# Galtvam/OthelloZero

Measured on AMD Instinct MI355X. Metric: mcts_node_expansions_per_sec, higher is better.
Workload: dtype f32 (3xbf16 split)

## Files before the change

include/othellozero_amd.h:

```cpp
#ifndef OTHELLOZERO_AMD_H
#define OTHELLOZERO_AMD_H
#include <stdint.h>
#ifdef __cplusplus
extern "C" {
#endif

#define OZ_OK 0
#define OZ_ERR_HIP 1
#define OZ_ERR_ARG 2
#define OZ_ERR_CAPACITY 3
#define OZ_ERR_KEY 4
#define OZ_ERR_STATE 5

#define OZ_QMODE_NEP50 0
#define OZ_QMODE_F64 1

#define OZ_LEAF_IDLE 0
#define OZ_LEAF_TERMINAL 1
#define OZ_LEAF_EVAL 2
#define OZ_LEAF_WAIT 3

const char* oz_last_error(void);
int oz_version(void);
int oz_device_count(void);
// ... 13 lines not shown
#define OZ_MINIMAX_NONE INT32_MIN
int oz_rules_minimax(const uint64_t* black, const uint64_t* white, const int8_t* player, int n, int count, int depth, int eval,
                     int32_t* values, uint64_t* bests);

#define OZ_SOLVE_MAX_EMPTIES 12
int oz_rules_solve(const uint64_t* black, const uint64_t* white, const int8_t* player, int n, int count, int max_empties,
                   int32_t* values , uint64_t* bests , int32_t* value , uint8_t* solved );
int oz_rules_solve_sign(const uint64_t* black, const uint64_t* white, const int8_t* player, int n, int count, int max_empties,
                        int8_t* sign , uint8_t* solved );
#define OZ_OPENING_MAX_PLIES 16
int oz_rules_random_openings(int n, int64_t count, int plies, uint64_t opening_seed, uint64_t first_opening_id,
                             uint64_t* black, uint64_t* white, int8_t* player, uint8_t* finished,
                             uint8_t* actions , int32_t* n_plies);
int oz_rules_profile(int enable);
int oz_rules_profile_read(double* ms_total, int64_t* launches, int reset);

typedef struct oz_net oz_net;
int oz_net_create(oz_net** out, int n, int channels, int max_batch);
int oz_net_create_bnn(oz_net** out, int n, int channels, int max_batch);
int oz_net_create_stub(oz_net** out, int n, uint64_t salt, uint64_t keep_mask, int max_batch);
int oz_net_destroy(oz_net* net);
int oz_net_num_weights(const oz_net* net);
int oz_net_weight_size(const oz_net* net, int index, int64_t* nelem);
int oz_net_set_weight(oz_net* net, int index, const float* data, int64_t nelem);
int oz_net_get_weight(const oz_net* net, int index, float* data, int64_t nelem);
int oz_net_init_random(oz_net* net, uint64_t seed);
int oz_net_set_precision(oz_net* net, int mode);
int oz_net_get_precision(const oz_net* net);
int oz_net_check(oz_net* net);
int oz_net_commit(oz_net* net);
int oz_net_predict(oz_net* net, const uint64_t* own, const uint64_t* opp, int count, float* pi, float* v);
int oz_net_predict_boards(oz_net* net, const uint8_t* boards_nhwc, int count, float* pi, float* v);
int oz_net_time_forward(oz_net* net, int count, int iters, float* ms_avg);
int oz_net_profile(oz_net* net, int enable );
int oz_net_profile_read(oz_net* net, double* conv2_ms_total, int64_t* conv2_launches);
#define OZ_NET_KERNELS 7
int oz_net_profile_kernels(oz_net* net, double* ms_total , int64_t* launches , int reset);
int oz_net_profiled_layer(oz_net* net, int* layer);
int oz_net_set_tables(oz_net* net, int mode);
int oz_net_set_eval_cache(oz_net* net, int64_t entries);
int oz_net_eval_cache_stats(oz_net* net, int64_t* entries, int64_t* lookups, int64_t* hits, int64_t* inserts);
#define OZ_NET_OPT_SIMPLE_LOOP 1
#define OZ_NET_OPT_ACT_TARGET_LOG2 2
#define OZ_NET_OPT_LOW_GUARD_LOG2 3
#define OZ_NET_OPT_SELF_CHECK 4
#define OZ_NET_OPT_W_TARGET_LOG2 5
#define OZ_NET_OPT_F32_STD_TILE 6
#define OZ_NET_OPT_LATENCY_SPLITS 7
#define OZ_NET_OPT_CONV3_TILE 8
#define OZ_NET_OPT_LOW_LOOP_PHASES 9
#define OZ_NET_OPT_B3_TILE 10
int oz_net_set_option(oz_net* net, int option, int value);
int oz_net_self_check(oz_net* net, double* max_dpi, double* max_dv, int* positions);
int oz_net_get_scaling(oz_net* net, int which, int32_t* out, int64_t nelem);
#define OZ_NET_INFO_CONV3_TILE_ROWS 1
#define OZ_NET_INFO_SELF_CHECK_GUARD 2
#define OZ_NET_INFO_ARITHMETIC 3
#define OZ_NET_INFO_LAYER_TILE_ROWS(l) (16 + (l))
#define OZ_NET_INFO_LAYER_KSLICES(l) (32 + (l))
#define OZ_NET_INFO_LAYER_KERNEL(l) (48 + (l))
enum {
    OZ_NET_KERNEL_NONE = 0,
    OZ_NET_KERNEL_F32_SKINNY = 1,
    OZ_NET_KERNEL_F32_STD = 2,
    OZ_NET_KERNEL_F32_STD_PIXMAJOR = 3,
    OZ_NET_KERNEL_F32_BIG = 4,
    OZ_NET_KERNEL_LUT = 5,
    OZ_NET_KERNEL_LUT_XCD = 6,
    OZ_NET_KERNEL_LUT_XCD_INLINE = 7,
    OZ_NET_KERNEL_H2_SMALL2 = 10, OZ_NET_KERNEL_H2_SMALL = 11, OZ_NET_KERNEL_H2_BIGPP = 12, OZ_NET_KERNEL_H2_BIGPP_LUT = 13,
    OZ_NET_KERNEL_H2_MIDPP = 14, OZ_NET_KERNEL_H2_LOWPP1 = 15, OZ_NET_KERNEL_H2_LOWPP = 16, OZ_NET_KERNEL_H2_BIG = 17, OZ_NET_KERNEL_H2_MID = 18,
    OZ_NET_KERNEL_H2_THIN2 = 19, OZ_NET_KERNEL_H2_THIN = 20, OZ_NET_KERNEL_H2_THIN4W = 21,
    OZ_NET_KERNEL_B3 = 30,
    OZ_NET_KERNEL_B3_BIG = 31
};
int oz_net_get_info(oz_net* net, int what, int* value);
int oz_net_get_activation(oz_net* net, int layer, int64_t first_row, int64_t rows, double* out );

typedef struct oz_mcts oz_mcts;
int oz_mcts_create(oz_mcts** out, int n, int num_games, int node_cap, double c, int q_mode);
int oz_mcts_destroy(oz_mcts* m);
int oz_mcts_reset(oz_mcts* m, int game );
int oz_mcts_set_dedup(oz_mcts* m, int enable);
int oz_mcts_set_roots(oz_mcts* m, const uint64_t* own, const uint64_t* opp, const uint8_t* active);
int oz_mcts_simulate(oz_mcts* m, oz_net* net, int nsims);
int oz_mcts_select(oz_mcts* m);
int oz_mcts_leaves(oz_mcts* m, int32_t* status, uint64_t* own, uint64_t* opp);
int oz_mcts_backup(oz_mcts* m, const float* pi , const float* v );
int oz_mcts_last_value(oz_mcts* m, double* value, int32_t* vtype, int32_t* depth);
int oz_mcts_root_counts(oz_mcts* m, int32_t* counts, uint64_t* legal, int32_t* rc);
int oz_mcts_policy(oz_mcts* m, double temperature, const uint64_t* tie_draws, double* policy, int32_t* rc);
int oz_mcts_num_nodes(oz_mcts* m, int32_t* num_nodes );
int oz_mcts_dump_node(oz_mcts* m, int game, int index, uint64_t* own, uint64_t* opp, int32_t* Ns, uint64_t* legal,
                      int32_t* N , double* Q , uint8_t* qtag , double* P );
int oz_mcts_stats(oz_mcts* m, int64_t* out5);

#define OZ_MCTS_MAX_LEAVES_PER_STEP 16
int oz_mcts_set_leaves_per_step(oz_mcts* m, int k);
int oz_mcts_get_leaves_per_step(oz_mcts* m, int* k);
int oz_mcts_use_wide_kernels(oz_mcts* m, int enable);
int oz_mcts_wide_stats(oz_mcts* m, int64_t* out3);

#define OZ_SOLVE_LEAVES_MAX_EMPTIES 10
int oz_mcts_set_solve_leaves(oz_mcts* m, int max_empties);
int oz_mcts_get_solve_leaves(oz_mcts* m, int* max_empties, int64_t* rows_solved );
int oz_mcts_solve_leaves_profile(oz_mcts* m, int enable);
int oz_mcts_solve_leaves_profile_read(oz_mcts* m, double* ms_total, int64_t* launches, int reset);

int oz_mcts_set_root_noise(oz_mcts* m, double eps, const double* eta, const uint8_t* armed);
int oz_mcts_sample_root_noise(oz_mcts* m, double alpha, double eps, uint64_t seed, const uint64_t* game_ids, const int32_t* plies);
int oz_mcts_get_root_noise(oz_mcts* m, double* eta , uint8_t* armed , double* eps);

int oz_mcts_sample_moves(oz_mcts* m, double temperature, uint64_t seed, const uint64_t* game_ids, const int32_t* plies,
                         int32_t* action , int32_t* rc );

typedef struct oz_selfplay oz_selfplay;
typedef struct {
    int32_t n;
    int32_t num_games;
    int32_t sims;
    int32_t q_mode;
    double c;
    double temperature;
    double e_greedy;
    uint64_t seed;
    uint64_t first_game_id;
    uint64_t game_id_stride;
    int32_t refill;
    int32_t node_cap;
    int32_t reserved0;
    int32_t record_cap;
    int32_t dedup;
    int32_t batch_cap;
    int32_t eval_cache;
    int32_t record_visits;
} oz_selfplay_config;
#define OZ_DEDUP_DEFAULT 0
#define OZ_DEDUP_ON 1
#define OZ_DEDUP_OFF 2

typedef struct {
    uint64_t black, white;
    uint64_t final_black, final_white;
    uint64_t game_id;
    uint8_t ply;
    uint8_t action;
    int8_t player;
    int8_t z;
    uint8_t greedy;
    uint8_t pad[3];
} oz_record;

typedef struct {
    int64_t simulations, node_visits, expansions, terminal_hits, fallbacks;
    int64_t moves, games_completed, records;
    int32_t live_games, overflow;
    int64_t leaves_evaluated;
} oz_selfplay_stats;

int oz_selfplay_create(oz_selfplay** out, const oz_selfplay_config* cfg, oz_net* net);
int oz_selfplay_destroy(oz_selfplay* sp);
int oz_selfplay_run(oz_selfplay* sp, int rounds);
int oz_selfplay_run_steps(oz_selfplay* sp, int steps);
int oz_selfplay_set_batch_cap(oz_selfplay* sp, int cap);
int oz_selfplay_set_dedup(oz_selfplay* sp, int enable);
int oz_selfplay_set_leaves_per_step(oz_selfplay* sp, int k);
int oz_selfplay_set_solve_leaves(oz_selfplay* sp, int max_empties);
int oz_selfplay_get_solve_leaves(oz_selfplay* sp, int* max_empties, int64_t* rows_solved);
int oz_selfplay_solve_leaves_profile(oz_selfplay* sp, int enable);
int oz_selfplay_solve_leaves_profile_read(oz_selfplay* sp, double* ms_total, int64_t* launches, int reset);
int oz_selfplay_set_root_noise(oz_selfplay* sp, double alpha, double eps);
int oz_selfplay_root_noise(oz_selfplay* sp, double* eta, uint8_t* armed);
int oz_selfplay_set_move_sampling(oz_selfplay* sp, double temperature, int plies);
int oz_selfplay_sync(oz_selfplay* sp);
int oz_selfplay_stagger(oz_selfplay* sp, int sims_pre);
#define OZ_TREE_KERNELS 5
int oz_selfplay_profile(oz_selfplay* sp, int enable);
int oz_selfplay_profile_read(oz_selfplay* sp, double* ms_total , int64_t* launches , int reset);
int oz_selfplay_get_stats(oz_selfplay* sp, oz_selfplay_stats* out);
int oz_selfplay_state(oz_selfplay* sp, uint64_t* black, uint64_t* white, int8_t* player, uint8_t* finished,
                      int32_t* ply, uint64_t* game_id);
int oz_selfplay_records(oz_selfplay* sp, oz_record* out, int64_t max_records, int64_t* written);
int oz_selfplay_records_device(oz_selfplay* sp, void* dst_device, int64_t max_records, int64_t* written);
int oz_selfplay_visits(oz_selfplay* sp, int32_t* out , int64_t max_records, int64_t* written);
int oz_selfplay_visits_device(oz_selfplay* sp, void* dst_device, int64_t max_records, int64_t* written);
typedef struct {
    int64_t records;
    int64_t solved;
    int64_t z_changed;
    int64_t optimal_moves;
    int64_t disc_loss_sum;
    int32_t disc_loss_max, pad;
} oz_endgame_stats;
int oz_selfplay_solve_records(oz_selfplay* sp, int64_t first_record, int max_empties, oz_endgame_stats* stats );
int oz_selfplay_last_counts(oz_selfplay* sp, int32_t* counts);
int oz_selfplay_eval_time(oz_selfplay* sp, double* ms_total, int64_t* launches, int64_t* leaves);

typedef struct oz_comm oz_comm;
#define OZ_COMM_ID_BYTES 128
int oz_comm_unique_id(uint8_t* id );
int oz_comm_create(oz_comm** out, const uint8_t* id, int rank, int world);
int oz_comm_destroy(oz_comm* comm);
int oz_selfplay_gather_records(oz_selfplay* sp, oz_comm* comm, int64_t first_record, oz_record* out, int64_t max_records, int64_t* written,
                               int64_t* per_rank);
int oz_selfplay_gather_visits(oz_selfplay* sp, oz_comm* comm, int64_t first_record, int32_t* out , int64_t max_records,
                              int64_t* written, int64_t* per_rank);

typedef struct oz_arena oz_arena;
int oz_arena_create(oz_arena** out, int n, int num_games, int sims, double c, int q_mode, uint64_t seed,
                    uint64_t first_game_id, oz_net* net_a, oz_net* net_b, int node_cap);
int oz_arena_destroy(oz_arena* a);
int oz_arena_run(oz_arena* a);
int oz_arena_run_rounds(oz_arena* a, int max_rounds);
int oz_arena_stats(oz_arena* a, int64_t* black5, int64_t* white5);
int oz_arena_set_dedup(oz_arena* a, int enable);
int oz_arena_leaves_evaluated(oz_arena* a, int64_t* black, int64_t* white);
int oz_arena_set_eval_cache(oz_arena* a, int enable);
int oz_arena_set_leaves_per_step(oz_arena* a, int k_black, int k_white);
int oz_arena_set_solve_leaves(oz_arena* a, int black, int white);
int oz_arena_get_solve_leaves(oz_arena* a, int64_t* rows_black, int64_t* rows_white);
int oz_arena_profile(oz_arena* a, int enable);
int oz_arena_profile_read(oz_arena* a, double* ms_total , int64_t* launches , int reset);
#define OZ_AGENT_RANDOM 0
#define OZ_AGENT_MINIMAX 1
int oz_arena_set_opponent(oz_arena* a, int side , int kind, int depth, int eval);
int oz_arena_opponent_time(oz_arena* a, double* ms_total, int64_t* launches);
int oz_arena_set_openings(oz_arena* a, int plies, uint64_t opening_seed, uint64_t first_opening_id);
int oz_arena_set_opening_moves(oz_arena* a, const uint8_t* moves , const int32_t* n_plies );
int oz_arena_opening_plies(oz_arena* a, int32_t* out );
int oz_arena_results(oz_arena* a, int8_t* winner , int32_t* points, int32_t* n_moves,
                     uint8_t* actions , int8_t* players ,
                     uint64_t* final_black, uint64_t* final_white);

int oz_examples_expand(const oz_record* records, int64_t count, int n, int alias_final, uint8_t* boards,
                       int32_t* policy_index, int8_t* z);
int oz_symmetry_table(int n, int32_t* perm );
int oz_examples_expand_visits(const oz_record* records, const int32_t* counts, int64_t count, int n, int alias_final, double temperature,
                              uint8_t* boards, double* pi, int8_t* z);

typedef struct oz_trainer oz_trainer;
int oz_trainer_arena_size(int n, int channels, int in_channels, int64_t* nelem);
int oz_trainer_create(oz_trainer** out, int n, int channels, int in_channels, int max_batch, float lr, float clipvalue ,
                      float dropout, float bn_momentum, uint64_t seed, float* external_grads);
int oz_trainer_destroy(oz_trainer* t);
int oz_trainer_set_precision(oz_trainer* t, int mode);
#define OZ_POLICY_LOSS_ROWS 0
#define OZ_POLICY_LOSS_FLAT 1
int oz_trainer_set_policy_loss(oz_trainer* t, int mode);
int oz_trainer_set_weight(oz_trainer* t, int index, const float* data, int64_t nelem);
int oz_trainer_get_weight(oz_trainer* t, int index, float* data, int64_t nelem);
int oz_trainer_get_grad(oz_trainer* t, int index, float* data, int64_t nelem);
int oz_trainer_grad_arena(oz_trainer* t, void** device_ptr, int64_t* nelem);
int oz_trainer_forward_backward(oz_trainer* t, const uint64_t* own, const uint64_t* opp, const float* pi_target,
                                const float* z_target, int B, float* losses3);
int oz_trainer_apply(oz_trainer* t);
int oz_trainer_set_dataset(oz_trainer* t, const uint64_t* own, const uint64_t* opp, const float* pi_target, const float* z_target, int64_t N);
int oz_trainer_fit_epoch(oz_trainer* t, const int32_t* order, int64_t count, int batch, float* losses3);
int oz_trainer_outputs(oz_trainer* t, int B, float* p , float* v );
int oz_trainer_get_activation(oz_trainer* t, int layer, int B, float* data, int64_t nelem);
#define OZ_TRAINER_PLAN_FIELDS 8
#define OZ_TRAINER_PLAN_FWD_KSLICES 0
#define OZ_TRAINER_PLAN_FWD_KERNEL 1
#define OZ_TRAINER_PLAN_DGRAD_KSLICES 2
#define OZ_TRAINER_PLAN_DGRAD_KERNEL 3
#define OZ_TRAINER_PLAN_DGRAD_TAP_SKIP 4
#define OZ_TRAINER_PLAN_WGRAD_KERNEL 5
#define OZ_TRAINER_PLAN_WGRAD_MSPLIT 6
enum {
    OZ_TRAINER_WGRAD_TAPS_F32 = 1,
    OZ_TRAINER_WGRAD_BOARDS_F32 = 2,
    OZ_TRAINER_WGRAD_OCT_H2 = 3,
    OZ_TRAINER_WGRAD_OCT_B3 = 4
};
int oz_trainer_get_preact(oz_trainer* t, int layer, int B, float* data, int64_t nelem);
int oz_trainer_get_dz(oz_trainer* t, int layer, int B, float* data, int64_t nelem);
int oz_trainer_set_capture(oz_trainer* t, int on);
int oz_trainer_get_dgrad(oz_trainer* t, int layer, int B, float* data, int64_t nelem);
int oz_trainer_get_head_grads(oz_trainer* t, int B, float* dlogit , float* dvpre );
int oz_trainer_get_plan(oz_trainer* t, int* plan, int n);
int oz_trainer_sync(oz_trainer* t);
int oz_trainer_step_count(oz_trainer* t, int64_t* step);

typedef struct oz_replay oz_replay;
#define OZ_REPLAY_TARGET_ONEHOT 0
#define OZ_REPLAY_TARGET_VISITS 1
int oz_replay_create(oz_replay** out, int n, int64_t capacity );
int oz_replay_destroy(oz_replay* r);
int oz_replay_clear(oz_replay* r);
int oz_replay_info(oz_replay* r, int64_t* held, int64_t* capacity, int64_t* total);
int oz_replay_append_selfplay(oz_replay* r, oz_selfplay* sp, int64_t first_record, int alias_final, int target, double temperature,
                              int64_t* appended_records);
int oz_replay_append_records(oz_replay* r, const oz_record* records, const int32_t* counts, int64_t count, int alias_final,
                             int target, double temperature);
int oz_replay_append_examples(oz_replay* r, const uint64_t* own, const uint64_t* opp, const float* pi ,
                              const float* z, int64_t count);
int oz_replay_restore(oz_replay* r, const uint64_t* own, const uint64_t* opp, const float* pi, const float* z, int64_t count, int64_t total);
int oz_replay_read(oz_replay* r, int64_t first_slot, int64_t count, uint64_t* own, uint64_t* opp, float* pi, float* z);
int oz_trainer_fit_epoch_replay(oz_trainer* t, oz_replay* r, const int32_t* order, int64_t count, int batch, float* losses3);

int oz_selftest_arith(const double* a, const double* b, int count, double* sqrt_a, double* div_ab, float* fdiv_ab,
                      float* fchain);
int oz_selftest_mfma_rate(int kind, double target_ms, double* tflops, double* clock_ghz, double* ms_measured);
int oz_selftest_b3_split(const float* x, int64_t count, float* planes, float* sum);

#ifdef __cplusplus
}
#endif
#endif
```

othellozero_amd/_lib.py:

```python
import ctypes as C
import os

import numpy as np

_HERE = os.path.dirname(os.path.abspath(__file__))
LIB_PATH = os.environ.get("OZ_LIB_PATH") or os.path.join(_HERE, "lib", "libothellozero_amd.so")

OZ_OK, OZ_ERR_HIP, OZ_ERR_ARG, OZ_ERR_CAPACITY, OZ_ERR_KEY, OZ_ERR_STATE = range(6)
QMODE_NEP50, QMODE_F64 = 0, 1
DEDUP_DEFAULT, DEDUP_ON, DEDUP_OFF = 0, 1, 2
NET_OPT_SIMPLE_LOOP, NET_OPT_ACT_TARGET_LOG2, NET_OPT_LOW_GUARD_LOG2, NET_OPT_SELF_CHECK, NET_OPT_W_TARGET_LOG2, NET_OPT_F32_STD_TILE, NET_OPT_LATENCY_SPLITS = 1, 2, 3, 4, 5, 6, 7
NET_OPT_CONV3_TILE = 8
NET_OPT_LOW_LOOP_PHASES = 9
NET_OPT_B3_TILE = 10
NET_INFO_CONV3_TILE_ROWS, NET_INFO_SELF_CHECK_GUARD, NET_INFO_ARITHMETIC = 1, 2, 3
NET_INFO_LAYER_TILE_ROWS, NET_INFO_LAYER_KSLICES, NET_INFO_LAYER_KERNEL = 16, 32, 48
NET_KERNEL_NAMES = {0: "none", 1: "f32_skinny", 2: "f32_std", 3: "f32_std_pixmajor", 4: "f32_big", 5: "lut", 6: "lut_xcd", 7: "lut_xcd_inline",
                    10: "h2_small2", 11: "h2_small", 12: "h2_bigpp", 13: "h2_bigpp_lut", 14: "h2_midpp", 15: "h2_lowpp1", 16: "h2_lowpp", 17: "h2_big",
                    18: "h2_mid", 19: "h2_thin2", 20: "h2_thin", 21: "h2_thin4w", 30: "b3", 31: "b3_big"}
LEAF_IDLE, LEAF_TERMINAL, LEAF_EVAL = 0, 1, 2
VT_INT, VT_F32, VT_F64 = 0, 1, 2
MAX_LEAVES_PER_STEP = 16
POLICY_LOSS_ROWS, POLICY_LOSS_FLAT = 0, 1
TRAINER_PLAN_FIELDS = 8
TRAINER_WGRAD_NAMES = {0: "none", 1: "taps_f32", 2: "boards_f32", 3: "oct_h2", 4: "oct_b3"}
MINIMAX_EVAL_DISCS, MINIMAX_EVAL_WEIGHTED, MINIMAX_MAX_DEPTH, MINIMAX_NONE = 0, 1, 6, -2 ** 31
MINIMAX_EVALS = {"discs": MINIMAX_EVAL_DISCS, "weighted": MINIMAX_EVAL_WEIGHTED}
SOLVE_MAX_EMPTIES = 12
SOLVE_LEAVES_MAX_EMPTIES = 10
AGENT_RANDOM, AGENT_MINIMAX = 0, 1
OPENING_MAX_PLIES = 16
REPLAY_TARGET_ONEHOT, REPLAY_TARGET_VISITS = 0, 1
NET_KERNELS = ("input", "conv2", "conv3", "conv4", "fc1", "fc2", "heads")
TREE_KERNELS = ("select", "compact", "network", "expand_backup", "roots_move")


class OzLibraryError(RuntimeError):
    pass


class OzError(RuntimeError):
    def __init__(self, code, msg):
        super().__init__(f"[oz error {code}] {msg}")
        self.code = code


class SelfplayConfig(C.Structure):
    _fields_ = [
        ("n", C.c_int32), ("num_games", C.c_int32), ("sims", C.c_int32), ("q_mode", C.c_int32),
        ("c", C.c_double), ("temperature", C.c_double), ("e_greedy", C.c_double),
        ("seed", C.c_uint64), ("first_game_id", C.c_uint64), ("game_id_stride", C.c_uint64),
        ("refill", C.c_int32), ("node_cap", C.c_int32), ("reserved0", C.c_int32), ("record_cap", C.c_int32),
        ("dedup", C.c_int32), ("batch_cap", C.c_int32), ("eval_cache", C.c_int32), ("record_visits", C.c_int32),
    ]


class SelfplayStats(C.Structure):
    _fields_ = [
        ("simulations", C.c_int64), ("node_visits", C.c_int64), ("expansions", C.c_int64),
        ("terminal_hits", C.c_int64), ("fallbacks", C.c_int64),
        ("moves", C.c_int64), ("games_completed", C.c_int64), ("records", C.c_int64),
        ("live_games", C.c_int32), ("overflow", C.c_int32),
        ("leaves_evaluated", C.c_int64),
    ]


class EndgameStats(C.Structure):
    _fields_ = [
        ("records", C.c_int64), ("solved", C.c_int64), ("z_changed", C.c_int64), ("optimal_moves", C.c_int64), ("disc_loss_sum", C.c_int64),
        ("disc_loss_max", C.c_int32), ("pad", C.c_int32),
    ]


RECORD_DTYPE = np.dtype([
    ("black", "<u8"), ("white", "<u8"), ("final_black", "<u8"), ("final_white", "<u8"), ("game_id", "<u8"),
    ("ply", "u1"), ("action", "u1"), ("player", "i1"), ("z", "i1"), ("greedy", "u1"), ("pad", "u1", (3,)),
])
assert RECORD_DTYPE.itemsize == 48

_u64p, _i32p, _f32p, _f64p = (C.POINTER(t) for t in (C.c_uint64, C.c_int32, C.c_float, C.c_double))
_u8p, _i8p, _i64p, _vp = C.POINTER(C.c_uint8), C.POINTER(C.c_int8), C.POINTER(C.c_int64), C.c_void_p

SIGNATURES = {
    "oz_version": [], "oz_device_count": [], "oz_set_device": [C.c_int],
    "oz_rules_legal_moves": [_u64p, _u64p, C.c_int, C.c_int, _u64p],
    "oz_rules_apply_moves": [_u64p, _u64p, _u8p, C.c_int, C.c_int, _u64p, _u64p],
    "oz_rules_status": [_u64p, _u64p, C.c_int, C.c_int, _u8p, _i32p, _i32p, _i8p],
    "oz_rules_play": [_u64p, _u64p, _i8p, _u8p, C.c_int, C.c_int, _u64p, _u64p, _i8p, _u8p],
    "oz_rules_minimax": [_u64p, _u64p, _i8p, C.c_int, C.c_int, C.c_int, C.c_int, _i32p, _u64p],
    "oz_rules_solve": [_u64p, _u64p, _i8p, C.c_int, C.c_int, C.c_int, _i32p, _u64p, _i32p, _u8p],
    "oz_rules_solve_sign": [_u64p, _u64p, _i8p, C.c_int, C.c_int, C.c_int, _i8p, _u8p],
    "oz_rules_random_openings": [C.c_int, C.c_int64, C.c_int, C.c_uint64, C.c_uint64, _u64p, _u64p, _i8p, _u8p, _u8p, _i32p],
    "oz_rules_profile": [C.c_int], "oz_rules_profile_read": [_f64p, _i64p, C.c_int],
    "oz_selfplay_solve_records": [_vp, C.c_int64, C.c_int, C.POINTER(EndgameStats)],
    "oz_net_create": [C.POINTER(_vp), C.c_int, C.c_int, C.c_int],
    "oz_net_create_bnn": [C.POINTER(_vp), C.c_int, C.c_int, C.c_int],
    "oz_net_create_stub": [C.POINTER(_vp), C.c_int, C.c_uint64, C.c_uint64, C.c_int],
    "oz_net_destroy": [_vp], "oz_net_num_weights": [_vp],
    "oz_net_weight_size": [_vp, C.c_int, _i64p],
    "oz_net_set_weight": [_vp, C.c_int, _f32p, C.c_int64],
    "oz_net_get_weight": [_vp, C.c_int, _f32p, C.c_int64],
    "oz_net_commit": [_vp],
    "oz_net_set_precision": [_vp, C.c_int], "oz_net_get_precision": [_vp], "oz_net_check": [_vp],
    "oz_net_init_random": [_vp, C.c_uint64],
    "oz_net_predict": [_vp, _u64p, _u64p, C.c_int, _f32p, _f32p],
    "oz_net_predict_boards": [_vp, _u8p, C.c_int, _f32p, _f32p],
    "oz_net_time_forward": [_vp, C.c_int, C.c_int, _f32p],
    "oz_net_profile": [_vp, C.c_int], "oz_net_profile_read": [_vp, _f64p, _i64p],
    "oz_net_profiled_layer": [_vp, C.POINTER(C.c_int)], "oz_net_set_tables": [_vp, C.c_int],
    "oz_net_profile_kernels": [_vp, _f64p, _i64p, C.c_int],
    "oz_net_set_eval_cache": [_vp, C.c_int64], "oz_net_eval_cache_stats": [_vp, _i64p, _i64p, _i64p, _i64p],
    "oz_net_set_option": [_vp, C.c_int, C.c_int], "oz_net_get_info": [_vp, C.c_int, C.POINTER(C.c_int)],
    "oz_net_get_scaling": [_vp, C.c_int, _i32p, C.c_int64],
    "oz_net_get_activation": [_vp, C.c_int, C.c_int64, C.c_int64, _f64p],
    "oz_net_self_check": [_vp, _f64p, _f64p, C.POINTER(C.c_int)],
    "oz_mcts_create": [C.POINTER(_vp), C.c_int, C.c_int, C.c_int, C.c_double, C.c_int],
    "oz_mcts_destroy": [_vp], "oz_mcts_reset": [_vp, C.c_int], "oz_mcts_set_dedup": [_vp, C.c_int],
    "oz_mcts_set_roots": [_vp, _u64p, _u64p, _u8p],
    "oz_mcts_simulate": [_vp, _vp, C.c_int], "oz_mcts_select": [_vp],
    "oz_mcts_leaves": [_vp, _i32p, _u64p, _u64p],
    "oz_mcts_backup": [_vp, _f32p, _f32p],
    "oz_mcts_last_value": [_vp, _f64p, _i32p, _i32p],
    "oz_mcts_root_counts": [_vp, _i32p, _u64p, _i32p],
    "oz_mcts_policy": [_vp, C.c_double, _u64p, C.POINTER(C.c_double), _i32p],
    "oz_mcts_num_nodes": [_vp, _i32p],
    "oz_mcts_dump_node": [_vp, C.c_int, C.c_int, _u64p, _u64p, _i32p, _u64p, _i32p, _f64p, _u8p, _f64p],
    "oz_mcts_stats": [_vp, _i64p],
    "oz_mcts_set_leaves_per_step": [_vp, C.c_int], "oz_mcts_get_leaves_per_step": [_vp, C.POINTER(C.c_int)],
    "oz_mcts_use_wide_kernels": [_vp, C.c_int], "oz_mcts_wide_stats": [_vp, _i64p],
    "oz_selfplay_set_leaves_per_step": [_vp, C.c_int], "oz_arena_set_leaves_per_step": [_vp, C.c_int, C.c_int],
    "oz_mcts_set_solve_leaves": [_vp, C.c_int], "oz_mcts_get_solve_leaves": [_vp, C.POINTER(C.c_int), _i64p],
    "oz_mcts_solve_leaves_profile": [_vp, C.c_int], "oz_mcts_solve_leaves_profile_read": [_vp, _f64p, _i64p, C.c_int],
    "oz_selfplay_set_solve_leaves": [_vp, C.c_int], "oz_selfplay_get_solve_leaves": [_vp, C.POINTER(C.c_int), _i64p],
    "oz_selfplay_solve_leaves_profile": [_vp, C.c_int], "oz_selfplay_solve_leaves_profile_read": [_vp, _f64p, _i64p, C.c_int],
    "oz_arena_set_solve_leaves": [_vp, C.c_int, C.c_int], "oz_arena_get_solve_leaves": [_vp, _i64p, _i64p],
    "oz_mcts_set_root_noise": [_vp, C.c_double, _f64p, _u8p],
    "oz_mcts_sample_root_noise": [_vp, C.c_double, C.c_double, C.c_uint64, _u64p, _i32p],
    "oz_mcts_get_root_noise": [_vp, _f64p, _u8p, _f64p],
    "oz_selfplay_set_root_noise": [_vp, C.c_double, C.c_double], "oz_selfplay_root_noise": [_vp, _f64p, _u8p],
    "oz_mcts_sample_moves": [_vp, C.c_double, C.c_uint64, _u64p, _i32p, _i32p, _i32p],
    "oz_selfplay_set_move_sampling": [_vp, C.c_double, C.c_int],
    "oz_selfplay_create": [C.POINTER(_vp), C.POINTER(SelfplayConfig), _vp],
    "oz_selfplay_destroy": [_vp], "oz_selfplay_run": [_vp, C.c_int], "oz_selfplay_run_steps": [_vp, C.c_int], "oz_selfplay_sync": [_vp],
    "oz_selfplay_stagger": [_vp, C.c_int], "oz_selfplay_profile": [_vp, C.c_int], "oz_selfplay_set_batch_cap": [_vp, C.c_int], "oz_selfplay_set_dedup": [_vp, C.c_int],
    "oz_selfplay_profile_read": [_vp, _f64p, _i64p, C.c_int],
    "oz_selfplay_get_stats": [_vp, C.POINTER(SelfplayStats)],
    "oz_selfplay_state": [_vp, _u64p, _u64p, _i8p, _u8p, _i32p, _u64p],
    "oz_selfplay_records": [_vp, _vp, C.c_int64, _i64p],
    "oz_selfplay_records_device": [_vp, _vp, C.c_int64, _i64p],
    "oz_selfplay_visits": [_vp, _i32p, C.c_int64, _i64p],
    "oz_selfplay_visits_device": [_vp, _vp, C.c_int64, _i64p],
    "oz_selfplay_last_counts": [_vp, _i32p],
    "oz_selfplay_eval_time": [_vp, _f64p, _i64p, _i64p],
    "oz_comm_unique_id": [_u8p], "oz_comm_create": [C.POINTER(_vp), _u8p, C.c_int, C.c_int], "oz_comm_destroy": [_vp],
    "oz_selfplay_gather_records": [_vp, _vp, C.c_int64, _vp, C.c_int64, _i64p, _i64p],
    "oz_selfplay_gather_visits": [_vp, _vp, C.c_int64, _i32p, C.c_int64, _i64p, _i64p],
    "oz_arena_create": [C.POINTER(_vp), C.c_int, C.c_int, C.c_int, C.c_double, C.c_int, C.c_uint64, C.c_uint64, _vp, _vp, C.c_int],
    "oz_arena_destroy": [_vp], "oz_arena_run": [_vp], "oz_arena_run_rounds": [_vp, C.c_int], "oz_arena_stats": [_vp, _i64p, _i64p],
    "oz_arena_set_dedup": [_vp, C.c_int], "oz_arena_set_eval_cache": [_vp, C.c_int], "oz_arena_profile": [_vp, C.c_int], "oz_arena_profile_read": [_vp, _f64p, _i64p, C.c_int], "oz_arena_leaves_evaluated": [_vp, _i64p, _i64p],
    "oz_arena_set_opponent": [_vp, C.c_int, C.c_int, C.c_int, C.c_int], "oz_arena_opponent_time": [_vp, _f64p, _i64p],
    "oz_arena_set_openings": [_vp, C.c_int, C.c_uint64, C.c_uint64], "oz_arena_set_opening_moves": [_vp, _u8p, _i32p],
    "oz_arena_opening_plies": [_vp, _i32p],
    "oz_arena_results": [_vp, _i8p, _i32p, _i32p, _u8p, _i8p, _u64p, _u64p],
    "oz_examples_expand": [_vp, C.c_int64, C.c_int, C.c_int, _u8p, _i32p, _i8p],
    "oz_examples_expand_visits": [_vp, _i32p, C.c_int64, C.c_int, C.c_int, C.c_double, _u8p, _f64p, _i8p],
    "oz_symmetry_table": [C.c_int, _i32p],
    "oz_selftest_arith": [_f64p, _f64p, C.c_int, _f64p, _f64p, _f32p, _f32p],
    "oz_selftest_mfma_rate": [C.c_int, C.c_double, _f64p, _f64p, _f64p],
    "oz_selftest_b3_split": [_f32p, C.c_int64, _f32p, _f32p],
    "oz_trainer_arena_size": [C.c_int, C.c_int, C.c_int, C.POINTER(C.c_int64)],
    "oz_trainer_create": [C.POINTER(_vp), C.c_int, C.c_int, C.c_int, C.c_int, C.c_float, C.c_float, C.c_float, C.c_float,
                          C.c_uint64, _vp],
    "oz_trainer_destroy": [_vp],
    "oz_trainer_set_weight": [_vp, C.c_int, _f32p, C.c_int64],
    "oz_trainer_get_weight": [_vp, C.c_int, _f32p, C.c_int64],
    "oz_trainer_get_grad": [_vp, C.c_int, _f32p, C.c_int64],
    "oz_trainer_grad_arena": [_vp, C.POINTER(_vp), C.POINTER(C.c_int64)],
    "oz_trainer_forward_backward": [_vp, _u64p, _u64p, _f32p, _f32p, C.c_int, _f32p],
    "oz_trainer_apply": [_vp],
    "oz_trainer_set_dataset": [_vp, _u64p, _u64p, _f32p, _f32p, C.c_int64],
    "oz_trainer_fit_epoch": [_vp, _i32p, C.c_int64, C.c_int, _f32p],
    "oz_trainer_outputs": [_vp, C.c_int, _f32p, _f32p],
    "oz_trainer_get_activation": [_vp, C.c_int, C.c_int, _f32p, C.c_int64],
    "oz_trainer_get_preact": [_vp, C.c_int, C.c_int, _f32p, C.c_int64], "oz_trainer_get_dz": [_vp, C.c_int, C.c_int, _f32p, C.c_int64],
    "oz_trainer_set_capture": [_vp, C.c_int], "oz_trainer_get_dgrad": [_vp, C.c_int, C.c_int, _f32p, C.c_int64],
    "oz_trainer_get_plan": [_vp, _i32p, C.c_int],
    "oz_trainer_get_head_grads": [_vp, C.c_int, _f32p, _f32p],
    "oz_trainer_sync": [_vp],
    "oz_trainer_set_precision": [_vp, C.c_int],
    "oz_trainer_set_policy_loss": [_vp, C.c_int],
    "oz_trainer_step_count": [_vp, C.POINTER(C.c_int64)],
    "oz_replay_create": [C.POINTER(_vp), C.c_int, C.c_int64], "oz_replay_destroy": [_vp], "oz_replay_clear": [_vp],
    "oz_replay_info": [_vp, _i64p, _i64p, _i64p],
    "oz_replay_append_selfplay": [_vp, _vp, C.c_int64, C.c_int, C.c_int, C.c_double, _i64p],
    "oz_replay_append_records": [_vp, _vp, _i32p, C.c_int64, C.c_int, C.c_int, C.c_double],
    "oz_replay_append_examples": [_vp, _u64p, _u64p, _f32p, _f32p, C.c_int64],
    "oz_replay_restore": [_vp, _u64p, _u64p, _f32p, _f32p, C.c_int64, C.c_int64],
    "oz_replay_read": [_vp, C.c_int64, C.c_int64, _u64p, _u64p, _f32p, _f32p],
    "oz_trainer_fit_epoch_replay": [_vp, _vp, _i32p, C.c_int64, C.c_int, _f32p],
}

_LIB = None
PRELOAD_TORCH_HIP = True


HIP_RUNTIME_BOUND = None


def _elf_dynamic_strings(path):
    import struct
    with open(path, "rb") as f:
        data = f.read()
    if data[:4] != b"\x7fELF" or data[4] != 2 or data[5] != 1:
        raise ValueError("not a little-endian ELF64 file")
    phoff, = struct.unpack_from("<Q", data, 0x20)
    phentsize, phnum = struct.unpack_from("<HH", data, 0x36)
    loads, dyn = [], None
    for k in range(phnum):
        p_type, _flags, p_offset, p_vaddr, _paddr, p_filesz = struct.unpack_from("<IIQQQQ", data, phoff + k * phentsize)
        if p_type == 1:
            loads.append((p_vaddr, p_offset, p_filesz))
        elif p_type == 2:
            dyn = (p_offset, p_filesz)
    if dyn is None:
        return None, []
    entries = [struct.unpack_from("<qQ", data, dyn[0] + 16 * k) for k in range(dyn[1] // 16)]
    strtab = next((v for t, v in entries if t == 5), None)
    if strtab is None:
        return None, []
    off = next((strtab - va + fo for va, fo, sz in loads if va <= strtab < va + sz), strtab)

    def name(idx):
        end = data.index(b"\0", off + idx)
        return data[off + idx:end].decode()
    soname = next((name(v) for t, v in entries if t == 14), None)
    return soname, [name(v) for t, v in entries if t == 1]


def _one_hip_runtime(lib_path):
    global HIP_RUNTIME_BOUND
    import importlib.util
    import sys
    import warnings
    HIP_RUNTIME_BOUND = "system"
    if not PRELOAD_TORCH_HIP:
        return
    try:
        spec = importlib.util.find_spec("torch")
        cand = os.path.join(os.path.dirname(spec.origin), "lib", "libamdhip64.so") if spec and spec.origin else None
    except Exception:
        return
    if not cand or not os.path.exists(cand):
        return
    try:
        bundled_soname, _ = _elf_dynamic_strings(cand)
        _, needed = _elf_dynamic_strings(lib_path)
        wanted = next((x for x in needed if x.startswith("libamdhip64.so")), None)
    except Exception as e:
        warnings.warn(f"othellozero_amd: could not compare PyTorch's bundled HIP runtime with the library's ({e}); using the system runtime")
        return
    if "torch" in sys.modules:
        HIP_RUNTIME_BOUND = "torch:" + cand
        if wanted and bundled_soname != wanted:
            warnings.warn(f"othellozero_amd: PyTorch's HIP runtime ({bundled_soname}) is not the one this library was linked against ({wanted}): "
                          "two HIP runtimes in one process; do not hand torch device pointers or streams to the library")
            HIP_RUNTIME_BOUND = "system"
        return
    if wanted and bundled_soname == wanted:
        C.CDLL(cand, mode=C.RTLD_GLOBAL)
        HIP_RUNTIME_BOUND = "torch:" + cand
    else:
        warnings.warn(f"othellozero_amd: PyTorch bundles HIP runtime {bundled_soname}, the library was linked against {wanted}: not preloading it; "
                      "a later `import torch` will put two HIP runtimes in this process (keep torch device pointers away from the library)")


def load(path=None):
    global _LIB
    if _LIB is not None and path is None:
        return _LIB
    p = path or LIB_PATH
    if not os.path.exists(p):
        raise OzLibraryError(
            f"{p} not found: the HIP extension is required (no CPU fallback). Build it with "
            "`python -m othellozero_amd.build` (hipcc --offload-arch=gfx950).")
    _one_hip_runtime(p)
    try:
        lib = C.CDLL(p)
    except OSError as e:
        raise OzLibraryError(f"cannot load {p}: {e}") from e
    lib.oz_last_error.restype = C.c_char_p
    lib.oz_last_error.argtypes = []
    for name, args in SIGNATURES.items():
        try:
            fn = getattr(lib, name)
        except AttributeError as e:
            raise OzLibraryError(f"{p} does not export {name}") from e
        fn.argtypes = args
        fn.restype = C.c_int
    if path is None:
        _LIB = lib
    return lib


def check_root_noise(root_noise):
    if root_noise is None:
        return None
    try:
        alpha, eps = (float(x) for x in root_noise)
    except (TypeError, ValueError):
        raise ValueError(f"root_noise must be None or (alpha, epsilon), got {root_noise!r}") from None
    if not 0.01 <= alpha <= 100.0:
        raise ValueError(f"root_noise: alpha must be in [0.01, 100] (got {alpha})")
    if not 0.0 <= eps <= 1.0:
        raise ValueError(f"root_noise: epsilon must be in [0, 1] (got {eps})")
    return alpha, eps


def check_sample_moves(sample_moves):
    if sample_moves is None:
        return None
    try:
        temperature, plies = sample_moves
        temperature = float(temperature)
        if isinstance(plies, bool) or int(plies) != plies:
            raise ValueError
        plies = int(plies)
    except (TypeError, ValueError):
        raise ValueError(f"sample_moves must be None or (temperature, plies), got {sample_moves!r}") from None
    if not 0.01 <= temperature <= 100.0:
        raise ValueError(f"sample_moves: temperature must be in [0.01, 100] (got {temperature})")
    if not 0 <= plies <= 64:
        raise ValueError(f"sample_moves: plies must be in [0, 64] (got {plies})")
    return temperature, plies


def check_minimax(depth, evaluation):
    if isinstance(depth, bool) or not isinstance(depth, (int, np.integer)) or not 1 <= depth <= MINIMAX_MAX_DEPTH:
        raise ValueError(f"minimax: depth must be a whole number in 1..{MINIMAX_MAX_DEPTH} (got {depth!r})")
    if not isinstance(evaluation, str) or evaluation not in MINIMAX_EVALS:
        raise ValueError(f"minimax: evaluation must be 'discs' or 'weighted' (got {evaluation!r})")
    return int(depth), MINIMAX_EVALS[evaluation]


def check_solve_empties(empties, least=0, what="max_empties"):
    if isinstance(empties, bool) or not isinstance(empties, (int, np.integer)) or not least <= empties <= SOLVE_MAX_EMPTIES:
        raise ValueError(f"endgame solver: {what} must be a whole number in {least}..{SOLVE_MAX_EMPTIES} (got {empties!r})")
    return int(empties)


def check_solve_leaves(solve_leaves, what="solve_leaves"):
    if (isinstance(solve_leaves, bool) or not isinstance(solve_leaves, (int, np.integer))
            or not 0 <= solve_leaves <= SOLVE_LEAVES_MAX_EMPTIES):
        raise ValueError(f"{what} must be a whole number in 0..{SOLVE_LEAVES_MAX_EMPTIES} (got {solve_leaves!r})")
    return int(solve_leaves)


def check_solve_leaves_pair(solve_leaves):
    if isinstance(solve_leaves, (tuple, list)):
        if len(solve_leaves) != 2:
            raise ValueError(f"solve_leaves must be E or (E_black, E_white) (got {solve_leaves!r})")
        return check_solve_leaves(solve_leaves[0], "solve_leaves[black]"), check_solve_leaves(solve_leaves[1], "solve_leaves[white]")
    e = check_solve_leaves(solve_leaves)
    return e, e


def check_endgame_targets(endgame_targets, alias_final_boards):
    e = check_solve_empties(endgame_targets, 0, "endgame_targets")
    if e > 0 and alias_final_boards:
        raise ValueError("endgame_targets needs alias_final_boards=False: an exact value belongs to the position of its move, not to the "
                         "game's final position")
    return e


def check_opponent(opponent):
    if opponent is None or (isinstance(opponent, str) and opponent == "random"):
        return None
    if isinstance(opponent, (tuple, list)) and len(opponent) in (2, 3) and isinstance(opponent[0], str) and opponent[0] == "minimax":
        return check_minimax(opponent[1], opponent[2] if len(opponent) == 3 else "weighted")
    raise ValueError(f"opponent must be None, 'random', ('minimax', depth) or ('minimax', depth, 'discs' | 'weighted'), got {opponent!r}")


def check_opponents(opponent, black_free, white_free):
    if isinstance(opponent, dict):
        if set(opponent) - {"black", "white"}:
            raise ValueError(f"opponent: a dict takes the keys 'black' and 'white' (got {sorted(map(str, opponent))})")
        black, white = check_opponent(opponent.get("black")), check_opponent(opponent.get("white"))
        if (black is not None and not black_free) or (white is not None and not white_free):
            raise ValueError("opponent: a colour that has a network cannot be given a minimax opponent")
        return black, white
    spec = check_opponent(opponent)
    if spec is None:
        return None, None
    if black_free and white_free:
        raise ValueError("opponent: neither colour has a network; say who plays which as {'black': ..., 'white': ...}")
    if not black_free and not white_free:
        raise ValueError("opponent: both colours have a network, there is no colour for the minimax opponent to play")
    return (spec, None) if black_free else (None, spec)


def _whole(x, lo, hi):
    return not isinstance(x, bool) and isinstance(x, (int, np.integer)) and lo <= x <= hi


def check_opening_plies(plies, what="openings"):
    if not _whole(plies, 0, OPENING_MAX_PLIES):
        raise ValueError(f"{what}: plies must be a whole number in 0..{OPENING_MAX_PLIES} (got {plies!r})")
    return int(plies)


def check_openings(openings=None, first_opening_id=0, opening_moves=None, num_games=None):
    if not _whole(first_opening_id, 0, 2 ** 64 - 1):
        raise ValueError(f"first_opening_id must be a whole number in 0..2^64 - 1 (got {first_opening_id!r})")
    if openings is not None and opening_moves is not None:
        raise ValueError("openings and opening_moves are two ways to say how the games start: give one of them")
    if openings is not None:
        if not isinstance(openings, (tuple, list)) or len(openings) != 2:
            raise ValueError(f"openings must be None or (plies, opening_seed), got {openings!r}")
        plies = check_opening_plies(openings[0])
        if not _whole(openings[1], 0, 2 ** 64 - 1):
            raise ValueError(f"openings: opening_seed must be a whole number in 0..2^64 - 1 (got {openings[1]!r})")
        return "random", plies, int(openings[1]), int(first_opening_id)
    if opening_moves is not None:
        if not isinstance(opening_moves, (tuple, list)) or len(opening_moves) != 2:
            raise ValueError(f"opening_moves must be None or (moves, n_plies), got {opening_moves!r}")
        moves, n_plies = opening_moves
        if not isinstance(moves, np.ndarray) or moves.dtype != np.uint8 or moves.ndim != 2 or moves.shape[1] != OPENING_MAX_PLIES:
            raise ValueError(f"opening_moves: moves must be a uint8 array of shape (num_games, {OPENING_MAX_PLIES})")
        if not isinstance(n_plies, np.ndarray) or n_plies.dtype != np.int32 or n_plies.shape != (moves.shape[0],):
            raise ValueError("opening_moves: n_plies must be an int32 array of shape (num_games,)")
        if num_games is not None and moves.shape[0] != num_games:
            raise ValueError(f"opening_moves: {moves.shape[0]} move lists for {num_games} games")
        if n_plies.size and (n_plies.min() < 0 or n_plies.max() > OPENING_MAX_PLIES):
            raise ValueError(f"opening_moves: every n_plies must be in 0..{OPENING_MAX_PLIES}")
        return "moves", np.ascontiguousarray(moves), np.ascontiguousarray(n_plies)
    return None


def check(rc):
    if rc != OZ_OK:
        msg = load().oz_last_error().decode("utf-8", "replace")
        if rc == OZ_ERR_KEY:
            raise KeyError(msg)
        raise OzError(rc, msg)


def require_gpu():
    lib = load()
    if lib.oz_device_count() <= 0:
        raise OzLibraryError("no HIP device visible: othellozero_amd computes on an MI355X only (no CPU fallback)")
    return lib


def mfma_rate(kind, target_ms=50.0):
    t, g, m = C.c_double(), C.c_double(), C.c_double()
    check(require_gpu().oz_selftest_mfma_rate({"f32": 0, "f16": 1, "bf16": 2}[kind], float(target_ms), C.byref(t), C.byref(g), C.byref(m)))
    return {"tflops": t.value, "clock_ghz": g.value, "ms": m.value}


def p_u64(a): return a.ctypes.data_as(_u64p)
def p_i32(a): return a.ctypes.data_as(_i32p)
def p_f32(a): return a.ctypes.data_as(_f32p)
def p_f64(a): return a.ctypes.data_as(_f64p)
def p_u8(a): return a.ctypes.data_as(_u8p)
def p_i8(a): return a.ctypes.data_as(_i8p)
def p_i64(a): return a.ctypes.data_as(_i64p)


def pack_board(board):
    b = np.asarray(board).astype(bool)
    n = b.shape[0]
    w = (np.uint64(1) << (np.arange(n, dtype=np.uint64)[:, None] * np.uint64(8) + np.arange(n, dtype=np.uint64)[None, :]))
    return int(w[b[:, :, 0]].sum(dtype=np.uint64)), int(w[b[:, :, 1]].sum(dtype=np.uint64))
# ... 9 lines not shown
```

othellozero_amd/csrc/oz_common.h:

```cpp
#pragma once
#include <hip/hip_runtime.h>
#include <math.h>
#include <stdint.h>

#define OZ_HD __host__ __device__ __forceinline__

OZ_HD uint64_t oz_sm64(uint64_t z) {
    z += 0x9E3779B97F4A7C15ULL;
    z = (z ^ (z >> 30)) * 0xBF58476D1CE4E5B9ULL;
    z = (z ^ (z >> 27)) * 0x94D049BB133111EBULL;
    return z ^ (z >> 31);
}
OZ_HD uint64_t oz_rotl64(uint64_t x, int r) { return (x << r) | (x >> (64 - r)); }

enum { OZ_RNG_COIN = 0, OZ_RNG_EXPLORE = 1, OZ_RNG_TIE = 2, OZ_RNG_NOISE = 3, OZ_RNG_SAMPLE = 4, OZ_RNG_OPENING = 5 };
OZ_HD uint64_t oz_rng(uint64_t seed, uint64_t game, uint64_t move, uint64_t stream) {
    uint64_t a = oz_sm64(seed + 0x632BE59BD9B4E019ULL * game);
    return oz_sm64(a ^ (move * 0x9E3779B97F4A7C15ULL) ^ (stream * 0xD1B54A32D192ED03ULL));
}
OZ_HD double oz_rng_unit(uint64_t u) { return (double)(u >> 11) * (1.0 / 9007199254740992.0); }

OZ_HD uint64_t oz_stub_h(uint64_t own, uint64_t opp, uint64_t salt, uint64_t i) {
    return oz_sm64(oz_sm64(own ^ salt) ^ oz_rotl64(opp, 29) ^ ((i + 1) * 0xD6E8FEB86659FD93ULL));
}

OZ_HD uint64_t oz_valid_mask(int n) {
    uint64_t row = (1ULL << n) - 1ULL, m = 0;
    for (int r = 0; r < n; ++r) m |= row << (8 * r);
    return m;
}

#define OZ_NOT_COL0 0xFEFEFEFEFEFEFEFEULL
#define OZ_NOT_COL7 0x7F7F7F7F7F7F7F7FULL

template <int D> OZ_HD uint64_t oz_shift(uint64_t x) {
    if (D == 0) return x << 8;
    if (D == 1) return x >> 8;
    if (D == 2) return (x << 1) & OZ_NOT_COL0;
    if (D == 3) return (x >> 1) & OZ_NOT_COL7;
    if (D == 4) return (x << 9) & OZ_NOT_COL0;
    if (D == 5) return (x >> 9) & OZ_NOT_COL7;
    if (D == 6) return (x << 7) & OZ_NOT_COL7;
    return (x >> 7) & OZ_NOT_COL0;
}

template <int D> OZ_HD uint64_t oz_legal_dir(uint64_t own, uint64_t opp) {
    uint64_t t = oz_shift<D>(own) & opp;
    t |= oz_shift<D>(t) & opp; t |= oz_shift<D>(t) & opp; t |= oz_shift<D>(t) & opp;
    t |= oz_shift<D>(t) & opp; t |= oz_shift<D>(t) & opp;
    return oz_shift<D>(t);
}

OZ_HD uint64_t oz_legal(uint64_t own, uint64_t opp, uint64_t valid) {
    uint64_t m = oz_legal_dir<0>(own, opp) | oz_legal_dir<1>(own, opp) | oz_legal_dir<2>(own, opp) |
                 oz_legal_dir<3>(own, opp) | oz_legal_dir<4>(own, opp) | oz_legal_dir<5>(own, opp) |
                 oz_legal_dir<6>(own, opp) | oz_legal_dir<7>(own, opp);
    return m & ~(own | opp) & valid;
}

template <int D, int B> OZ_HD uint64_t oz_flips_dir(uint64_t bit, uint64_t own, uint64_t opp) {
    uint64_t x = oz_shift<D>(bit) & opp;
    if (!x) return 0;
    const uint64_t occ = own | opp;
    uint64_t seg = x;
    seg |= oz_shift<D>(seg) & occ; seg |= oz_shift<D>(seg) & occ; seg |= oz_shift<D>(seg) & occ;
    seg |= oz_shift<D>(seg) & occ; seg |= oz_shift<D>(seg) & occ; seg |= oz_shift<D>(seg) & occ;
    uint64_t back = seg & own;
    back |= oz_shift<B>(back) & seg; back |= oz_shift<B>(back) & seg; back |= oz_shift<B>(back) & seg;
    back |= oz_shift<B>(back) & seg; back |= oz_shift<B>(back) & seg; back |= oz_shift<B>(back) & seg;
    return back & opp;
}

OZ_HD uint64_t oz_flips(uint64_t own, uint64_t opp, int sq) {
    const uint64_t bit = 1ULL << sq;
    return oz_flips_dir<0, 1>(bit, own, opp) | oz_flips_dir<1, 0>(bit, own, opp) |
           oz_flips_dir<2, 3>(bit, own, opp) | oz_flips_dir<3, 2>(bit, own, opp) |
           oz_flips_dir<4, 5>(bit, own, opp) | oz_flips_dir<5, 4>(bit, own, opp) |
           oz_flips_dir<6, 7>(bit, own, opp) | oz_flips_dir<7, 6>(bit, own, opp);
}

OZ_HD void oz_apply(uint64_t& own, uint64_t& opp, int sq) {
    const uint64_t f = oz_flips(own, opp, sq);
    own |= f | (1ULL << sq);
    opp &= ~(f | (1ULL << sq));
}

OZ_HD void oz_game_play(uint64_t& black, uint64_t& white, int& player, int& finished, int sq, uint64_t valid) {
    if (player == 1) oz_apply(black, white, sq); else oz_apply(white, black, sq);
    player = -player;
    uint64_t mine = player == 1 ? black : white, theirs = player == 1 ? white : black;
    if (oz_legal(mine, theirs, valid) == 0) {
        if (oz_legal(theirs, mine, valid) == 0) finished = 1;
        else player = -player;
    }
}

OZ_HD int oz_popc(uint64_t x) {
#if defined(__HIP_DEVICE_COMPILE__)
    return __popcll(x);
#else
    return __builtin_popcountll(x);
#endif
}
OZ_HD int oz_ctz(uint64_t x) {
#if defined(__HIP_DEVICE_COMPILE__)
    return __ffsll((unsigned long long)x) - 1;
#else
    return __builtin_ctzll(x);
#endif
}
OZ_HD int oz_kth_bit(uint64_t m, int k) {
    for (int i = 0; i < k; ++i) m &= m - 1;
    return oz_ctz(m);
}

__host__ __device__ inline double pairwise_sum(const double* a, int len) {
    double r0 = a[0], r1 = a[1], r2 = a[2], r3 = a[3], r4 = a[4], r5 = a[5], r6 = a[6], r7 = a[7];
    int i;
    for (i = 8; i < len - (len % 8); i += 8) {
        r0 += a[i]; r1 += a[i + 1]; r2 += a[i + 2]; r3 += a[i + 3];
        r4 += a[i + 4]; r5 += a[i + 5]; r6 += a[i + 6]; r7 += a[i + 7];
    }
    double res = ((r0 + r1) + (r2 + r3)) + ((r4 + r5) + (r6 + r7));
    for (; i < len; ++i) res += a[i];
    return res;
}

OZ_HD int oz_sym_src(int t, int n, int r, int c) {
    const int k = (t >> 1) + 1, flip = !(t & 1);
    int rr = r, cc = flip ? (n - 1 - c) : c;
    for (int q = 0; q < (k & 3); ++q) { int ti = cc, tj = n - 1 - rr; rr = ti; cc = tj; }
    return rr * n + cc;
}

__device__ __forceinline__ double oz_count_pow(int cnt, double inv, int k) {
    const double x = (double)cnt;
    if (k > 0) {
        double r = x;
        for (int i = 1; i < k; ++i) r *= x;
        if (r <= 9007199254740992.0) return r;
    }
    return pow(x, inv);
}
inline int oz_count_pow_k(double inv) { return (inv == floor(inv) && inv <= 64.0) ? (int)inv : 0; }

#include <stdio.h>
void oz_set_error(const char* fmt, ...);
#define OZ_HIP(call)                                                                     \
    do {                                                                                  \
        hipError_t e__ = (call);                                                          \
        if (e__ != hipSuccess) {                                                          \
            oz_set_error("%s failed: %s (%s:%d)", #call, hipGetErrorString(e__), __FILE__, __LINE__); \
            return OZ_ERR_HIP;                                                            \
        }                                                                                 \
    } while (0)
#define OZ_REQUIRE(cond, ...)                                                             \
    do {                                                                                  \
        if (!(cond)) { oz_set_error(__VA_ARGS__); return OZ_ERR_ARG; }                    \
    } while (0)

typedef float f32x4 __attribute__((ext_vector_type(4)));
typedef float f32x16 __attribute__((ext_vector_type(16)));
typedef _Float16 f16x8 __attribute__((ext_vector_type(8)));
typedef __bf16 bf16x8 __attribute__((ext_vector_type(8)));
typedef unsigned u32x4 __attribute__((ext_vector_type(4)));
typedef const __attribute__((address_space(1))) void* oz_gptr;
typedef __attribute__((address_space(3))) void* oz_lptr;

__device__ __forceinline__ void h2_split(float x, _Float16& h1, _Float16& h2) {
    h1 = (_Float16)x;
    h2 = (_Float16)(x - (float)h1);
}
__device__ __forceinline__ void b3_split(float x, __bf16& b1, __bf16& b2, __bf16& b3) {
    b1 = (__bf16)x;
    if (__builtin_isinf((float)b1) && !__builtin_isinf(x)) b1 = __builtin_bit_cast(__bf16, (unsigned short)(x < 0.f ? 0xFF7Fu : 0x7F7Fu));
    const float r1 = x - (float)b1;
    b2 = (__bf16)r1;
    b3 = (__bf16)(r1 - (float)b2);
}
template <bool NT> __device__ __forceinline__ void oz_store16(uint4* dst, u32x4 v) {
    if constexpr (NT) __builtin_nontemporal_store(v, reinterpret_cast<u32x4*>(dst));
    else *reinterpret_cast<u32x4*>(dst) = v;
}
template <int PLANES, bool NT = false>
__device__ __forceinline__ void oz_split8_store(uint4* dst, size_t pstride, const float (&v)[8]) {
    static_assert(PLANES == 2 || PLANES == 3, "f16x2 or bf16x3");
    if constexpr (PLANES == 2) {
        f16x8 h1, h2;
#pragma unroll
        for (int j = 0; j < 8; ++j) {
            _Float16 a, b;
            h2_split(v[j], a, b);
            h1[j] = a; h2[j] = b;
        }
        oz_store16<NT>(dst, __builtin_bit_cast(u32x4, h1));
        oz_store16<NT>(dst + pstride, __builtin_bit_cast(u32x4, h2));
    } else {
        bf16x8 p0, p1, p2;
#pragma unroll
        for (int j = 0; j < 8; ++j) {
            __bf16 a, b, c;
            b3_split(v[j], a, b, c);
            p0[j] = a; p1[j] = b; p2[j] = c;
        }
        oz_store16<NT>(dst, __builtin_bit_cast(u32x4, p0));
        oz_store16<NT>(dst + pstride, __builtin_bit_cast(u32x4, p1));
        oz_store16<NT>(dst + 2 * pstride, __builtin_bit_cast(u32x4, p2));
    }
}
OZ_HD size_t h2_group_chunk(size_t row, int K, int k) { return (row * (size_t)(K >> 3) + (k >> 3)) * 2; }
template <bool NT = false>
__device__ __forceinline__ void h2_store8(uint4* out, size_t row, int K, int k, const float (&v)[8]) {
    oz_split8_store<2, NT>(out + h2_group_chunk(row, K, k), 1, v);
}
OZ_HD size_t b3_group_chunk(size_t row, int K, int k) { return row * (size_t)(K / 32 * 12) + (k >> 5) * 12 + ((k >> 3) & 3); }
template <bool NT = false>
__device__ __forceinline__ void b3_store8(uint4* out, size_t row, int K, int k, const float (&v)[8]) {
    oz_split8_store<3, NT>(out + b3_group_chunk(row, K, k), 4, v);
}
template <int PLANES>
__device__ __forceinline__ void oz_split8_load(const uint4* src, size_t pstride, double (&v)[8]) {
    static_assert(PLANES == 2 || PLANES == 3, "f16x2 or bf16x3");
#pragma unroll
    for (int j = 0; j < 8; ++j) v[j] = 0.0;
#pragma unroll
    for (int p = 0; p < PLANES; ++p) {
        const u32x4 raw = *reinterpret_cast<const u32x4*>(src + p * pstride);
        if constexpr (PLANES == 2) {
            const f16x8 h = __builtin_bit_cast(f16x8, raw);
#pragma unroll
            for (int j = 0; j < 8; ++j) v[j] += (double)(float)h[j];
        } else {
            const bf16x8 b = __builtin_bit_cast(bf16x8, raw);
#pragma unroll
            for (int j = 0; j < 8; ++j) v[j] += (double)(float)b[j];
        }
    }
}
```

othellozero_amd/csrc/oz_net.hip:

```cpp
#include <math.h>
#include <stdlib.h>
#include <string.h>

#include <algorithm>
#include <type_traits>
#include <vector>

#include "oz_internal.h"

__global__ __launch_bounds__(256) void k_conv1(const uint64_t* __restrict__ own, const uint64_t* __restrict__ opp,
                                               const int* __restrict__ d_count, int n, int C,
                                               const float* __restrict__ W , const float* __restrict__ scale,
                                               const float* __restrict__ shift, float* __restrict__ out ) {
    const int P = n * n, cq = C >> 2;
    const long long M = (long long)(*d_count) * P;
    const long long idx = (long long)blockIdx.x * blockDim.x + threadIdx.x;
    const long long m = idx / cq;
    if (m >= M) return;
    const int c4 = (int)(idx % cq) * 4;
    const int b = (int)(m / P), pix = (int)(m % P), y = pix / n, x = pix % n;
    const uint64_t o = own[b], p = opp[b];
    float acc0 = 0.f, acc1 = 0.f, acc2 = 0.f, acc3 = 0.f;
#pragma unroll
    for (int ky = 0; ky < 3; ++ky)
// ... 101 lines not shown
    };
    const int swz = chunk ^ ((srow >> 1) & 7);
    static_assert((RPP / 2) % 8 == 0, "rows of one thread must share the swizzle key");
    const int wave_u = __builtin_amdgcn_readfirstlane(wave);
    const float* brow[IB];
#pragma unroll
    for (int i = 0; i < IB; ++i) brow[i] = Wt + (size_t)(nt * BN + srow + RPP * i) * g.K + swz * 4;
    const float* zsrc = g_gm_zero_line + swz * 4;

    auto stage = [&](int kt, int buf) {
        const int tap = tap_of(kt), ci0 = (kt % kpt) * GM_BK, k0 = tap * g.Cin + ci0;
        const long long toff = ((long long)(tap / 3) * g.Hin + (tap % 3)) * g.Cin + ci0 + swz * 4;
        float* la = tileA(buf);
        float* lb = tileB(buf);
#pragma unroll
        for (int i = 0; i < IA; ++i) {
            const float* ga = ((amask[i] >> tap) & 1) ? in + abase[i] + toff : zsrc;
            __builtin_amdgcn_global_load_lds((oz_gptr)ga, (oz_lptr)(la + (wave_u * 8 + RPP * i) * GM_LDS_STRIDE), 16, 0, 0);
        }
#pragma unroll
        for (int i = 0; i < IB; ++i)
            __builtin_amdgcn_global_load_lds((oz_gptr)(brow[i] + k0), (oz_lptr)(lb + (wave_u * 8 + RPP * i) * GM_LDS_STRIDE), 16, 0, 0);
    };

    f32x16 acc[TI][TJ];
#pragma unroll
    for (int i = 0; i < TI; ++i)
#pragma unroll
        for (int jj = 0; jj < TJ; ++jj)
#pragma unroll
            for (int r = 0; r < 16; ++r) acc[i][jj][r] = 0.f;

    const int nk_all = g.pixmajor ? __builtin_popcount(tmask) * kpt : g.K / GM_BK, nk_s = (nk_all + g.ksplit - 1) / g.ksplit;
    const int kt0 = blockIdx.y * nk_s, nk = min(nk_all, kt0 + nk_s);
    const int r32 = lane & 31, half = lane >> 5;
    const int key = (r32 >> 1) & 7;
    if (kt0 < nk) stage(kt0, kt0 & 1);
    asm volatile("s_waitcnt vmcnt(0)" ::: "memory");
    __syncthreads();
    for (int kt = kt0; kt < nk; ++kt) {
        const int buf = kt & 1;
        if (kt + 1 < nk) stage(kt + 1, buf ^ 1);
        const float* At = tileA(buf) + (wm * TI * 32 + r32) * GM_LDS_STRIDE;
        const float* Bt = tileB(buf) + (wn * TJ * 32 + r32) * GM_LDS_STRIDE;
        f32x4 fa[2][TI], fb[2][TJ];
        auto ldfrag = [&](int s, int w) {
            const int off = ((2 * s + half) ^ key) * 4;
#pragma unroll
            for (int i = 0; i < TI; ++i) fa[w][i] = *reinterpret_cast<const f32x4*>(At + i * 32 * GM_LDS_STRIDE + off);
#pragma unroll
            for (int jj = 0; jj < TJ; ++jj) fb[w][jj] = *reinterpret_cast<const f32x4*>(Bt + jj * 32 * GM_LDS_STRIDE + off);
        };
        ldfrag(0, 0);
#pragma unroll
        for (int s = 0; s < 4; ++s) {
            const int w = s & 1;
            if (s < 3) ldfrag(s + 1, w ^ 1);
            __builtin_amdgcn_sched_barrier(0);
#pragma unroll
            for (int q = 0; q < 4; ++q)
#pragma unroll
                for (int i = 0; i < TI; ++i)
#pragma unroll
                    for (int jj = 0; jj < TJ; ++jj)
                        acc[i][jj] = __builtin_amdgcn_mfma_f32_32x32x2f32(fa[w][i][q], fb[w][jj][q], acc[i][jj], 0, 0, 0);
            __builtin_amdgcn_sched_barrier(0);
        }
        asm volatile("s_waitcnt vmcnt(0)" ::: "memory");
        __syncthreads();
    }

    int colj[TJ];
    float scj[TJ], shj[TJ];
#pragma unroll
    for (int jj = 0; jj < TJ; ++jj) {
        colj[jj] = nt * BN + wn * TJ * 32 + jj * 32 + r32;
        scj[jj] = scale[colj[jj]]; shj[jj] = shift[colj[jj]];
    }
#pragma unroll
    for (int i = 0; i < TI; ++i)
#pragma unroll
        for (int r = 0; r < 16; ++r) {
            const int tr = wm * TI * 32 + i * 32 + (r & 3) + 8 * (r >> 2) + 4 * half;
            const long long m = g.pixmajor ? (long long)(tile_b0 + tr) * P + tile_pix : (long long)mt * BM + tr;
            const bool ok = g.pixmajor ? tile_b0 + tr < count : m < M;
            if (!ok) continue;
            if (g.ksplit > 1) {
                float* prow = partial + (size_t)blockIdx.y * g.slab + (size_t)m * g.N;
#pragma unroll
                for (int jj = 0; jj < TJ; ++jj) prow[colj[jj]] = acc[i][jj][r];
            } else {
                float* orow = out + (size_t)m * g.N;
#pragma unroll
                for (int jj = 0; jj < TJ; ++jj) {
                    float v = fmaf(acc[i][jj][r], scj[jj], shj[jj]);
                    if (g.relu) v = v > 0.f ? v : 0.f;
                    orow[colj[jj]] = v;
                }
            }
        }
}

#define SK_COLS 128
#define SK_KB_MAX 256
__global__ __launch_bounds__(256) void k_gemm_f32_skinny(const float* __restrict__ A, const float* __restrict__ Wt, const int* __restrict__ d_count,
                                                         int K, int N, int kb, float* __restrict__ partial, long long slab, GemmGeom g) {
    __shared__ __attribute__((aligned(16))) float As[64 * (SK_KB_MAX + 4)];
    const int P = g.Hout * g.Hout;
    const int M = *d_count * P;
    const int tid = threadIdx.x, lane = tid & 63, wave = tid >> 6, r32 = lane & 31, half = lane >> 5;
    const int n0 = blockIdx.x * SK_COLS + wave * 32, k0 = blockIdx.y * kb, stride = kb + 4;
    const float* wrow = Wt + (size_t)(n0 + r32) * K + k0 + 4 * half;
    f32x4 b[SK_KB_MAX / 8];
#pragma unroll
    for (int q = 0; q < SK_KB_MAX / 8; ++q)
        if (q * 8 < kb) b[q] = *reinterpret_cast<const f32x4*>(wrow + 8 * q);
    const int tiles = M > 32 ? 2 : 1, q4 = kb / 4;
    const int tap = k0 / g.Cin, ci0 = k0 - tap * g.Cin, dy = g.taps == 9 ? tap / 3 : 0, dx = g.taps == 9 ? tap % 3 : 0;
    for (int u = tid; u < tiles * 32 * q4; u += 256) {
        const int m = u / q4, c = (u % q4) * 4;
        f32x4 v = {0.f, 0.f, 0.f, 0.f};
        if (m < M) {
            const int b = m / P, pix = m - b * P, iy = pix / g.Hout - g.pad + dy, ix = pix % g.Hout - g.pad + dx;
            if (iy >= 0 && iy < g.Hin && ix >= 0 && ix < g.Hin)
                v = *reinterpret_cast<const f32x4*>(A + (((size_t)b * g.Hin + iy) * g.Hin + ix) * g.Cin + ci0 + c);
        }
        *reinterpret_cast<f32x4*>(&As[m * stride + c]) = v;
    }
    __syncthreads();
    f32x16 acc0, acc1;
#pragma unroll
    for (int r = 0; r < 16; ++r) { acc0[r] = 0.f; acc1[r] = 0.f; }
    const float* a0p = &As[r32 * stride + 4 * half];
    const float* a1p = a0p + 32 * stride;
#pragma unroll
    for (int q = 0; q < SK_KB_MAX / 8; ++q) {
        if (q * 8 < kb) {
            const f32x4 a0 = *reinterpret_cast<const f32x4*>(a0p + 8 * q);
#pragma unroll
            for (int j = 0; j < 4; ++j) acc0 = __builtin_amdgcn_mfma_f32_32x32x2f32(a0[j], b[q][j], acc0, 0, 0, 0);
            if (tiles == 2) {
                const f32x4 a1 = *reinterpret_cast<const f32x4*>(a1p + 8 * q);
#pragma unroll
                for (int j = 0; j < 4; ++j) acc1 = __builtin_amdgcn_mfma_f32_32x32x2f32(a1[j], b[q][j], acc1, 0, 0, 0);
            }
        }
    }
    float* outp = partial + (size_t)blockIdx.y * slab;
#pragma unroll
    for (int r = 0; r < 16; ++r) {
        const int m = (r & 3) + 8 * (r >> 2) + 4 * half;
        if (m < M) outp[(size_t)m * N + n0 + r32] = acc0[r];
        if (tiles == 2 && m + 32 < M) outp[(size_t)(m + 32) * N + n0 + r32] = acc1[r];
    }
}

__global__ __launch_bounds__(256) void k_splitk_reduce_f32(const float* __restrict__ partial, long long slab, int ksplit, int N, int P,
                                                           const int* __restrict__ d_count, const float* __restrict__ scale,
                                                           const float* __restrict__ shift, int relu, float* __restrict__ out) {
    const long long total = (long long)(*d_count) * P * N;
    const long long i = ((long long)blockIdx.x * blockDim.x + threadIdx.x) * 4;
    if (i >= total) return;
    f32x4 a = *reinterpret_cast<const f32x4*>(partial + i);
    constexpr int RB = 24;
    for (int s0 = 1; s0 < ksplit; s0 += RB) {
        f32x4 b[RB];
#pragma unroll
        for (int q = 0; q < RB; ++q) if (s0 + q < ksplit) b[q] = *reinterpret_cast<const f32x4*>(partial + (size_t)(s0 + q) * slab + i);
#pragma unroll
        for (int q = 0; q < RB; ++q) if (s0 + q < ksplit) { a[0] += b[q][0]; a[1] += b[q][1]; a[2] += b[q][2]; a[3] += b[q][3]; }
    }
    const int col = (int)(i % N);
    f32x4 r;
#pragma unroll
    for (int q = 0; q < 4; ++q) {
        float v = fmaf(a[q], scale[col + q], shift[col + q]);
        r[q] = relu && v < 0.f ? 0.f : v;
    }
    *reinterpret_cast<f32x4*>(out + i) = r;
}

static inline int gemm_grid(int num_mt, int per_mt) { return num_mt < 8 ? ((per_mt + 7) / 8) * 8 * num_mt : ((num_mt + 7) / 8) * 8 * per_mt; }

static void launch_splitk_reduce_f32(const float* partial, long long slab, int ksplit, int N, int P, int max_count, const int* d_count,
                                     const float* scale, const float* shift, int relu, float* out, hipStream_t s) {
    const long long quads = ((long long)max_count * P * N + 3) / 4;
    hipLaunchKernelGGL(k_splitk_reduce_f32, dim3((unsigned)((quads + 255) / 256)), dim3(256), 0, s, partial, slab, ksplit, N, P, d_count, scale, shift, relu, out);
}

int oz_gemm_f32_launch(const float* in, const float* Wt, const float* scale, const float* shift, float* out,
                       const int* d_count, int max_count, int Hin, int Hout, int pad, int Cin, int taps, int N, int relu,
                       hipStream_t s, float* partial, long long partial_floats, int sizing_count, int core_lo, int core_hi,
                       int* tile_rows_out, int force_std_tile, OzDeferredReduce* defer, int* plan_out) {
    if (defer) *defer = OzDeferredReduce();
    int tile_rows_dummy = 0, plan_dummy[2] = {1, 0};
    int& tile_rows = tile_rows_out ? *tile_rows_out : tile_rows_dummy;
    int* const plan = plan_out ? plan_out : plan_dummy;
    OZ_REQUIRE(N % GM_BN == 0 && Cin % GM_BK == 0, "gemm_f32: N %% 128 and Cin %% 32 must be 0 (N=%d Cin=%d)", N, Cin);
    GemmGeom g;
    oz_geom_set_shape(g, OzLayerShape{Hin, Hout, pad, Cin, taps, N});
    g.relu = relu; g.core_lo = core_lo; g.core_hi = core_hi;
    const long long Mmax = (long long)max_count * Hout * Hout;
    const int cap = sizing_count > 0 ? sizing_count : max_count;
    const bool has_zero_taps = pad > 0 || core_lo > 0 || (core_hi >= 0 && core_hi < Hin);
    g.pixmajor = taps == 9 && has_zero_taps && cap >= 2 * GM_BM && ((cap + GM_BM - 1) / GM_BM) * GM_BM <= cap + cap / 8;
    const int num_mt = g.pixmajor ? ((max_count + GM_BM - 1) / GM_BM) * Hout * Hout : (int)((Mmax + GM_BM - 1) / GM_BM);
    const int grid = ((num_mt + 7) / 8) * 8 * (N / GM_BN);
    const int Pout = Hout * Hout;
    if (partial && (long long)cap * Pout <= 64 && (long long)max_count * Pout <= 64 && Cin % 64 == 0 && N % SK_COLS == 0) {
        int kb = SK_KB_MAX;
        while (kb > 64 && (Cin % kb != 0 || (long long)(N / SK_COLS) * (g.K / kb) < 192)) kb /= 2;
        const int ks = g.K / kb;
        if ((long long)ks * max_count * Pout * N <= partial_floats) {
            const long long slab = (long long)max_count * Pout * N;
            g.ksplit = ks; g.slab = slab; g.pixmajor = 0;
            tile_rows = 64; plan[0] = ks; plan[1] = OZ_NET_KERNEL_F32_SKINNY;
            hipLaunchKernelGGL(k_gemm_f32_skinny, dim3(N / SK_COLS, ks), dim3(256), 0, s, in, Wt, d_count, g.K, N, kb, partial, slab, g);
            if (defer && relu) { defer->partial = partial; defer->slab = slab; defer->ksplit = ks; defer->scale = scale; defer->shift = shift; OZ_HIP(hipGetLastError()); return OZ_OK; }
            launch_splitk_reduce_f32(partial, slab, ks, N, Pout, max_count, d_count, scale, shift, relu, out, s);
            OZ_HIP(hipGetLastError());
            return OZ_OK;
        }
    }
    int ksplit = 1;
    const int nk = g.K / GM_BK;
    if (partial && !g.pixmajor) {
        const long long Ms = (long long)(sizing_count > 0 ? sizing_count : max_count) * Hout * Hout;
        const int grid_s = (int)((Ms + GM_BM - 1) / GM_BM) * (N / GM_BN);
        const int split_blocks = 256;
        while (ksplit < 16 && grid_s * ksplit < split_blocks && nk / (ksplit * 2) >= 8 && (long long)(ksplit * 2) * (Ms > Mmax ? Ms : Mmax) * N <= partial_floats) ksplit *= 2;
    }
    g.ksplit = ksplit; g.slab = Mmax * N;
    const long long big_blocks = ((Mmax + GmBig::BM - 1) / GmBig::BM) * (N / GmBig::BN);
    if (taps == 9 && !g.pixmajor && ksplit == 1 && N % GmBig::BN == 0 && big_blocks >= 192 && !force_std_tile) {
        tile_rows = GmBig::BM; plan[0] = 1; plan[1] = OZ_NET_KERNEL_F32_BIG;
        const int num_mt_big = (int)((Mmax + GmBig::BM - 1) / GmBig::BM);
        const int grid_big = ((num_mt_big + 7) / 8) * 8 * (N / GmBig::BN);
        if (int rc = set_max_lds_once<k_gemm_f32<GmBig>>(GmBig::LDS_BYTES)) return rc;
        hipLaunchKernelGGL(k_gemm_f32<GmBig>, dim3(grid_big, 1), dim3(GmBig::NT), GmBig::LDS_BYTES, s, in, Wt, scale, shift, out, d_count, g, num_mt_big, partial);
        OZ_HIP(hipGetLastError());
        return OZ_OK;
    }
    tile_rows = GmStd::BM; plan[0] = ksplit; plan[1] = g.pixmajor ? OZ_NET_KERNEL_F32_STD_PIXMAJOR : OZ_NET_KERNEL_F32_STD;
    if (int rc = set_max_lds_once<k_gemm_f32<GmStd>>(GmStd::LDS_BYTES)) return rc;
    hipLaunchKernelGGL(k_gemm_f32<GmStd>, dim3(grid, ksplit), dim3(GmStd::NT), GmStd::LDS_BYTES, s, in, Wt, scale, shift, out, d_count, g, num_mt, partial);
    OZ_HIP(hipGetLastError());
    if (ksplit > 1 && defer && relu) { defer->partial = partial; defer->slab = g.slab; defer->ksplit = ksplit; defer->scale = scale; defer->shift = shift; }
    else if (ksplit > 1) {
        launch_splitk_reduce_f32(partial, g.slab, ksplit, N, Pout, max_count, d_count, scale, shift, relu, out, s);
        OZ_HIP(hipGetLastError());
    }
    return OZ_OK;
}

#include "oz_net_h2.h"
#include "oz_net_b3.h"
#define B3_MIN_BATCH 128
#define CONV3_LOW_COST 1.30


static int trainer_ksplit(long long blocks, int nk, long long slab_floats, long long partial_floats) {
    int ksplit = 1;
    while (ksplit < 16 && blocks * (ksplit + 1) <= 256 && nk / (ksplit + 1) >= 8 && (long long)(ksplit + 1) * slab_floats <= partial_floats) ++ksplit;
    return ksplit;
}

static long long tile_cost(long long rows, int N, int bm) { return ((((rows + bm - 1) / bm) * (N / 256) + 255) / 256) * bm; }

template <typename CF, int TAG = 0>
static int launch_h2(const OzLayerShape& L, const void* in, const uint4* W, const float* scale, const float* shift, void* out, int packed, OzDeferredReduce* defer,
                     const int* d_count, int max_count, int ksplit, float* slabs, long long slab, const uint4* zero_line, int* flag, hipStream_t s,
                     int relu = 1, H2Low low = H2Low(), const unsigned* lut_ids = nullptr) {
    if (defer) *defer = OzDeferredReduce();
    H2Geom g;
    oz_geom_set_shape(g, L);
    g.out_h2 = packed; g.relu = relu; g.ksplit = ksplit; g.slab = slab;
    if (packed && ksplit == 1) g.low = low;
    const int P = L.pixels(), N = L.N;
    const int num_mt = (int)(((long long)max_count * P + CF::BM - 1) / CF::BM);
    constexpr int LDS = CF::LDS + (CF::LUT ? 9 * CF::BM * 2 : 0);
    if (int rc = set_max_lds_once<k_gemm_h2<CF, TAG>>(LDS)) return rc;
    hipLaunchKernelGGL((k_gemm_h2<CF, TAG>), dim3(gemm_grid(num_mt, (N / CF::BN) * ksplit)), dim3(CF::NT), LDS, s, (const uint4*)in, W, scale, shift,
                       ksplit > 1 ? (void*)slabs : out, d_count, g, num_mt, zero_line, flag, lut_ids);
    if (ksplit > 1 && packed) {
        const long long threads = (long long)max_count * P * (N / 8);
        hipLaunchKernelGGL(k_splitk_reduce_h2, dim3((unsigned)((threads + 255) / 256)), dim3(256), 0, s, (const float*)slabs, slab, ksplit, N, P, d_count,
                           scale, shift, relu, (uint4*)out, flag, low);
    } else if (ksplit > 1 && defer && relu) *defer = OzDeferredReduce{slabs, slab, ksplit, scale, shift};
    else if (ksplit > 1) launch_splitk_reduce_f32(slabs, slab, ksplit, N, P, max_count, d_count, scale, shift, relu, (float*)out, s);
    OZ_HIP(hipGetLastError());
    return OZ_OK;
}

template <int TAG>
static int launch_b3(const OzLayerShape& L, const uint4* in, const uint4* W, const float* scale, const float* shift, void* out, int packed, OzDeferredReduce* defer,
                     const int* d_count, int max_count, bool big, int ksplit, float* slabs, long long slab, const uint4* zero_line, hipStream_t s, int relu = 1) {
    OZ_REQUIRE(L.N % B3_BN == 0 && L.Cin % B3_BK == 0, "gemm_b3: N %% 256 and Cin %% 32 must be 0 (N=%d Cin=%d)", L.N, L.Cin);
    if (defer) *defer = OzDeferredReduce();
    B3Geom g;
    oz_geom_set_shape(g, L);
    g.out_b3 = packed; g.relu = relu; g.ksplit = ksplit; g.slab = slab;
    const int P = L.pixels(), N = L.N, BM = big ? B3B_BM : B3_BM;
    const int num_mt = (int)(((long long)max_count * P + BM - 1) / BM);
    const dim3 grid(gemm_grid(num_mt, (N / B3_BN) * ksplit));
    void* dst = ksplit > 1 ? (void*)slabs : out;
    if (big) {
        if (int rc = set_max_lds_once<k_gemm_b3_big<TAG>>(B3B_LDS)) return rc;
        hipLaunchKernelGGL((k_gemm_b3_big<TAG>), grid, dim3(B3_NT), B3B_LDS, s, in, W, scale, shift, dst, d_count, g, num_mt, zero_line);
    } else {
        if (int rc = set_max_lds_once<k_gemm_b3<TAG>>(B3_LDS)) return rc;
        hipLaunchKernelGGL((k_gemm_b3<TAG>), grid, dim3(B3_NT), B3_LDS, s, in, W, scale, shift, dst, d_count, g, num_mt, zero_line);
    }
    if (ksplit > 1 && packed) {
        const long long threads = (long long)max_count * P * (N / 8);
        hipLaunchKernelGGL(k_splitk_reduce_b3, dim3((unsigned)((threads + 255) / 256)), dim3(256), 0, s, (const float*)slabs, slab, ksplit, N, P, d_count,
                           scale, shift, (uint4*)out);
    } else if (ksplit > 1 && defer && relu) *defer = OzDeferredReduce{slabs, slab, ksplit, scale, shift};
    else if (ksplit > 1) launch_splitk_reduce_f32(slabs, slab, ksplit, N, P, max_count, d_count, scale, shift, relu, (float*)out, s);
    OZ_HIP(hipGetLastError());
    return OZ_OK;
}

static bool b3_big_tile_pays(long long rows, int N) {
    auto paid = [&](int bm) { return (double)tile_cost(rows, N, bm); };
    const long long big_blocks = ((rows + B3B_BM - 1) / B3B_BM) * (N / B3B_BN);
    return big_blocks >= 192 && 0.96 * paid(B3B_BM) <= paid(B3_BM);
}

int oz_gemm_h2_launch(const void* in_h2, const void* Wh, const float* scale, const float* shift, float* out, const int* d_count, int max_count,
                      int Hin, int Hout, int pad, int Cin, int taps, int N, hipStream_t s, float* partial, long long partial_floats,
                      const void* zero_line, int* flag, int* plan_out) {
    OZ_REQUIRE(N % 256 == 0 && Cin % 32 == 0, "gemm_h2: N %% 256 and Cin %% 32 must be 0 (N=%d Cin=%d)", N, Cin);
    const OzLayerShape L = {Hin, Hout, pad, Cin, taps, N};
    const long long Mmax = (long long)max_count * L.pixels();
    const bool big = ((Mmax + 255) / 256) * (N / 256) >= 192;
    const bool mid = big && tile_cost(Mmax, N, 192) < tile_cost(Mmax, N, 256);
    const bool low = !big && partial != nullptr;
    const int ksplit = low ? trainer_ksplit(((Mmax + 127) / 128) * (N / 256), L.K() / H2_BK, Mmax * N, partial_floats) : 1;
    auto go = [&](auto cf) {
        return launch_h2<decltype(cf)>(L, in_h2, (const uint4*)Wh, scale, shift, out, 0, nullptr, d_count, max_count, ksplit, partial, Mmax * N,
                                       (const uint4*)zero_line, flag, s, 0);
    };
    if (plan_out) { plan_out[0] = ksplit; plan_out[1] = mid ? OZ_NET_KERNEL_H2_MIDPP : big ? OZ_NET_KERNEL_H2_BIGPP : low ? OZ_NET_KERNEL_H2_LOWPP : OZ_NET_KERNEL_H2_SMALL; }
    return mid ? go(H2MidPP()) : big ? go(H2BigPP()) : low ? go(H2LowPP()) : go(H2Small());
}

int oz_gemm_b3_launch(const void* in_b3, const void* Wb, const float* scale, const float* shift, float* out, const int* d_count, int max_count,
                      int Hin, int Hout, int pad, int Cin, int taps, int N, int relu, hipStream_t s, float* partial, long long partial_floats,
                      const void* zero_line, int tag, int* plan_out) {
    const OzLayerShape L = {Hin, Hout, pad, Cin, taps, N};
    const long long Mmax = (long long)max_count * L.pixels();
    const bool big = pad == 0 && b3_big_tile_pays(Mmax, N);
    const int ksplit = !big && partial ? trainer_ksplit(((Mmax + B3_BM - 1) / B3_BM) * (N / B3_BN), L.K() / B3_BK, Mmax * N, partial_floats) : 1;
    auto go = [&](auto t) {
        return launch_b3<decltype(t)::value>(L, (const uint4*)in_b3, (const uint4*)Wb, scale, shift, out, 0, nullptr, d_count, max_count, big, ksplit, partial,
                                             Mmax * N, (const uint4*)zero_line, s, relu);
    };
    if (plan_out) { plan_out[0] = ksplit; plan_out[1] = big ? OZ_NET_KERNEL_B3_BIG : OZ_NET_KERNEL_B3; }
    return tag ? go(std::integral_constant<int, 8>()) : go(std::integral_constant<int, 7>());
}
int oz_f32_to_b3_launch(const float* x, const int* d_count, int max_count, int P, int C, void* out, hipStream_t s) {
    OZ_REQUIRE(C % 32 == 0, "f32_to_b3: C %% 32 must be 0 (C=%d)", C);
    const long long threads = (long long)max_count * P * (C / 8);
    hipLaunchKernelGGL(k_f32_to_b3, dim3((unsigned)((threads + 255) / 256)), dim3(256), 0, s, x, d_count, P, C, (uint4*)out);
    OZ_HIP(hipGetLastError());
    return OZ_OK;
}
int oz_w_to_b3_launch(const float* W, int K, int N, int taps, void* out, hipStream_t s) {
    OZ_REQUIRE(K % (32 * taps) == 0, "w_to_b3: K / taps %% 32 must be 0 (K=%d, taps=%d)", K, taps);
    const long long threads = (long long)N * (K / 8);
    hipLaunchKernelGGL(k_w_to_b3, dim3((unsigned)((threads + 255) / 256)), dim3(256), 0, s, W, K, N, taps, (uint4*)out);
    OZ_HIP(hipGetLastError());
    return OZ_OK;
}

__device__ __forceinline__ float oz_deferred_finish(float a, float sc, float sh) { const float y = fmaf(a, sc, sh); return y < 0.f ? 0.f : y; }
template <int LP>
__global__ __launch_bounds__(256) void k_heads_t(const float* __restrict__ f2 , const int* __restrict__ d_count,
                                                 int A, const float* __restrict__ Wpi , const float* __restrict__ bpi,
                                                 const float* __restrict__ Wv , const float* __restrict__ bv,
                                                 float* __restrict__ pi, float* __restrict__ v, OzDeferredReduce dr) {
    __shared__ __attribute__((aligned(16))) float xs[LP][512];
    __shared__ float part[4][LP][64];
    __shared__ float vpart_s[4][LP];
    const int b0 = blockIdx.x * LP, lane = threadIdx.x & 63, w = __builtin_amdgcn_readfirstlane(threadIdx.x >> 6), count = *d_count;
    if (b0 >= count) return;
    const bool act = lane < A;
    const auto wrs = __builtin_amdgcn_make_buffer_rsrc(const_cast<float*>(Wpi + (size_t)w * 128 * A), 0, 128 * A * 4, 0x00020000);
    const int lo = (act ? lane : 0) * 4;
    const float wv0 = Wv[w * 128 + lane * 2], wv1 = Wv[w * 128 + lane * 2 + 1];
    const float bl = act ? bpi[lane] : 0.f, bvv = bv[0];
    constexpr int WB = LP <= 8 ? 64 : 32;
    float wgt[WB];
#pragma unroll
    for (int j = 0; j < WB; ++j) wgt[j] = __builtin_bit_cast(float, __builtin_amdgcn_raw_buffer_load_b32(wrs, lo, j * A * 4, 0));
    if (dr.ksplit > 1) {
#pragma unroll 1
        for (int q = threadIdx.x; q < LP * 128; q += 256) {
            const int p = q >> 7, c4 = (q & 127) * 4;
            if (b0 + p >= count) break;
            const float* src = dr.partial + (size_t)(b0 + p) * 512 + c4;
            f32x4 a = *reinterpret_cast<const f32x4*>(src);
            constexpr int RB = 15;
            for (int s0 = 1; s0 < dr.ksplit; s0 += RB) {
                f32x4 b[RB];
#pragma unroll
                for (int t = 0; t < RB; ++t) if (s0 + t < dr.ksplit) b[t] = *reinterpret_cast<const f32x4*>(src + (size_t)(s0 + t) * dr.slab);
#pragma unroll
                for (int t = 0; t < RB; ++t) if (s0 + t < dr.ksplit) { a[0] += b[t][0]; a[1] += b[t][1]; a[2] += b[t][2]; a[3] += b[t][3]; }
            }
            const f32x4 sc = *reinterpret_cast<const f32x4*>(dr.scale + c4), sh = *reinterpret_cast<const f32x4*>(dr.shift + c4);
            f32x4 r;
#pragma unroll
            for (int t = 0; t < 4; ++t) r[t] = oz_deferred_finish(a[t], sc[t], sh[t]);
            *reinterpret_cast<f32x4*>(&xs[p][c4]) = r;
        }
    } else
    for (int q = threadIdx.x; q < LP * 128; q += 256) {
        const int p = q >> 7, c4 = (q & 127) * 4;
        *reinterpret_cast<f32x4*>(&xs[p][c4]) = *reinterpret_cast<const f32x4*>(f2 + (size_t)(b0 + p < count ? b0 + p : count - 1) * 512 + c4);
    }
    __syncthreads();
    float logit[LP], vp[LP];
#pragma unroll
    for (int p = 0; p < LP; ++p) { logit[p] = 0.f; vp[p] = 0.f; }
#pragma unroll 1
    for (int i0 = 0; i0 < 128; i0 += WB) {
        float nxt[WB];
        const bool more = i0 + WB < 128;
#pragma unroll
        for (int j = 0; j < WB; ++j) nxt[j] = __builtin_bit_cast(float, __builtin_amdgcn_raw_buffer_load_b32(wrs, lo, ((more ? i0 + WB : 0) + j) * A * 4, 0));
        __builtin_amdgcn_sched_barrier(0);
#pragma unroll
        for (int p = 0; p < LP; ++p) {
#pragma unroll
            for (int j4 = 0; j4 < WB; j4 += 4) {
                const f32x4 x = *reinterpret_cast<const f32x4*>(&xs[p][w * 128 + i0 + j4]);
#pragma unroll
                for (int j = 0; j < 4; ++j) logit[p] = fmaf(x[j], wgt[j4 + j], logit[p]);
            }
            if ((p & 1) == 1) __builtin_amdgcn_sched_barrier(0);
        }
#pragma unroll
        for (int j = 0; j < WB; ++j) wgt[j] = nxt[j];
    }
#pragma unroll
    for (int i = 0; i < 2; ++i) {
        const float wv = i == 0 ? wv0 : wv1;
#pragma unroll
        for (int p = 0; p < LP; ++p) vp[p] = fmaf(xs[p][w * 128 + lane * 2 + i], wv, vp[p]);
    }
#pragma unroll
    for (int p = 0; p < LP; ++p) {
#pragma unroll
        for (int off = 32; off > 0; off >>= 1) vp[p] += __shfl_xor(vp[p], off, 64);
        part[w][p][lane] = logit[p];
        if (lane == 0) vpart_s[w][p] = vp[p];
    }
    __syncthreads();
#pragma unroll
    for (int q = 0; q < LP / 4; ++q) {
        const int p = w * (LP / 4) + q;
        const float sum = ((part[0][p][lane] + part[1][p][lane]) + part[2][p][lane]) + part[3][p][lane];
        const float lg = act ? sum + bl : -INFINITY;
        float mx = lg;
#pragma unroll
        for (int off = 32; off > 0; off >>= 1) mx = fmaxf(mx, __shfl_xor(mx, off, 64));
        const float e = act ? expf(lg - mx) : 0.f;
        float s = e;
#pragma unroll
        for (int off = 32; off > 0; off >>= 1) s += __shfl_xor(s, off, 64);
        if (b0 + p < count) {
            if (act) pi[(size_t)(b0 + p) * A + lane] = e / s;
            if (lane == 0) v[b0 + p] = tanhf(((vpart_s[0][p] + vpart_s[1][p]) + vpart_s[2][p]) + vpart_s[3][p] + bvv);
        }
    }
}
#define HEADS_P 8
#define HEADS_LP 16

template <int FMT>
__global__ __launch_bounds__(256) void k_act_rows_f64(const void* __restrict__ src, const int* __restrict__ aexp, long long first_row, long long rows, int N,
                                                      double* __restrict__ out) {
    const int ng = N >> 3;
    const long long idx = (long long)blockIdx.x * blockDim.x + threadIdx.x;
    const long long r = idx / ng;
    if (r >= rows) return;
    const int c8 = (int)(idx % ng) * 8;
    const size_t row = (size_t)(first_row + r);
    double v[8];
    if constexpr (FMT == 0) {
#pragma unroll
        for (int j = 0; j < 8; ++j) v[j] = (double)static_cast<const float*>(src)[row * N + c8 + j];
    } else if constexpr (FMT == 1) {
        oz_split8_load<2>(static_cast<const uint4*>(src) + h2_group_chunk(row, N, c8), 1, v);
#pragma unroll
        for (int j = 0; j < 8; ++j) v[j] = ldexp(v[j], -aexp[c8 + j]);
    } else oz_split8_load<3>(static_cast<const uint4*>(src) + b3_group_chunk(row, N, c8), 4, v);
#pragma unroll
    for (int j = 0; j < 8; ++j) out[(size_t)r * N + c8 + j] = v[j];
}
__global__ __launch_bounds__(256) void k_deferred_rows_f64(OzDeferredReduce dr, long long first_row, long long rows, int N, double* __restrict__ out) {
    const long long idx = (long long)blockIdx.x * blockDim.x + threadIdx.x;
    if (idx >= rows * N) return;
    const int c = (int)(idx % N);
    const float* src = dr.partial + (size_t)(first_row + idx / N) * N + c;
    float a = src[0];
    for (int s = 1; s < dr.ksplit; ++s) a += src[(size_t)s * dr.slab];
    out[idx] = (double)oz_deferred_finish(a, dr.scale[c], dr.shift[c]);
}

__global__ __launch_bounds__(64) void k_stub(const uint64_t* __restrict__ own, const uint64_t* __restrict__ opp,
                                             const int* __restrict__ d_count, int n, uint64_t salt, uint64_t keep,
                                             float* __restrict__ pi, float* __restrict__ v) {
    const int b = blockIdx.x, lane = threadIdx.x;
    if (b >= *d_count) return;
    const uint64_t o = own[b], p = opp[b];
    const int r = lane >> 3, c = lane & 7;
    const bool inb = r < n && c < n;
    uint32_t w = 0;
    if (inb) {
        const uint64_t u = oz_stub_h(o, p, salt, (uint64_t)lane);
        w = (uint32_t)((u >> 40) & 0xFFFF);
        if (((u >> 8) & keep) != 0) w = 0;
    }
    uint32_t sum = w;
#pragma unroll
    for (int off = 32; off > 0; off >>= 1) sum += __shfl_xor(sum, off, 64);
    if (sum == 0) { if (lane == 0) w = 1; sum = 1; }
    if (inb) pi[(size_t)b * n * n + r * n + c] = (float)w / (float)sum;
    if (lane == 0) {
        const int32_t m = (int32_t)(oz_stub_h(o, p, salt, 64) >> 40);
        v[b] = (float)(m - 8388608) / 8388608.0f;
    }
}

struct StubNet : oz_net {
    uint64_t salt = 0, keep = 0;
    int forward_device(const uint64_t* d_own, const uint64_t* d_opp, const int* d_count, int max_count, float* d_pi,
                       float* d_v, hipStream_t s) override {
        hipLaunchKernelGGL(k_stub, dim3(max_count), dim3(64), 0, s, d_own, d_opp, d_count, n, salt, keep, d_pi, d_v);
        OZ_HIP(hipGetLastError());
        return OZ_OK;
    }
};

static void calib_positions(int n, int total, std::vector<uint64_t>& own, std::vector<uint64_t>& opp) {
    const uint64_t valid = oz_valid_mask(n);
    const int h = n / 2;
    uint64_t r = 0x0CA11B8A7E5EEDull + (uint64_t)n;
    own.clear(); opp.clear();
    while ((int)own.size() < total) {
        uint64_t white = (1ULL << ((h - 1) * 8 + h - 1)) | (1ULL << (h * 8 + h)), black = (1ULL << ((h - 1) * 8 + h)) | (1ULL << (h * 8 + h - 1));
        int player = 1, finished = 0;
        while (!finished && (int)own.size() < total) {
            const uint64_t mine = player == 1 ? black : white, theirs = player == 1 ? white : black;
            own.push_back(mine); opp.push_back(theirs);
            const uint64_t legal = oz_legal(mine, theirs, valid);
            if (!legal) break;
            r = oz_sm64(r);
            oz_game_play(black, white, player, finished, oz_kth_bit(legal, (int)(r % (uint64_t)oz_popc(legal))), valid);
        }
    }
}
static void pick_exponents(const std::vector<float>& mx, int top, std::vector<int>& e) {
    e.assign(mx.size(), 0);
    std::vector<int> live;
    for (size_t c = 0; c < mx.size(); ++c)
        if (mx[c] > 0.f) {
            int ex = 0;
            frexpf(mx[c], &ex);
            e[c] = std::min(60, std::max(-60, top - ex));
            live.push_back(e[c]);
        }
    int med = 0;
    if (!live.empty()) { std::nth_element(live.begin(), live.begin() + live.size() / 2, live.end()); med = live[live.size() / 2]; }
    for (size_t c = 0; c < mx.size(); ++c) if (!(mx[c] > 0.f)) e[c] = med;
}

struct OnnNet : oz_net {
    int F = 0, A = 0;
    int cin = 2;
    std::vector<std::vector<float>> w;
    bool committed = false;
    float *d_w1 = nullptr, *d_wt[5] = {nullptr, nullptr, nullptr, nullptr, nullptr};
    float *d_scale[6] = {}, *d_shift[6] = {};
    float *d_wpi = nullptr, *d_bpi = nullptr, *d_wv = nullptr, *d_bv = nullptr;
    float *act1 = nullptr, *act2 = nullptr, *act3 = nullptr, *act4 = nullptr, *f1 = nullptr, *f2 = nullptr;
    int precision = 0;
    uint4* d_wh[5] = {nullptr, nullptr, nullptr, nullptr, nullptr};
    float* d_scale_h2[5] = {nullptr, nullptr, nullptr, nullptr, nullptr};
    int* d_flag = nullptr;
    float* d_partial = nullptr;
    float* d_part32 = nullptr;
    uint4* d_zero = nullptr;
    uint4* d_lut = nullptr;
    unsigned* d_lut_ids = nullptr;
    bool lut_ok = false;
    float* d_t2 = nullptr;
    uint4* d_wtap = nullptr;
    float* d_raw = nullptr;
    float* d_lut32 = nullptr;
    float* d_wtap32 = nullptr;
    bool t2f_ok = false;
    float *d_one = nullptr, *d_nul = nullptr;
    int* d_rows = nullptr;
    bool t2_ok = false;
    std::vector<void*> allocs;
    int profile = 0;
    OzTimer timer{OZ_NET_KERNELS};
    int tables_mode = -1;
    OzLayers layers() const { return oz_onn_layers(n, C); }
    int sizing() const { return max_batch; }
    size_t partial_cap = 0;
// ... 755 lines not shown
    *nelem = (int64_t)o->w[index].size();
    return OZ_OK;
}
OZ_API int oz_net_set_weight(oz_net* net, int index, const float* data, int64_t nelem) {
    OnnNet* o = as_onn(net);
    OZ_REQUIRE(o && data, "not an OthelloNN network");
    OZ_REQUIRE(index >= 0 && index < 40, "weight index out of range");
    OZ_REQUIRE(nelem == (int64_t)o->w[index].size(), "weight %d: expected %lld elements, got %lld", index, (long long)o->w[index].size(), (long long)nelem);
    std::lock_guard<std::mutex> lk(o->mu);
    memcpy(o->w[index].data(), data, sizeof(float) * (size_t)nelem);
    o->committed = false;
    return OZ_OK;
}
OZ_API int oz_net_init_random(oz_net* net, uint64_t seed) {
    OnnNet* o = as_onn(net);
    OZ_REQUIRE(o, "not an OthelloNN network");
    std::lock_guard<std::mutex> lk(o->mu);
    const int C_ = o->C, n2 = o->A;
    for (int i = 0; i < 40; ++i) {
        std::vector<float>& a = o->w[i];
        const int layer = i < 36 ? i / 6 : 6 + (i - 36) / 2, part = i < 36 ? i % 6 : (i - 36) % 2;
        if (part == 0) {
            double fan_in, fan_out;
            if (layer < 4) { fan_in = 9.0 * (layer == 0 ? o->cin : C_); fan_out = 9.0 * C_; }
            else if (layer == 4) { fan_in = o->F; fan_out = 1024; }
            else if (layer == 5) { fan_in = 1024; fan_out = 512; }
            else { fan_in = 512; fan_out = layer == 6 ? n2 : 1; }
            const double lim = sqrt(6.0 / (fan_in + fan_out));
            for (size_t k = 0; k < a.size(); ++k) {
                const uint64_t r = oz_sm64(oz_sm64(seed * 0x9E3779B97F4A7C15ull + (uint64_t)i) + k);
                a[k] = (float)((2.0 * ((double)(r >> 11) * (1.0 / 9007199254740992.0)) - 1.0) * lim);
            }
        } else {
            const float fill = (part == 2 || part == 5) ? 1.0f : 0.0f;
            for (auto& x : a) x = fill;
        }
    }
    o->committed = false;
    return OZ_OK;
}
OZ_API int oz_net_get_weight(const oz_net* net, int index, float* data, int64_t nelem) {
    const OnnNet* o = as_onn(const_cast<oz_net*>(net));
    OZ_REQUIRE(o && data, "not an OthelloNN network");
    OZ_REQUIRE(index >= 0 && index < 40, "weight index out of range");
    OZ_REQUIRE(nelem == (int64_t)o->w[index].size(), "weight %d: size mismatch", index);
    memcpy(data, o->w[index].data(), sizeof(float) * (size_t)nelem);
    return OZ_OK;
}

static int upload(OnnNet* o, float** dst, const std::vector<float>& h) {
    if (!*dst) { if (int rc = o->alloc(dst, h.size())) return rc; }
    OZ_HIP(hipMemcpy(*dst, h.data(), sizeof(float) * h.size(), hipMemcpyHostToDevice));
    return OZ_OK;
}

OZ_API int oz_net_commit(oz_net* net) {
    OnnNet* o = as_onn(net);
    OZ_REQUIRE(o, "not an OthelloNN network");
    std::lock_guard<std::mutex> lk(o->mu);
    hipSetDevice(o->device);
    const int C = o->C, n = o->n;
    const int widths[6] = {C, C, C, C, 1024, 512};
    for (int l = 0; l < 6; ++l) {
        std::vector<float> sc(widths[l]), sh(widths[l]);
        const auto &bias = o->w[6 * l + 1], &g = o->w[6 * l + 2], &be = o->w[6 * l + 3], &mu = o->w[6 * l + 4], &var = o->w[6 * l + 5];
        for (int c = 0; c < widths[l]; ++c) {
            const double s = (double)g[c] / sqrt((double)var[c] + 1e-3);
            sc[c] = (float)s;
            sh[c] = (float)(((double)bias[c] - (double)mu[c]) * s + (double)be[c]);
        }
        if (int rc = upload(o, &o->d_scale[l], sc)) return rc;
        if (int rc = upload(o, &o->d_shift[l], sh)) return rc;
        o->bn_sc[l] = sc; o->bn_sh[l] = sh;
    }
    if (o->cin == 2) {
        if (int rc = upload(o, &o->d_w1, o->w[0])) return rc;
    } else {
        std::vector<float> w2((size_t)9 * 2 * C);
        for (int t = 0; t < 9; ++t)
            for (int c = 0; c < C; ++c) { w2[(size_t)(t * 2) * C + c] = o->w[0][(size_t)t * C + c]; w2[(size_t)(t * 2 + 1) * C + c] = -o->w[0][(size_t)t * C + c]; }
        if (int rc = upload(o, &o->d_w1, w2)) return rc;
    }
    const int gl[5] = {6, 12, 18, 24, 30};
    const OzLayers L = o->layers();
    {
        size_t raw_max = 0;
        for (const OzLayerShape& l : L) raw_max = std::max(raw_max, (size_t)l.K() * l.N);
        if (!o->d_raw) { if (int rc = o->alloc(&o->d_raw, raw_max)) return rc; }
    }
    if (o->precision != 1 && !o->d_part32 && o->part32_mult() > 0) {
        if (int rc = o->alloc(&o->d_part32, o->part32_floats())) return rc;
    }
    if (!o->act1) {
        const size_t B = (size_t)o->max_batch;
        if (int rc = o->alloc(&o->act1, B * n * n * C)) return rc;
        float** const outs[5] = {&o->act2, &o->act3, &o->act4, &o->f1, &o->f2};
        for (int i = 0; i < 5; ++i)
            if (int rc = o->alloc(outs[i], B * L[i].pixels() * L[i].N)) return rc;
    }
    if (int rc = upload(o, &o->d_wpi, o->w[36])) return rc;
    if (int rc = upload(o, &o->d_bpi, o->w[37])) return rc;
    if (int rc = upload(o, &o->d_wv, o->w[38])) return rc;
    if (int rc = upload(o, &o->d_bv, o->w[39])) return rc;
    o->t2f_ok = false;
    o->t2_ok = false;
    if (o->precision != 1) {
        for (int i = 0; i < 5; ++i) {
            const auto& src = o->w[gl[i]];
            const int K = L[i].K(), N = L[i].N;
            OZ_REQUIRE(src.size() == (size_t)K * N, "weight %d has %zu values, expected %zu", gl[i], src.size(), (size_t)K * N);
            OZ_HIP(hipMemcpy(o->d_raw, src.data(), sizeof(float) * src.size(), hipMemcpyHostToDevice));
            if (!o->d_wt[i]) { if (int rc = o->alloc(&o->d_wt[i], (size_t)K * N)) return rc; }
            hipLaunchKernelGGL(k_w_transpose, dim3((K + 31) / 32, (N + 31) / 32), dim3(256), 0, 0, o->d_raw, K, N, o->d_wt[i]);
            if (i == 0) {
                if (!o->d_wtap32) { if (int rc = o->alloc(&o->d_wtap32, (size_t)9 * C * C)) return rc; }
                for (int t = 0; t < 9; ++t)
                    hipLaunchKernelGGL(k_w_transpose, dim3((C + 31) / 32, (C + 31) / 32), dim3(256), 0, 0, o->d_raw + (size_t)t * C * C, C, C,
                                       o->d_wtap32 + (size_t)t * C * C);
            }
            if (o->use_b3()) {
                if (!o->d_wb[i]) { if (int rc = o->alloc(&o->d_wb[i], (size_t)N * (K / 32) * 12)) return rc; }
                if (int rc = oz_w_to_b3_launch(o->d_raw, K, N, L[i].taps, o->d_wb[i], 0)) return rc;
            }
            OZ_HIP(hipGetLastError());
            OZ_HIP(hipDeviceSynchronize());
        }
        if (o->use_b3() && !o->b3a2) {
            const size_t B = (size_t)o->max_batch;
            uint4** const outs[4] = {&o->b3a2, &o->b3a3, &o->b3a4, &o->b3f1};
            for (int q = 0; q < 4; ++q)
                if (int rc = o->alloc(outs[q], B * L[q].pixels() * (L[q].N / 32 * 12))) return rc;
            size_t part = (size_t)std::max(o->fc1_b3_ksplit() * L[3].N, o->fc2_b3_ksplit() * L[4].N) * B;
            for (int q = 0; q < 3; ++q)
                if (const int k = o->conv_b3_ksplit(L[q].pixels()); k > 1) part = std::max(part, (size_t)k * B * L[q].pixels() * C);
            if (int rc = o->alloc(&o->d_part_b3, part)) return rc;
            if (!o->d_zero) { if (int rc = o->alloc(&o->d_zero, 16)) return rc; }
            OZ_HIP(hipMemset(o->d_zero, 0, 256));
        }
        if (int rc = o->ensure_b3a1()) return rc;
        if (int rc = o->build_t2_f32()) return rc;
    } else {
        if (int rc = o->commit_h2()) return rc;
    }
    OZ_HIP(hipDeviceSynchronize());
    if (int rc = eval_cache_clear(o)) return rc;
    o->last_count = 0;
    o->committed = true;
    return OZ_OK;
}

OZ_API int oz_net_predict(oz_net* net, const uint64_t* own, const uint64_t* opp, int count, float* pi, float* v) {
    OZ_REQUIRE(net && own && opp && pi && v, "null argument");
    OZ_REQUIRE(count >= 0 && count <= net->max_batch, "count %d outside [0, max_batch=%d]", count, net->max_batch);
    if (count == 0) return OZ_OK;
    std::lock_guard<std::mutex> lk(net->mu);
    hipSetDevice(net->device);
    const int n2 = net->n * net->n;
    const size_t B = (size_t)net->max_batch;
    if (count <= OZ_PREDICT_DIRECT) {
        if (!net->hp_in) {
            hipError_t e;
            int consts[OZ_PREDICT_DIRECT + 1];
            for (int i = 0; i <= OZ_PREDICT_DIRECT; ++i) consts[i] = i;
            if ((e = hipHostMalloc((void**)&net->hp_in, 8 * 2 * OZ_PREDICT_DIRECT, hipHostMallocDefault)) != hipSuccess ||
                (e = hipHostMalloc((void**)&net->hp_out, 4 * OZ_PREDICT_DIRECT * 65, hipHostMallocDefault)) != hipSuccess ||
                (e = hipMalloc((void**)&net->d_counts, sizeof consts)) != hipSuccess ||
                (e = hipMemcpy(net->d_counts, consts, sizeof consts, hipMemcpyHostToDevice)) != hipSuccess) {
                if (net->hp_in) hipHostFree(net->hp_in);
                if (net->hp_out) hipHostFree(net->hp_out);
                if (net->d_counts) hipFree(net->d_counts);
                net->hp_in = nullptr; net->hp_out = nullptr; net->d_counts = nullptr;
                oz_set_error("pinned staging allocation failed: %s", hipGetErrorString(e));
                return OZ_ERR_HIP;
            }
        }
        memcpy(net->hp_in, own, 8ull * count);
        memcpy(net->hp_in + OZ_PREDICT_DIRECT, opp, 8ull * count);
        float* h_pi = net->hp_out;
        float* h_v = net->hp_out + (size_t)OZ_PREDICT_DIRECT * 64;
        if (int rc = net->forward_device(net->hp_in, net->hp_in + OZ_PREDICT_DIRECT, net->d_counts + count, count, h_pi, h_v, 0)) return rc;
        int flag = 0;
        const int* fd = net->flag_device();
        if (fd) OZ_HIP(hipMemcpyAsync(&flag, fd, sizeof(int), hipMemcpyDeviceToHost, 0));
        hipError_t e = hipStreamSynchronize(0);
        if (e != hipSuccess) { oz_set_error("forward failed: %s", hipGetErrorString(e)); return OZ_ERR_HIP; }
        memcpy(pi, h_pi, 4ull * count * n2);
        memcpy(v, h_v, 4ull * count);
        return flag ? net->check() : OZ_OK;
    }
    if (!net->p_in) {
        hipError_t e;
        if ((e = hipMalloc((void**)&net->p_in, 8 * (2 * B + 1))) != hipSuccess || (e = hipMalloc((void**)&net->p_out, 4 * B * (n2 + 1))) != hipSuccess) {
            hipFree(net->p_in); hipFree(net->p_out);
            net->p_in = nullptr; net->p_out = nullptr;
            oz_set_error("hipMalloc failed: %s", hipGetErrorString(e));
            return OZ_ERR_HIP;
        }
        net->h_in.resize(2 * B + 1);
        net->h_out.resize(B * (n2 + 1) + 1);
    }
    memcpy(net->h_in.data(), own, 8ull * count);
    memcpy(net->h_in.data() + count, opp, 8ull * count);
    net->h_in[2 * count] = (uint64_t)(uint32_t)count;
    OZ_HIP(hipMemcpyAsync(net->p_in, net->h_in.data(), 8ull * (2 * count + 1), hipMemcpyHostToDevice, 0));
    float* d_pi = net->p_out;
    float* d_v = net->p_out + (size_t)count * n2;
    if (int rc = net->forward_device(net->p_in, net->p_in + count, reinterpret_cast<const int*>(net->p_in + 2 * count), count, d_pi, d_v, 0)) return rc;
    OZ_HIP(hipMemcpyAsync(net->h_out.data(), net->p_out, 4ull * count * (n2 + 1), hipMemcpyDeviceToHost, 0));
    int flag = 0;
    const int* fd = net->flag_device();
    if (fd) OZ_HIP(hipMemcpyAsync(&flag, fd, sizeof(int), hipMemcpyDeviceToHost, 0));
    hipError_t e = hipStreamSynchronize(0);
    if (e != hipSuccess) { oz_set_error("forward failed: %s", hipGetErrorString(e)); return OZ_ERR_HIP; }
    memcpy(pi, net->h_out.data(), 4ull * count * n2);
    memcpy(v, net->h_out.data() + (size_t)count * n2, 4ull * count);
    return flag ? net->check() : OZ_OK;
}

OZ_API int oz_net_predict_boards(oz_net* net, const uint8_t* boards, int count, float* pi, float* v) {
    OZ_REQUIRE(net && boards && pi && v, "null argument");
    OZ_REQUIRE(count >= 0 && count <= net->max_batch, "count %d outside [0, max_batch=%d]", count, net->max_batch);
    const int n = net->n;
    std::vector<uint64_t> own((size_t)count), opp((size_t)count);
    for (int b = 0; b < count; ++b) {
        const uint8_t* p = boards + (size_t)b * n * n * 2;
        uint64_t o = 0, q = 0;
        for (int r = 0; r < n; ++r)
            for (int c = 0; c < n; ++c) {
                const uint8_t* cell = p + (size_t)(r * n + c) * 2;
                OZ_REQUIRE(!(cell[0] && cell[1]), "board %d: square (%d, %d) holds a disc in both channels", b, r, c);
                if (cell[0]) o |= 1ull << (r * 8 + c);
                if (cell[1]) q |= 1ull << (r * 8 + c);
            }
        own[b] = o; opp[b] = q;
    }
    return oz_net_predict(net, own.data(), opp.data(), count, pi, v);
}

__global__ void k_fill_boards(uint64_t* own, uint64_t* opp, int count, uint64_t valid) {
    const int i = blockIdx.x * blockDim.x + threadIdx.x;
    if (i >= count) return;
    const uint64_t a = oz_sm64(0x1234 + i), b = oz_sm64(0x9876 + 7ull * i), e = oz_sm64(0x5555 + 3ull * i);
    own[i] = a & ~b & e & valid;
    opp[i] = b & ~a & e & valid;
}

OZ_API int oz_net_time_forward(oz_net* net, int count, int iters, float* ms_avg) {
    OZ_REQUIRE(net && ms_avg, "null argument");
    OZ_REQUIRE(count > 0 && count <= net->max_batch && iters > 0, "bad count / iters");
    std::lock_guard<std::mutex> lk(net->mu);
    hipSetDevice(net->device);
    const int n2 = net->n * net->n;
    uint64_t *d_own, *d_opp; int* d_count; float *d_pi, *d_v;
    OZ_HIP(hipMalloc((void**)&d_own, 8ull * count)); OZ_HIP(hipMalloc((void**)&d_opp, 8ull * count));
    OZ_HIP(hipMalloc((void**)&d_count, 4)); OZ_HIP(hipMalloc((void**)&d_pi, 4ull * count * n2)); OZ_HIP(hipMalloc((void**)&d_v, 4ull * count));
    hipLaunchKernelGGL(k_fill_boards, dim3((count + 255) / 256), dim3(256), 0, 0, d_own, d_opp, count, oz_valid_mask(net->n));
    hipMemcpy(d_count, &count, 4, hipMemcpyHostToDevice);
    hipEvent_t e0, e1;
    hipEventCreate(&e0); hipEventCreate(&e1);
    int rc = net->forward_device(d_own, d_opp, d_count, count, d_pi, d_v, 0);
    hipEventRecord(e0, 0);
    for (int i = 0; i < iters && !rc; ++i) rc = net->forward_device(d_own, d_opp, d_count, count, d_pi, d_v, 0);
    hipEventRecord(e1, 0);
    hipError_t e = hipEventSynchronize(e1);
    float ms = 0;
    hipEventElapsedTime(&ms, e0, e1);
    *ms_avg = ms / iters;
    hipEventDestroy(e0); hipEventDestroy(e1);
    hipFree(d_own); hipFree(d_opp); hipFree(d_count); hipFree(d_pi); hipFree(d_v);
    if (rc) return rc;
    OZ_HIP(e);
    return OZ_OK;
}

__global__ __launch_bounds__(256) void k_selftest_b3_split(const float* __restrict__ x, long long count, float* __restrict__ planes, float* __restrict__ sum) {
    const long long i = (long long)blockIdx.x * blockDim.x + threadIdx.x;
    if (i >= count) return;
    __bf16 b1, b2, b3;
    b3_split(x[i], b1, b2, b3);
    const float f1 = (float)b1, f2 = (float)b2, f3 = (float)b3;
    if (planes) { planes[3 * i] = f1; planes[3 * i + 1] = f2; planes[3 * i + 2] = f3; }
    sum[i] = (f1 + f2) + f3;
}
OZ_API int oz_selftest_b3_split(const float* x, int64_t count, float* planes, float* sum) {
    OZ_REQUIRE(x && sum && count > 0 && count <= (1ll << 28), "oz_selftest_b3_split: null argument or count outside (0, 2^28]");
    float *d_x = nullptr, *d_p = nullptr, *d_s = nullptr;
    hipError_t e = hipMalloc((void**)&d_x, sizeof(float) * (size_t)count);
    if (e == hipSuccess) e = hipMalloc((void**)&d_s, sizeof(float) * (size_t)count);
    if (e == hipSuccess && planes) e = hipMalloc((void**)&d_p, sizeof(float) * 3 * (size_t)count);
    if (e == hipSuccess) e = hipMemcpy(d_x, x, sizeof(float) * (size_t)count, hipMemcpyHostToDevice);
    if (e == hipSuccess) {
        hipLaunchKernelGGL(k_selftest_b3_split, dim3((unsigned)((count + 255) / 256)), dim3(256), 0, 0, d_x, (long long)count, d_p, d_s);
        e = hipGetLastError();
    }
    if (e == hipSuccess) e = hipMemcpy(sum, d_s, sizeof(float) * (size_t)count, hipMemcpyDeviceToHost);
    if (e == hipSuccess && planes) e = hipMemcpy(planes, d_p, sizeof(float) * 3 * (size_t)count, hipMemcpyDeviceToHost);
    if (d_x) hipFree(d_x);
    if (d_s) hipFree(d_s);
    if (d_p) hipFree(d_p);
    OZ_HIP(e);
    return OZ_OK;
}

OZ_API int oz_net_set_precision(oz_net* net, int mode) {
    OnnNet* o = as_onn(net);
    OZ_REQUIRE(o, "not an OthelloNN network");
    OZ_REQUIRE(mode == 0 || mode == 1 || mode == 2, "precision must be 0 (f32), 1 (f16x2) or 2 (bf16x3)");
    OZ_REQUIRE(mode == 0 || o->C % 256 == 0, "precision f16x2 / bf16x3 needs channels %% 256 == 0 (got %d)", o->C);
    OZ_REQUIRE(mode != 1 || o->C <= 2048, "precision f16x2 supports at most 2048 channels (got %d): use precision f32", o->C);
    std::lock_guard<std::mutex> lk(o->mu);
    if (o->precision != mode) { o->precision = mode; o->committed = false; }
    return OZ_OK;
}
OZ_API int oz_net_get_precision(const oz_net* net) {
    const OnnNet* o = as_onn(const_cast<oz_net*>(net));
    return o ? o->precision : 0;
}
OZ_API int oz_net_check(oz_net* net) {
    OZ_REQUIRE(net, "null net");
    std::lock_guard<std::mutex> lk(net->mu);
    hipSetDevice(net->device);
    return net->check();
}

OZ_API int oz_net_profile(oz_net* net, int enable) {
    OnnNet* o = as_onn(net);
    OZ_REQUIRE(o, "not an OthelloNN network");
    OZ_REQUIRE(enable >= 0 && enable <= 2, "profile mode must be 0 (off), 1 (dominant launch) or 2 (every kernel)");
    std::lock_guard<std::mutex> lk(o->mu);
    o->profile = enable;
    return OZ_OK;
}

OZ_API int oz_net_set_tables(oz_net* net, int mode) {
    OnnNet* o = as_onn(net);
    OZ_REQUIRE(o, "not an OthelloNN network");
    OZ_REQUIRE(mode >= -1 && mode <= 2, "tables mode must be -1 (default), 0 (none), 1 (conv1) or 2 (conv1 + conv2)");
    std::lock_guard<std::mutex> lk(o->mu);
    if (o->tables_mode != mode) {
        hipSetDevice(o->device);
        OZ_HIP(hipDeviceSynchronize());
        if (int rc = eval_cache_clear(o)) return rc;
    }
    o->tables_mode = mode;
    if (o->committed) { hipSetDevice(o->device); return o->ensure_b3a1(); }
    return OZ_OK;
}

OZ_API int oz_net_set_option(oz_net* net, int option, int value) {
    OnnNet* o = as_onn(net);
    OZ_REQUIRE(o, "not an OthelloNN network");
    OZ_REQUIRE(option == OZ_NET_OPT_SIMPLE_LOOP || option == OZ_NET_OPT_ACT_TARGET_LOG2 || option == OZ_NET_OPT_LOW_GUARD_LOG2 ||
               option == OZ_NET_OPT_SELF_CHECK || option == OZ_NET_OPT_W_TARGET_LOG2 || option == OZ_NET_OPT_F32_STD_TILE ||
               option == OZ_NET_OPT_LATENCY_SPLITS || option == OZ_NET_OPT_CONV3_TILE || option == OZ_NET_OPT_LOW_LOOP_PHASES || option == OZ_NET_OPT_B3_TILE, "unknown network option %d", option);
    std::lock_guard<std::mutex> lk(o->mu);
    if (option == OZ_NET_OPT_SIMPLE_LOOP) o->simple_loop = value != 0;
    else if (option == OZ_NET_OPT_B3_TILE) {
        OZ_REQUIRE(value == 0 || value == 128 || value == 256, "OZ_NET_OPT_B3_TILE must be 0, 128 or 256 (got %d)", value);
        o->b3_tile = value;
    }
    else if (option == OZ_NET_OPT_LOW_LOOP_PHASES) {
        OZ_REQUIRE(value == 1 || value == 2, "OZ_NET_OPT_LOW_LOOP_PHASES must be 1 or 2 (got %d)", value);
        o->low_loop_phases = value;
    }
    else if (option == OZ_NET_OPT_F32_STD_TILE) o->f32_std_tile = value != 0;
    else if (option == OZ_NET_OPT_CONV3_TILE) {
        OZ_REQUIRE(value == 0 || value == 128 || value == 192 || value == 256, "OZ_NET_OPT_CONV3_TILE must be 0, 128, 192 or 256 (got %d)", value);
        o->conv3_tile = value;
    }
    else if (option == OZ_NET_OPT_LATENCY_SPLITS) { if (o->latency_splits != (value != 0)) { o->latency_splits = value != 0; o->committed = false; } }
    else if (option == OZ_NET_OPT_W_TARGET_LOG2) {
        OZ_REQUIRE(value >= -12 && value <= 15, "OZ_NET_OPT_W_TARGET_LOG2 must be in [-12, 15] (got %d)", value);
        if (o->w_target_log2 != value) { o->w_target_log2 = value; o->committed = false; }
    } else if (option == OZ_NET_OPT_SELF_CHECK) {
        OZ_REQUIRE(value >= 0 && value <= 2, "OZ_NET_OPT_SELF_CHECK must be 0 (off), 1 (enforce) or 2 (measure only); got %d", value);
        if (o->self_check != value) { o->self_check = value; o->committed = false; }
    } else if (option == OZ_NET_OPT_ACT_TARGET_LOG2) {
        OZ_REQUIRE(value >= -12 && value <= 20, "OZ_NET_OPT_ACT_TARGET_LOG2 must be in [-12, 20] (got %d)", value);
        if (o->act_target_log2 != value) { o->act_target_log2 = value; o->committed = false; }
    } else {
        OZ_REQUIRE(value <= 15, "OZ_NET_OPT_LOW_GUARD_LOG2 must be <= 15 (got %d)", value);
        if (o->low_guard_log2 != value) { o->low_guard_log2 = value; o->committed = false; }
    }
    return OZ_OK;
}

OZ_API int oz_net_self_check(oz_net* net, double* max_dpi, double* max_dv, int* positions) {
    OnnNet* o = as_onn(net);
    OZ_REQUIRE(o, "not an OthelloNN network");
    std::lock_guard<std::mutex> lk(o->mu);
    if (max_dpi) *max_dpi = o->sc_dpi;
    if (max_dv) *max_dv = o->sc_dv;
    if (positions) *positions = o->sc_positions;
    return OZ_OK;
}

OZ_API int oz_net_get_scaling(oz_net* net, int which, int32_t* out, int64_t nelem) {
    OnnNet* o = as_onn(net);
    OZ_REQUIRE(o && out, "not an OthelloNN network / null argument");
    OZ_REQUIRE(which >= 0 && which <= 9, "oz_net_get_scaling: which must be 0 .. 9 (got %d)", which);
    std::lock_guard<std::mutex> lk(o->mu);
    OZ_REQUIRE(o->precision == 1 && o->committed, "oz_net_get_scaling: the network is not committed in precision f16x2");
    const std::vector<int>& e = which < 5 ? o->aexp[which] : o->wexp[which - 5];
    OZ_REQUIRE(nelem == (int64_t)e.size(), "oz_net_get_scaling(%d): %lld elements expected, got %lld", which, (long long)e.size(), (long long)nelem);
    for (size_t i = 0; i < e.size(); ++i) out[i] = e[i];
    return OZ_OK;
}

OZ_API int oz_net_get_info(oz_net* net, int what, int* value) {
    OnnNet* o = as_onn(net);
    OZ_REQUIRE(o && value, "not an OthelloNN network / null argument");
    std::lock_guard<std::mutex> lk(o->mu);
    for (int l = 1; l <= 5; ++l) {
        const OnnNet::LayerPlan& p = o->plan[l];
        if (what == OZ_NET_INFO_LAYER_TILE_ROWS(l)) { *value = p.tile_rows; return OZ_OK; }
        if (what == OZ_NET_INFO_LAYER_KSLICES(l)) { *value = p.ksplit; return OZ_OK; }
        if (what == OZ_NET_INFO_LAYER_KERNEL(l)) { *value = p.kernel; return OZ_OK; }
    }
    OZ_REQUIRE(what == OZ_NET_INFO_CONV3_TILE_ROWS || what == OZ_NET_INFO_SELF_CHECK_GUARD || what == OZ_NET_INFO_ARITHMETIC, "unknown network info %d", what);
    *value = what == OZ_NET_INFO_CONV3_TILE_ROWS ? o->last_conv3_rows : what == OZ_NET_INFO_ARITHMETIC ? (o->precision == 2 && !o->use_b3() ? 0 : o->precision) : o->sc_guard;
    return OZ_OK;
}

OZ_API int oz_net_get_activation(oz_net* net, int layer, int64_t first_row, int64_t rows, double* out) {
    OnnNet* o = as_onn(net);
    OZ_REQUIRE(o && out, "oz_net_get_activation: not an OthelloNN network / null argument");
    OZ_REQUIRE(layer >= 0 && layer <= 5, "oz_net_get_activation: layer must be 0 .. 5 (got %d)", layer);
    std::lock_guard<std::mutex> lk(o->mu);
    hipSetDevice(o->device);
    if (!o->committed || o->last_count == 0) { oz_set_error("oz_net_get_activation: no forward since the last oz_net_commit"); return OZ_ERR_STATE; }
    const int P = layer == 0 ? o->n * o->n : o->layers()[layer - 1].pixels(), N = layer == 0 ? o->C : o->layers()[layer - 1].N;
    const long long total = (long long)o->last_count * P;
    OZ_REQUIRE(first_row >= 0 && rows > 0 && first_row <= total && rows <= total - first_row,
               "oz_net_get_activation: rows [%lld, %lld) outside the %lld rows of the last forward", (long long)first_row, (long long)(first_row + rows), total);
    const OnnNet::ActView v = o->view[layer];
    if (v.fmt < 0 || (v.fmt != 3 && !v.p)) {
        oz_set_error("oz_net_get_activation: the last forward did not materialise the output of layer %d (conv1 folded into a pattern table: "
                     "oz_net_set_tables(0) runs it as a kernel)", layer);
        return OZ_ERR_STATE;
    }
    double* d_out = nullptr;
    OZ_HIP(hipMalloc((void**)&d_out, sizeof(double) * (size_t)rows * N));
    const dim3 grid8((unsigned)((rows * (N / 8) + 255) / 256)), grid1((unsigned)((rows * N + 255) / 256));
    if (v.fmt == 0) hipLaunchKernelGGL(k_act_rows_f64<0>, grid8, dim3(256), 0, 0, v.p, (const int*)nullptr, (long long)first_row, (long long)rows, N, d_out);
    else if (v.fmt == 1) hipLaunchKernelGGL(k_act_rows_f64<1>, grid8, dim3(256), 0, 0, v.p, v.aexp, (long long)first_row, (long long)rows, N, d_out);
    else if (v.fmt == 2) hipLaunchKernelGGL(k_act_rows_f64<2>, grid8, dim3(256), 0, 0, v.p, (const int*)nullptr, (long long)first_row, (long long)rows, N, d_out);
    else hipLaunchKernelGGL(k_deferred_rows_f64, grid1, dim3(256), 0, 0, o->last_defer, (long long)first_row, (long long)rows, N, d_out);
    hipError_t e = hipGetLastError();
    if (e == hipSuccess) e = hipMemcpy(out, d_out, sizeof(double) * (size_t)rows * N, hipMemcpyDeviceToHost);
    hipFree(d_out);
    OZ_HIP(e);
    return OZ_OK;
}

OZ_API int oz_net_profiled_layer(oz_net* net, int* layer) {
    OnnNet* o = as_onn(net);
    OZ_REQUIRE(o && layer, "not an OthelloNN network / null argument");
    std::lock_guard<std::mutex> lk(o->mu);
    *layer = o->profiled_layer;
    return OZ_OK;
}

OZ_API int oz_net_profile_read(oz_net* net, double* conv2_ms_total, int64_t* conv2_launches) {
    OnnNet* o = as_onn(net);
    OZ_REQUIRE(o, "not an OthelloNN network");
    std::lock_guard<std::mutex> lk(o->mu);
    hipSetDevice(o->device);
    if (int rc = o->collect_profile()) return rc;
    const int slot = o->profiled_layer - 1;
    if (conv2_ms_total) *conv2_ms_total = o->timer.ms[slot];
    if (conv2_launches) *conv2_launches = o->timer.count[slot];
    return OZ_OK;
}

OZ_API int oz_net_profile_kernels(oz_net* net, double* ms_total, int64_t* launches, int reset) {
    OnnNet* o = as_onn(net);
    OZ_REQUIRE(o, "not an OthelloNN network");
    std::lock_guard<std::mutex> lk(o->mu);
    hipSetDevice(o->device);
    if (int rc = o->collect_profile()) return rc;
    for (int i = 0; i < OZ_NET_KERNELS; ++i) {
        if (ms_total) ms_total[i] = o->timer.ms[i];
        if (launches) launches[i] = o->timer.count[i];
    }
    if (reset) o->timer.reset();
    return OZ_OK;
}
```

othellozero_amd/csrc/oz_net_b3.h:

```cpp
#pragma once

#define B3_BK 32
#define B3_BM 128
#define B3_BN 256
#define B3_NT 512
#define B3_ROWB 192
#define B3_BLK (16 * B3_ROWB)
#define B3_TILEA (B3_BM * B3_ROWB)
#define B3_TILEB (B3_BN * B3_ROWB)
#define B3_BUF (B3_TILEA + B3_TILEB)
#define B3_LDS (2 * B3_BUF)
#define B3_SLICE (32 * 384)

struct B3Geom {
    int Hin, Hout, pad, Cin, taps;
    int N, K;
    int out_b3;
    int relu;
    int ksplit;
    long long slab;
};


__global__ __launch_bounds__(256) void k_f32_to_b3(const float* __restrict__ x, const int* __restrict__ d_count, int P, int C, uint4* __restrict__ out) {
    const int cg = C >> 3;
    const long long idx = (long long)blockIdx.x * blockDim.x + threadIdx.x;
    const long long row = idx / cg;
    if (row >= (long long)(*d_count) * P) return;
    const int c8 = (int)(idx % cg) * 8;
    const f32x4 lo = *reinterpret_cast<const f32x4*>(x + (size_t)row * C + c8), hi = *reinterpret_cast<const f32x4*>(x + (size_t)row * C + c8 + 4);
    const float v[8] = {lo[0], lo[1], lo[2], lo[3], hi[0], hi[1], hi[2], hi[3]};
    b3_store8(out, row, C, c8, v);
}

__global__ __launch_bounds__(256) void k_splitk_reduce_b3(const float* __restrict__ part, long long slab, int ksplit, int N, int P,
                                                          const int* __restrict__ d_count, const float* __restrict__ scale,
                                                          const float* __restrict__ shift, uint4* __restrict__ out) {
    const int ng = N >> 3;
    const long long idx = (long long)blockIdx.x * blockDim.x + threadIdx.x;
    const long long m = idx / ng;
    if (m >= (long long)(*d_count) * P) return;
    const int c8 = (int)(idx % ng) * 8;
    const float* p = part + (size_t)m * N + c8;
    f32x4 lo = *reinterpret_cast<const f32x4*>(p), hi = *reinterpret_cast<const f32x4*>(p + 4);
    for (int s = 1; s < ksplit; ++s) {
        lo += *reinterpret_cast<const f32x4*>(p + (size_t)s * slab);
        hi += *reinterpret_cast<const f32x4*>(p + (size_t)s * slab + 4);
    }
    float v[8];
#pragma unroll
    for (int j = 0; j < 8; ++j) v[j] = fmaxf(fmaf(j < 4 ? lo[j] : hi[j - 4], scale[c8 + j], shift[c8 + j]), 0.f);
    b3_store8(out, m, N, c8, v);
}

__global__ __launch_bounds__(256) void k_w_to_b3(const float* __restrict__ src, int K, int N, int taps, uint4* __restrict__ out) {
    const long long idx = (long long)blockIdx.x * blockDim.x + threadIdx.x;
    const int c = (int)(idx % N);
    const int grp = (int)(idx / N);
    if (grp >= (K >> 3)) return;
    const int Cin = K / taps;
    float v[8];
#pragma unroll
    for (int j = 0; j < 8; ++j) {
        const int kp = grp * 8 + j, tile = kp >> 5, c32 = kp & 31, slice = tile / taps, tap = tile - slice * taps;
        const int k = tap * Cin + slice * 32 + c32;
        v[j] = src[(size_t)k * N + c];
    }
    b3_store8(out, c, K, grp * 8, v);
}

template <int TAG = 0>
__global__ __launch_bounds__(B3_NT, 2) void k_gemm_b3(const uint4* __restrict__ in, const uint4* __restrict__ Wb,
                                                      const float* __restrict__ scale, const float* __restrict__ shift,
                                                      void* __restrict__ out, const int* __restrict__ d_count, B3Geom g,
                                                      int num_mt, const uint4* __restrict__ zero_line) {
    extern __shared__ __attribute__((aligned(16))) unsigned char smem[];
    constexpr int BM = B3_BM, BN = B3_BN, RI = 4, RJ = 4;
    const int nnt = g.N / BN, per_mt = nnt * g.ksplit;
    const int id = blockIdx.x, xcd = id & 7, jb = id >> 3;
    int mt, nt, ks;
    if (num_mt < 8) {
        mt = jb % num_mt;
        const int q = (jb / num_mt) * 8 + xcd;
        if (q >= per_mt) return;
        nt = q / g.ksplit; ks = q - nt * g.ksplit;
    } else {
        const int rem = jb % per_mt;
        mt = (jb / per_mt) * 8 + xcd; nt = rem / g.ksplit; ks = rem - nt * g.ksplit;
    }
    const int P = g.Hout * g.Hout;
    const long long M = (long long)(*d_count) * P;
    if (mt >= num_mt || (long long)mt * BM >= M) return;

    const int tid = threadIdx.x, lane = tid & 63;
    const int wave = __builtin_amdgcn_readfirstlane(tid >> 6);
    const int wm = wave >> 2, wn = wave & 3;
    const int rowq = g.Cin / 32 * 12;
    const int wrowq = g.K / 32 * 12;

    long long aidx[3];
    unsigned amask[3];
    unsigned bidx_e[3], bidx_l[3];
    const int eb = (wave >> 1) * 4 + (wave & 1), lb = eb + 2;
#pragma unroll
    for (int i = 0; i < 3; ++i) {
        const int cidx = 64 * i + lane, r = cidx / 12, pos = cidx - 12 * r, pl = pos >> 2, kgs = (pos & 3) ^ ((4 - (r >> 2)) & 3);
        const int src_chunk = pl * 4 + kgs;
        const long long m = (long long)mt * BM + wave * 16 + r;
        aidx[i] = 0; amask[i] = 0;
        if (m < M) {
            const int b = (int)(m / P), pix = (int)(m % P), oy = pix / g.Hout, ox = pix % g.Hout;
            aidx[i] = (((long long)b * g.Hin + (oy - g.pad)) * g.Hin + (ox - g.pad)) * rowq + src_chunk;
            unsigned mk = 0;
            for (int t = 0; t < g.taps; ++t) {
                const int iy = oy - g.pad + t / 3, ix = ox - g.pad + t % 3;
                if (iy >= 0 && iy < g.Hin && ix >= 0 && ix < g.Hin) mk |= 1u << t;
            }
            amask[i] = mk;
        }
        bidx_e[i] = (unsigned)(nt * BN + eb * 16 + r) * (unsigned)wrowq + (unsigned)src_chunk;
        bidx_l[i] = (unsigned)(nt * BN + lb * 16 + r) * (unsigned)wrowq + (unsigned)src_chunk;
    }
    const uint4* zsrc = zero_line + (lane & 7);
    const int nk_all = g.K / B3_BK, kbeg = (int)((long long)nk_all * ks / g.ksplit), nk = (int)((long long)nk_all * (ks + 1) / g.ksplit);

    auto put_a = [&](int slice, int tap, unsigned char* la) {
        const int dy = (tap * 11) >> 5, dx = tap - 3 * dy;
        const long long toff = ((long long)dy * g.Hin + dx) * rowq + slice * 12;
#pragma unroll
        for (int i = 0; i < 3; ++i) {
            const uint4* ga = ((amask[i] >> tap) & 1) ? in + (aidx[i] + toff) : zsrc;
            __builtin_amdgcn_global_load_lds((oz_gptr)ga, (oz_lptr)(la + wave * B3_BLK + i * 1024), 16, 0, 0);
        }
    };
    auto put_be = [&](int ktc, unsigned char* lbp) {
#pragma unroll
        for (int i = 0; i < 3; ++i)
            __builtin_amdgcn_global_load_lds((oz_gptr)(Wb + bidx_e[i] + ktc * 12), (oz_lptr)(lbp + eb * B3_BLK + i * 1024), 16, 0, 0);
    };
    auto put_bl = [&](int ktc, unsigned char* lbp) {
#pragma unroll
        for (int i = 0; i < 3; ++i)
            __builtin_amdgcn_global_load_lds((oz_gptr)(Wb + bidx_l[i] + ktc * 12), (oz_lptr)(lbp + lb * B3_BLK + i * 1024), 16, 0, 0);
    };

    f32x4 acc[RI][RJ];
#pragma unroll
    for (int i = 0; i < RI; ++i)
#pragma unroll
        for (int j = 0; j < RJ; ++j)
#pragma unroll
            for (int r = 0; r < 4; ++r) acc[i][j][r] = 0.f;

    const int r16 = lane & 15, kg = lane >> 4;
    const int lofs = r16 * B3_ROWB + ((kg ^ ((4 - (r16 >> 2)) & 3)) * 16);

    constexpr int KEEP = 9;
    int k1 = kbeg + 1 < nk ? kbeg + 1 : nk - 1, slice1 = k1 / g.taps, tap1 = k1 - slice1 * g.taps;
    int k2 = kbeg + 2 < nk ? kbeg + 2 : nk - 1, slice2 = k2 / g.taps, tap2 = k2 - slice2 * g.taps;
    {
        const int slice0 = kbeg / g.taps, tap0 = kbeg - slice0 * g.taps;
        put_a(slice0, tap0, smem);
        put_be(kbeg, smem + B3_TILEA); put_bl(kbeg, smem + B3_TILEA);
        put_be(k1, smem + B3_BUF + B3_TILEA);
        put_a(slice1, tap1, smem + B3_BUF);
    }
    asm volatile("s_waitcnt vmcnt(6)" ::: "memory");
    __builtin_amdgcn_s_barrier();
    asm volatile("" ::: "memory");
    bf16x8 fa[3][RI], fb[3][RJ];
    {
        const unsigned char* Bt0 = smem + B3_TILEA + wn * 4 * B3_BLK + lofs;
#pragma unroll
        for (int j = 0; j < 2; ++j)
#pragma unroll
            for (int p = 0; p < 3; ++p) fb[p][j] = *reinterpret_cast<const bf16x8*>(Bt0 + j * B3_BLK + p * 64);
        asm volatile("s_waitcnt lgkmcnt(0)" ::: "memory");
    }
    __builtin_amdgcn_s_barrier();
    asm volatile("" ::: "memory");
    if (wm == 1) __builtin_amdgcn_s_barrier();
    for (int kt = kbeg; kt < nk; ++kt) {
        const int buf = (kt - kbeg) & 1;
        unsigned char* la_cur = smem + (size_t)buf * B3_BUF;
        unsigned char* la_oth = smem + (size_t)(buf ^ 1) * B3_BUF;
        const unsigned char* At = la_cur + wm * 4 * B3_BLK + lofs;
        const unsigned char* Bt = la_cur + B3_TILEA + wn * 4 * B3_BLK + lofs;
        const unsigned char* Btn = la_oth + B3_TILEA + wn * 4 * B3_BLK + lofs;
        auto ldb = [&](int half, const unsigned char* base) {
#pragma unroll
            for (int j = 0; j < 2; ++j)
#pragma unroll
                for (int p = 0; p < 3; ++p) fb[p][half * 2 + j] = *reinterpret_cast<const bf16x8*>(base + (half * 2 + j) * B3_BLK + p * 64);
        };
        auto l_end = [&]() {
            asm volatile("s_waitcnt vmcnt(%0)" :: "n"(KEEP) : "memory");
            asm volatile("s_waitcnt lgkmcnt(0)" ::: "memory");
            __builtin_amdgcn_s_barrier();
            asm volatile("" ::: "memory");
            __builtin_amdgcn_sched_barrier(0);
        };
        auto mma = [&](int nh) {
#pragma unroll
            for (int q = 0; q < 6; ++q) {
                constexpr int PA[6] = {2, 0, 1, 1, 0, 0}, PB[6] = {0, 2, 1, 0, 1, 0};
#pragma unroll
                for (int i = 0; i < RI; ++i)
#pragma unroll
                    for (int j = 0; j < 2; ++j) {
                        f32x4& c = acc[i][nh * 2 + j];
                        c = __builtin_amdgcn_mfma_f32_16x16x32_bf16(fa[PA[q]][i], fb[PB[q]][nh * 2 + j], c, 0, 0, 0);
                    }
            }
            __builtin_amdgcn_sched_barrier(0);
        };
        auto m_end = [&]() {
            asm volatile("" ::: "memory");
            __builtin_amdgcn_s_barrier();
            asm volatile("" ::: "memory");
            __builtin_amdgcn_sched_barrier(0);
        };
#pragma unroll
        for (int i = 0; i < RI; ++i)
#pragma unroll
            for (int p = 0; p < 3; ++p) fa[p][i] = *reinterpret_cast<const bf16x8*>(At + i * B3_BLK + p * 64);
        put_bl(k1, la_oth + B3_TILEA); put_be(k2, la_cur + B3_TILEA);
        l_end(); mma(0); m_end();
        ldb(1, Bt); ldb(0, Btn);
        put_a(slice2, tap2, la_cur);
        l_end(); mma(1); m_end();
        k1 = k2; slice1 = slice2; tap1 = tap2;
        if (k2 + 1 < nk) { ++k2; if (++tap2 == g.taps) { tap2 = 0; ++slice2; } }
    }
    if (wm == 0) __builtin_amdgcn_s_barrier();
    asm volatile("s_waitcnt vmcnt(0)" ::: "memory");
    __builtin_amdgcn_s_barrier();
    asm volatile("" ::: "memory");

    if (g.ksplit > 1) {
        float* o = reinterpret_cast<float*>(out) + (size_t)ks * g.slab;
#pragma unroll
        for (int j = 0; j < RJ; ++j) {
            const int col = nt * BN + wn * 64 + j * 16 + r16;
#pragma unroll
            for (int i = 0; i < RI; ++i)
#pragma unroll
                for (int r = 0; r < 4; ++r) {
                    const long long m = (long long)mt * BM + wm * 64 + i * 16 + kg * 4 + r;
                    if (m < M) o[(size_t)m * g.N + col] = acc[i][j][r];
                }
        }
        return;
    }
    if (!g.out_b3) {
        float* o = reinterpret_cast<float*>(out);
#pragma unroll
        for (int j = 0; j < RJ; ++j) {
            const int col = nt * BN + wn * 64 + j * 16 + r16;
            const float sc = scale[col], sh = shift[col];
#pragma unroll
            for (int i = 0; i < RI; ++i)
#pragma unroll
                for (int r = 0; r < 4; ++r) {
                    const long long m = (long long)mt * BM + wm * 64 + i * 16 + kg * 4 + r;
                    float v = fmaf(acc[i][j][r], sc, sh);
                    if (g.relu) v = fmaxf(v, 0.f);
                    if (m < M) o[(size_t)m * g.N + col] = v;
                }
        }
        return;
    }
    __bf16* slice = reinterpret_cast<__bf16*>(smem + wave * B3_SLICE);
    uint4* o = reinterpret_cast<uint4*>(out);
    const int nq = g.N / 32 * 12;
#pragma unroll
    for (int hh = 0; hh < 2; ++hh) {
#pragma unroll
        for (int ii = 0; ii < 2; ++ii) {
            const int i = hh * 2 + ii;
#pragma unroll
            for (int j = 0; j < RJ; ++j) {
                const int lc = j * 16 + r16;
                const int col = nt * BN + wn * 64 + lc;
                const float sc = scale[col], sh = shift[col];
#pragma unroll
                for (int r = 0; r < 4; ++r) {
                    const int lr = ii * 16 + kg * 4 + r;
                    float v = fmaf(acc[i][j][r], sc, sh);
                    if (g.relu) v = fmaxf(v, 0.f);
                    __bf16 b1, b2, b3;
                    b3_split(v, b1, b2, b3);
                    __bf16* p = slice + lr * 192 + (lc >> 5) * 96 + (lc & 31);
                    p[0] = b1; p[32] = b2; p[64] = b3;
                }
            }
        }
        __builtin_amdgcn_s_waitcnt(0xC07F);
        __builtin_amdgcn_wave_barrier();
#pragma unroll
        for (int c = 0; c < 12; ++c) {
            const int q = c * 64 + lane, lr = q / 24, cq = q - lr * 24;
            const long long m = (long long)mt * BM + wm * 64 + hh * 32 + lr;
            const uint4 val = *reinterpret_cast<const uint4*>(reinterpret_cast<const unsigned char*>(slice) + lr * 384 + cq * 16);
            if (m < M) o[(size_t)m * nq + ((nt * BN + wn * 64) >> 5) * 12 + cq] = val;
        }
        __builtin_amdgcn_s_waitcnt(0xC07F);
        __builtin_amdgcn_wave_barrier();
    }
}

#define B3B_BM 256
#define B3B_BN 256
#define B3B_REG (8 * B3_BLK)
#define B3B_LDS (5 * B3B_REG)
template <int TAG = 0>
__global__ __launch_bounds__(B3_NT, 2) void k_gemm_b3_big(const uint4* __restrict__ in, const uint4* __restrict__ Wb,
                                                          const float* __restrict__ scale, const float* __restrict__ shift,
                                                          void* __restrict__ out, const int* __restrict__ d_count, B3Geom g,
                                                          int num_mt, const uint4* __restrict__ zero_line) {
    extern __shared__ __attribute__((aligned(16))) unsigned char smem[];
    constexpr int BM = B3B_BM, BN = B3B_BN, HA = 4, RJ = 4;
    unsigned char* const rA0 = smem;
    unsigned char* const rA1 = smem + B3B_REG;
    unsigned char* const rB0 = smem + 2 * B3B_REG;
    unsigned char* const rB1 = smem + 4 * B3B_REG;
    const int nnt = g.N / BN, per_mt = nnt * g.ksplit;
    const int id = blockIdx.x, xcd = id & 7, jb = id >> 3;
    int mt, nt, ks;
    if (num_mt < 8) {
        mt = jb % num_mt;
        const int q = (jb / num_mt) * 8 + xcd;
        if (q >= per_mt) return;
        nt = q / g.ksplit; ks = q - nt * g.ksplit;
    } else {
        const int rem = jb % per_mt;
        mt = (jb / per_mt) * 8 + xcd; nt = rem / g.ksplit; ks = rem - nt * g.ksplit;
    }
    const int P = g.Hout * g.Hout;
    const long long M = (long long)(*d_count) * P;
    if (mt >= num_mt || (long long)mt * BM >= M) return;

    const int tid = threadIdx.x, lane = tid & 63;
    const int wave = __builtin_amdgcn_readfirstlane(tid >> 6);
    const int wm = wave >> 2, wn = wave & 3;
    const int rowq = g.Cin / 32 * 12, wrowq = g.K / 32 * 12;

    unsigned aoff[2][3], boff[3];
#pragma unroll
    for (int i = 0; i < 3; ++i) {
        const int cidx = 64 * i + lane, r = cidx / 12, pos = cidx - 12 * r, src_chunk = (pos >> 2) * 4 + ((pos & 3) ^ ((4 - (r >> 2)) & 3));
#pragma unroll
        for (int h = 0; h < 2; ++h) {
            const long long m = (long long)mt * BM + (wave >> 2) * 128 + h * 64 + (wave & 3) * 16 + r;
            aoff[h][i] = ~0u;
            if (m < M) {
                const int b = (int)(m / P), pix = (int)(m % P), oy = pix / g.Hout, ox = pix % g.Hout;
                aoff[h][i] = (unsigned)((((long long)b * g.Hin + oy) * g.Hin + ox) * rowq + src_chunk);
            }
        }
        boff[i] = (unsigned)(nt * BN + (wave >> 1) * 64 + (wave & 1) * 16 + r) * (unsigned)wrowq + (unsigned)src_chunk;
    }
    const unsigned bhalf = 32u * (unsigned)wrowq;
    const uint4* zsrc = zero_line + (lane & 7);
    const int nk_all = g.K / B3_BK, kbeg = (int)((long long)nk_all * ks / g.ksplit), nk = (int)((long long)nk_all * (ks + 1) / g.ksplit);

    auto put_a = [&](int h, int slice, int tap, unsigned char* reg) {
        const int dy = (tap * 11) >> 5, dx = tap - 3 * dy;
        const unsigned toff = (unsigned)((dy * g.Hin + dx) * rowq + slice * 12);
#pragma unroll
        for (int i = 0; i < 3; ++i) {
            const uint4* ga = aoff[h][i] != ~0u ? in + (aoff[h][i] + toff) : zsrc;
            __builtin_amdgcn_global_load_lds((oz_gptr)ga, (oz_lptr)(reg + wave * B3_BLK + i * 1024), 16, 0, 0);
        }
    };
    auto put_b = [&](int h, int ktc, unsigned char* reg) {
#pragma unroll
        for (int i = 0; i < 3; ++i)
            __builtin_amdgcn_global_load_lds((oz_gptr)(Wb + (boff[i] + (h ? bhalf : 0u) + (unsigned)ktc * 12u)), (oz_lptr)(reg + wave * B3_BLK + i * 1024), 16, 0, 0);
    };

    f32x4 acc[2 * HA][RJ];
#pragma unroll
    for (int i = 0; i < 2 * HA; ++i)
#pragma unroll
        for (int j = 0; j < RJ; ++j)
#pragma unroll
            for (int r = 0; r < 4; ++r) acc[i][j][r] = 0.f;

    const int r16 = lane & 15, kg = lane >> 4;
    const int lofs = r16 * B3_ROWB + ((kg ^ ((4 - (r16 >> 2)) & 3)) * 16);
    const unsigned char* const At0 = rA0 + wm * HA * B3_BLK + lofs;
    const unsigned char* const At1 = rA1 + wm * HA * B3_BLK + lofs;
    const unsigned char* const Bt1 = rB1 + wn * 2 * B3_BLK + lofs;

    constexpr int KEEP = 6;
    int ktn = kbeg + 1 < nk ? kbeg + 1 : nk - 1, slice_n = ktn / g.taps, tap_n = ktn - slice_n * g.taps;
    {
        const int slice0 = kbeg / g.taps, tap0 = kbeg - slice0 * g.taps;
        put_b(0, kbeg, rB0); put_a(0, slice0, tap0, rA0); put_b(1, kbeg, rB1); put_a(1, slice0, tap0, rA1);
    }
    asm volatile("s_waitcnt vmcnt(%0)" :: "n"(KEEP) : "memory");
    __builtin_amdgcn_s_barrier();
    asm volatile("" ::: "memory");
    if (wm == 1) __builtin_amdgcn_s_barrier();
    bf16x8 fa[3][HA], fb[3][2];
    for (int kt = kbeg; kt < nk; ++kt) {
        const int par = (kt - kbeg) & 1;
        unsigned char* const rB0cur = rB0 + par * B3B_REG;
        unsigned char* const rB0nxt = rB0 + (par ^ 1) * B3B_REG;
        const unsigned char* const Bt0 = rB0cur + wn * 2 * B3_BLK + lofs;
        auto lda = [&](const unsigned char* base) {
#pragma unroll
            for (int i = 0; i < HA; ++i)
#pragma unroll
                for (int p = 0; p < 3; ++p) fa[p][i] = *reinterpret_cast<const bf16x8*>(base + i * B3_BLK + p * 64);
        };
        auto ldb = [&](const unsigned char* base) {
#pragma unroll
            for (int j = 0; j < 2; ++j)
#pragma unroll
                for (int p = 0; p < 3; ++p) fb[p][j] = *reinterpret_cast<const bf16x8*>(base + j * B3_BLK + p * 64);
        };
        auto l_end = [&]() {
            asm volatile("s_waitcnt vmcnt(%0)" :: "n"(KEEP) : "memory");
            asm volatile("s_waitcnt lgkmcnt(0)" ::: "memory");
            __builtin_amdgcn_s_barrier();
            asm volatile("" ::: "memory");
            __builtin_amdgcn_sched_barrier(0);
        };
        auto mma = [&](int mh, int nh) {
#pragma unroll
            for (int q = 0; q < 6; ++q) {
                constexpr int PA[6] = {2, 0, 1, 1, 0, 0}, PB[6] = {0, 2, 1, 0, 1, 0};
#pragma unroll
                for (int i = 0; i < HA; ++i)
#pragma unroll
                    for (int j = 0; j < 2; ++j) {
                        f32x4& c = acc[mh * HA + i][nh * 2 + j];
                        c = __builtin_amdgcn_mfma_f32_16x16x32_bf16(fa[PA[q]][i], fb[PB[q]][j], c, 0, 0, 0);
                    }
            }
            __builtin_amdgcn_sched_barrier(0);
        };
        auto m_end = [&]() {
            asm volatile("" ::: "memory");
            __builtin_amdgcn_s_barrier();
            asm volatile("" ::: "memory");
            __builtin_amdgcn_sched_barrier(0);
        };
        lda(At0); ldb(Bt0); put_b(0, ktn, rB0nxt); l_end(); mma(0, 0); m_end();
        ldb(Bt1); put_a(0, slice_n, tap_n, rA0); l_end(); mma(0, 1); m_end();
        lda(At1); put_b(1, ktn, rB1); l_end(); mma(1, 1); m_end();
        ldb(Bt0); put_a(1, slice_n, tap_n, rA1); l_end(); mma(1, 0); m_end();
        if (ktn + 1 < nk) { ++ktn; if (++tap_n == g.taps) { tap_n = 0; ++slice_n; } }
    }
    if (wm == 0) __builtin_amdgcn_s_barrier();
    asm volatile("s_waitcnt vmcnt(0)" ::: "memory");
    __builtin_amdgcn_s_barrier();
    asm volatile("" ::: "memory");

    if (g.ksplit > 1) {
        float* o = reinterpret_cast<float*>(out) + (size_t)ks * g.slab;
#pragma unroll
        for (int j = 0; j < RJ; ++j) {
            const int col = nt * BN + wn * 64 + j * 16 + r16;
#pragma unroll
            for (int i = 0; i < 2 * HA; ++i)
#pragma unroll
                for (int r = 0; r < 4; ++r) {
                    const long long m = (long long)mt * BM + wm * 128 + i * 16 + kg * 4 + r;
                    if (m < M) o[(size_t)m * g.N + col] = acc[i][j][r];
                }
        }
        return;
    }
    if (!g.out_b3) {
        float* o = reinterpret_cast<float*>(out);
#pragma unroll
        for (int j = 0; j < RJ; ++j) {
            const int col = nt * BN + wn * 64 + j * 16 + r16;
            const float sc = scale[col], sh = shift[col];
#pragma unroll
            for (int i = 0; i < 2 * HA; ++i)
#pragma unroll
                for (int r = 0; r < 4; ++r) {
                    const long long m = (long long)mt * BM + wm * 128 + i * 16 + kg * 4 + r;
                    float v = fmaf(acc[i][j][r], sc, sh);
                    if (g.relu) v = fmaxf(v, 0.f);
                    if (m < M) o[(size_t)m * g.N + col] = v;
                }
        }
        return;
    }
    __bf16* slice = reinterpret_cast<__bf16*>(smem + wave * B3_SLICE);
    uint4* o = reinterpret_cast<uint4*>(out);
    const int nq = g.N / 32 * 12;
#pragma unroll
    for (int hh = 0; hh < HA; ++hh) {
#pragma unroll
        for (int ii = 0; ii < 2; ++ii) {
            const int i = hh * 2 + ii;
#pragma unroll
            for (int j = 0; j < RJ; ++j) {
                const int lc = j * 16 + r16;
                const int col = nt * BN + wn * 64 + lc;
                const float sc = scale[col], sh = shift[col];
#pragma unroll
                for (int r = 0; r < 4; ++r) {
                    const int lr = ii * 16 + kg * 4 + r;
                    float v = fmaf(acc[i][j][r], sc, sh);
                    if (g.relu) v = fmaxf(v, 0.f);
                    __bf16 b1, b2, b3;
                    b3_split(v, b1, b2, b3);
                    __bf16* p = slice + lr * 192 + (lc >> 5) * 96 + (lc & 31);
                    p[0] = b1; p[32] = b2; p[64] = b3;
                }
            }
        }
        __builtin_amdgcn_s_waitcnt(0xC07F);
        __builtin_amdgcn_wave_barrier();
#pragma unroll
        for (int c = 0; c < 12; ++c) {
            const int q = c * 64 + lane, lr = q / 24, cq = q - lr * 24;
            const long long m = (long long)mt * BM + wm * 128 + hh * 32 + lr;
            const uint4 val = *reinterpret_cast<const uint4*>(reinterpret_cast<const unsigned char*>(slice) + lr * 384 + cq * 16);
            if (m < M) o[(size_t)m * nq + ((nt * BN + wn * 64) >> 5) * 12 + cq] = val;
        }
        __builtin_amdgcn_s_waitcnt(0xC07F);
        __builtin_amdgcn_wave_barrier();
    }
}
```

Baseline: 947,400.

## Specialize b3 GEMM for unpadded layers and replace integer divisions with magic multiplies

New measurement: 959,300 (median of 6 runs). No clear change (+1.3%).

```diff
diff --git a/include/othellozero_amd.h b/include/othellozero_amd.h
--- a/include/othellozero_amd.h
+++ b/include/othellozero_amd.h
@@ -339,6 +339,7 @@
                       float* fchain);
 int oz_selftest_mfma_rate(int kind, double target_ms, double* tflops, double* clock_ghz, double* ms_measured);
 int oz_selftest_b3_split(const float* x, int64_t count, float* planes, float* sum);
+int oz_selftest_b3_row_map(uint32_t m0, int64_t count, int Hout, uint32_t* out, int* ok);
 
 #ifdef __cplusplus
 }
diff --git a/othellozero_amd/_lib.py b/othellozero_amd/_lib.py
--- a/othellozero_amd/_lib.py
+++ b/othellozero_amd/_lib.py
@@ -168,6 +168,7 @@
     "oz_selftest_arith": [_f64p, _f64p, C.c_int, _f64p, _f64p, _f32p, _f32p],
     "oz_selftest_mfma_rate": [C.c_int, C.c_double, _f64p, _f64p, _f64p],
     "oz_selftest_b3_split": [_f32p, C.c_int64, _f32p, _f32p],
+    "oz_selftest_b3_row_map": [C.c_uint32, C.c_int64, C.c_int, C.POINTER(C.c_uint32), _i32p],
     "oz_trainer_arena_size": [C.c_int, C.c_int, C.c_int, C.POINTER(C.c_int64)],
     "oz_trainer_create": [C.POINTER(_vp), C.c_int, C.c_int, C.c_int, C.c_int, C.c_float, C.c_float, C.c_float, C.c_float,
                           C.c_uint64, _vp],
diff --git a/othellozero_amd/csrc/oz_common.h b/othellozero_amd/csrc/oz_common.h
--- a/othellozero_amd/csrc/oz_common.h
+++ b/othellozero_amd/csrc/oz_common.h
@@ -171,9 +171,12 @@
     h1 = (_Float16)x;
     h2 = (_Float16)(x - (float)h1);
 }
+#define B3_SPLIT_CLAMP_FROM_BITS 0x7F7F8000u
+template <bool CLAMP = true>
 __device__ __forceinline__ void b3_split(float x, __bf16& b1, __bf16& b2, __bf16& b3) {
     b1 = (__bf16)x;
-    if (__builtin_isinf((float)b1) && !__builtin_isinf(x)) b1 = __builtin_bit_cast(__bf16, (unsigned short)(x < 0.f ? 0xFF7Fu : 0x7F7Fu));
+    if constexpr (CLAMP)
+        if (__builtin_isinf((float)b1) && !__builtin_isinf(x)) b1 = __builtin_bit_cast(__bf16, (unsigned short)(x < 0.f ? 0xFF7Fu : 0x7F7Fu));
     const float r1 = x - (float)b1;
     b2 = (__bf16)r1;
     b3 = (__bf16)(r1 - (float)b2);
@@ -218,6 +221,15 @@
 __device__ __forceinline__ void b3_store8(uint4* out, size_t row, int K, int k, const float (&v)[8]) {
     oz_split8_store<3, NT>(out + b3_group_chunk(row, K, k), 4, v);
 }
+OZ_HD unsigned oz_div_magic(unsigned d) { return d > 1 ? (unsigned)(((1ull << 32) + d - 1) / d) : 0u; }
+OZ_HD bool oz_div_magic_ok(unsigned long long max_m, unsigned d) { return max_m * d <= (1ull << 32); }
+OZ_HD unsigned oz_div_u32(unsigned m, unsigned mul) { return mul ? (unsigned)(((unsigned long long)m * mul) >> 32) : m; }
+OZ_HD void oz_row_map(unsigned m, unsigned P, unsigned Hout, unsigned mulP, unsigned mulH, unsigned& b, unsigned& oy, unsigned& ox) {
+    b = oz_div_u32(m, mulP);
+    const unsigned pix = m - b * P;
+    oy = oz_div_u32(pix, mulH);
+    ox = pix - oy * Hout;
+}
 template <int PLANES>
 __device__ __forceinline__ void oz_split8_load(const uint4* src, size_t pstride, double (&v)[8]) {
     static_assert(PLANES == 2 || PLANES == 3, "f16x2 or bf16x3");
diff --git a/othellozero_amd/csrc/oz_net.hip b/othellozero_amd/csrc/oz_net.hip
--- a/othellozero_amd/csrc/oz_net.hip
+++ b/othellozero_amd/csrc/oz_net.hip
@@ -427,14 +427,26 @@
     g.out_b3 = packed; g.relu = relu; g.ksplit = ksplit; g.slab = slab;
     const int P = L.pixels(), N = L.N, BM = big ? B3B_BM : B3_BM;
     const int num_mt = (int)(((long long)max_count * P + BM - 1) / BM);
+    g.mulP = oz_div_magic((unsigned)P); g.mulH = oz_div_magic((unsigned)L.Hout);
+    g.mulNumMt = oz_div_magic((unsigned)num_mt); g.mulPerMt = oz_div_magic((unsigned)((N / B3_BN) * ksplit));
+    g.mulKs = oz_div_magic((unsigned)ksplit); g.mulTaps = oz_div_magic((unsigned)L.taps);
+    const long long in_chunks = (long long)max_count * L.Hin * L.Hin * (L.Cin / 32 * 12);
+    OZ_REQUIRE((long long)num_mt * BM < (1ll << 31) && oz_div_magic_ok((unsigned long long)num_mt * BM, (unsigned)P) && in_chunks < 0xFFFFFFFFll &&
+               num_mt > 0 && ksplit > 0 && (long long)gemm_grid(num_mt, (N / B3_BN) * ksplit) * std::max(num_mt, (N / B3_BN) * ksplit) < (1ll << 31) &&
+               (long long)(L.K() / B3_BK) * (ksplit + 1) * std::max(ksplit, L.taps) < (1ll << 31),
+               "gemm_b3: %d positions of %d x %d x %d do not fit the kernels' 32-bit row and input offsets", max_count, L.Hin, L.Hin, L.Cin);
+    OZ_REQUIRE(!big || L.pad == 0, "gemm_b3: the 256 x 256 tile has no padding (pad=%d)", L.pad);
     const dim3 grid(gemm_grid(num_mt, (N / B3_BN) * ksplit));
     void* dst = ksplit > 1 ? (void*)slabs : out;
     if (big) {
         if (int rc = set_max_lds_once<k_gemm_b3_big<TAG>>(B3B_LDS)) return rc;
         hipLaunchKernelGGL((k_gemm_b3_big<TAG>), grid, dim3(B3_NT), B3B_LDS, s, in, W, scale, shift, dst, d_count, g, num_mt, zero_line);
+    } else if (L.pad != 0) {
+        if (int rc = set_max_lds_once<k_gemm_b3<TAG, true>>(B3_LDS)) return rc;
+        hipLaunchKernelGGL((k_gemm_b3<TAG, true>), grid, dim3(B3_NT), B3_LDS, s, in, W, scale, shift, dst, d_count, g, num_mt, zero_line);
     } else {
-        if (int rc = set_max_lds_once<k_gemm_b3<TAG>>(B3_LDS)) return rc;
-        hipLaunchKernelGGL((k_gemm_b3<TAG>), grid, dim3(B3_NT), B3_LDS, s, in, W, scale, shift, dst, d_count, g, num_mt, zero_line);
+        if (int rc = set_max_lds_once<k_gemm_b3<TAG, false>>(B3_LDS)) return rc;
+        hipLaunchKernelGGL((k_gemm_b3<TAG, false>), grid, dim3(B3_NT), B3_LDS, s, in, W, scale, shift, dst, d_count, g, num_mt, zero_line);
     }
     if (ksplit > 1 && packed) {
         const long long threads = (long long)max_count * P * (N / 8);
@@ -1796,6 +1808,29 @@
     return OZ_OK;
 }
 
+OZ_API int oz_selftest_b3_row_map(uint32_t m0, int64_t count, int Hout, uint32_t* out, int* ok) {
+    OZ_REQUIRE(out && count > 0 && Hout > 0 && Hout <= 1024 && (unsigned long long)m0 + (unsigned long long)count <= (1ull << 32),
+               "oz_selftest_b3_row_map: null argument, Hout outside [1, 1024] or rows beyond 2^32");
+    const unsigned P = (unsigned)(Hout * Hout), mulP = oz_div_magic(P), mulH = oz_div_magic((unsigned)Hout);
+    if (ok) *ok = oz_div_magic_ok((unsigned long long)m0 + (unsigned long long)count, P) ? 1 : 0;
+    for (int64_t i = 0; i < count; ++i) oz_row_map(m0 + (uint32_t)i, P, (unsigned)Hout, mulP, mulH, out[3 * i], out[3 * i + 1], out[3 * i + 2]);
+    return OZ_OK;
+}
+
+#ifdef OZ_B3_STAMPS
+OZ_API int oz_b3_stamps_read(unsigned long long* dst, int clear) {
+    OZ_REQUIRE(dst, "oz_b3_stamps_read: null argument");
+    OZ_HIP(hipDeviceSynchronize());
+    OZ_HIP(hipMemcpyFromSymbol(dst, HIP_SYMBOL(oz_b3_stamp_buf), sizeof(oz_b3_stamp_buf)));
+    if (clear) {
+        void* p = nullptr;
+        OZ_HIP(hipGetSymbolAddress(&p, HIP_SYMBOL(oz_b3_stamp_buf)));
+        OZ_HIP(hipMemset(p, 0, sizeof(oz_b3_stamp_buf)));
+    }
+    return OZ_OK;
+}
+#endif
+
 OZ_API int oz_net_set_precision(oz_net* net, int mode) {
     OnnNet* o = as_onn(net);
     OZ_REQUIRE(o, "not an OthelloNN network");
diff --git a/othellozero_amd/csrc/oz_net_b3.h b/othellozero_amd/csrc/oz_net_b3.h
--- a/othellozero_amd/csrc/oz_net_b3.h
+++ b/othellozero_amd/csrc/oz_net_b3.h
@@ -19,8 +19,39 @@
     int relu;
     int ksplit;
     long long slab;
+    unsigned mulP, mulH;
+    unsigned mulNumMt, mulPerMt, mulKs, mulTaps;
 };
 
+
+#ifdef OZ_B3_STAMPS
+#define B3_STAMP_BLOCKS 4096
+#define B3_STAMP_SLOTS 5
+__device__ unsigned long long oz_b3_stamp_buf[8][B3_STAMP_BLOCKS][2 * B3_STAMP_SLOTS];
+#define B3_STAMP_DECL unsigned long long st_c[B3_STAMP_SLOTS] = {}, st_r[B3_STAMP_SLOTS] = {};
+#define B3_STAMP(i)                                                                                                                       \
+    do {                                                                                                                                  \
+        __builtin_amdgcn_sched_barrier(0);                                                                                                \
+        if (__builtin_amdgcn_readfirstlane(threadIdx.x >> 6) == 0)                                                                        \
+            asm volatile("s_memtime %0\n\ts_memrealtime %1\n\ts_waitcnt lgkmcnt(0)" : "=&s"(st_c[i]), "=&s"(st_r[i]) :: "memory");        \
+        __builtin_amdgcn_sched_barrier(0);                                                                                                \
+    } while (0)
+#define B3_STAMP_OUT(TAG)                                                                                                                 \
+    do {                                                                                                                                  \
+        B3_STAMP(3);                                                                                                                      \
+        asm volatile("s_waitcnt vmcnt(0)" ::: "memory");                                                                                  \
+        B3_STAMP(4);                                                                                                                      \
+        if (threadIdx.x == 0 && blockIdx.x < B3_STAMP_BLOCKS)                                                                             \
+            _Pragma("unroll") for (int s_ = 0; s_ < B3_STAMP_SLOTS; ++s_) {                                                               \
+                oz_b3_stamp_buf[(TAG) & 7][blockIdx.x][s_] = st_c[s_];                                                                    \
+                oz_b3_stamp_buf[(TAG) & 7][blockIdx.x][B3_STAMP_SLOTS + s_] = st_r[s_];                                                   \
+            }                                                                                                                             \
+    } while (0)
+#else
+#define B3_STAMP_DECL
+#define B3_STAMP(i)
+#define B3_STAMP_OUT(TAG)
+#endif
 
 __global__ __launch_bounds__(256) void k_f32_to_b3(const float* __restrict__ x, const int* __restrict__ d_count, int P, int C, uint4* __restrict__ out) {
     const int cg = C >> 3;
@@ -69,28 +100,32 @@
     b3_store8(out, c, K, grp * 8, v);
 }
 
-template <int TAG = 0>
+template <int TAG = 0, bool PAD = true>
 __global__ __launch_bounds__(B3_NT, 2) void k_gemm_b3(const uint4* __restrict__ in, const uint4* __restrict__ Wb,
                                                       const float* __restrict__ scale, const float* __restrict__ shift,
                                                       void* __restrict__ out, const int* __restrict__ d_count, B3Geom g,
                                                       int num_mt, const uint4* __restrict__ zero_line) {
     extern __shared__ __attribute__((aligned(16))) unsigned char smem[];
+    B3_STAMP_DECL
+    B3_STAMP(0);
     constexpr int BM = B3_BM, BN = B3_BN, RI = 4, RJ = 4;
     const int nnt = g.N / BN, per_mt = nnt * g.ksplit;
     const int id = blockIdx.x, xcd = id & 7, jb = id >> 3;
     int mt, nt, ks;
     if (num_mt < 8) {
-        mt = jb % num_mt;
-        const int q = (jb / num_mt) * 8 + xcd;
+        const int jq = (int)oz_div_u32((unsigned)jb, g.mulNumMt);
+        mt = jb - jq * num_mt;
+        const int q = jq * 8 + xcd;
         if (q >= per_mt) return;
-        nt = q / g.ksplit; ks = q - nt * g.ksplit;
+        nt = (int)oz_div_u32((unsigned)q, g.mulKs); ks = q - nt * g.ksplit;
     } else {
-        const int rem = jb % per_mt;
-        mt = (jb / per_mt) * 8 + xcd; nt = rem / g.ksplit; ks = rem - nt * g.ksplit;
-    }
-    const int P = g.Hout * g.Hout;
-    const long long M = (long long)(*d_count) * P;
-    if (mt >= num_mt || (long long)mt * BM >= M) return;
+        const int jq = (int)oz_div_u32((unsigned)jb, g.mulPerMt), rem = jb - jq * per_mt;
+        mt = jq * 8 + xcd; nt = (int)oz_div_u32((unsigned)rem, g.mulKs); ks = rem - nt * g.ksplit;
+    }
+    const unsigned P = (unsigned)(g.Hout * g.Hout);
+    const unsigned M = (unsigned)(*d_count) * P;
+    if (mt >= num_mt || (unsigned)mt * BM >= M) return;
+    const bool full = (unsigned)(mt + 1) * BM <= M;
 
     const int tid = threadIdx.x, lane = tid & 63;
     const int wave = __builtin_amdgcn_readfirstlane(tid >> 6);
@@ -98,39 +133,35 @@
     const int rowq = g.Cin / 32 * 12;
     const int wrowq = g.K / 32 * 12;
 
-    long long aidx[3];
+    const uint4* aptr[3];
     unsigned amask[3];
     unsigned bidx_e[3], bidx_l[3];
+    int arow[3], achunk[3];
     const int eb = (wave >> 1) * 4 + (wave & 1), lb = eb + 2;
 #pragma unroll
     for (int i = 0; i < 3; ++i) {
         const int cidx = 64 * i + lane, r = cidx / 12, pos = cidx - 12 * r, pl = pos >> 2, kgs = (pos & 3) ^ ((4 - (r >> 2)) & 3);
-        const int src_chunk = pl * 4 + kgs;
-        const long long m = (long long)mt * BM + wave * 16 + r;
-        aidx[i] = 0; amask[i] = 0;
-        if (m < M) {
-            const int b = (int)(m / P), pix = (int)(m % P), oy = pix / g.Hout, ox = pix % g.Hout;
-            aidx[i] = (((long long)b * g.Hin + (oy - g.pad)) * g.Hin + (ox - g.pad)) * rowq + src_chunk;
-            unsigned mk = 0;
-            for (int t = 0; t < g.taps; ++t) {
-                const int iy = oy - g.pad + t / 3, ix = ox - g.pad + t % 3;
-                if (iy >= 0 && iy < g.Hin && ix >= 0 && ix < g.Hin) mk |= 1u << t;
-            }
-            amask[i] = mk;
-        }
-        bidx_e[i] = (unsigned)(nt * BN + eb * 16 + r) * (unsigned)wrowq + (unsigned)src_chunk;
-        bidx_l[i] = (unsigned)(nt * BN + lb * 16 + r) * (unsigned)wrowq + (unsigned)src_chunk;
+        arow[i] = r; achunk[i] = pl * 4 + kgs;
+        bidx_e[i] = (unsigned)(nt * BN + eb * 16 + r) * (unsigned)wrowq + (unsigned)achunk[i];
+        bidx_l[i] = (unsigned)(nt * BN + lb * 16 + r) * (unsigned)wrowq + (unsigned)achunk[i];
     }
     const uint4* zsrc = zero_line + (lane & 7);
-    const int nk_all = g.K / B3_BK, kbeg = (int)((long long)nk_all * ks / g.ksplit), nk = (int)((long long)nk_all * (ks + 1) / g.ksplit);
+    const int nk_all = g.K / B3_BK, kbeg = (int)oz_div_u32((unsigned)(nk_all * ks), g.mulKs), nk = (int)oz_div_u32((unsigned)(nk_all * (ks + 1)), g.mulKs);
 
     auto put_a = [&](int slice, int tap, unsigned char* la) {
         const int dy = (tap * 11) >> 5, dx = tap - 3 * dy;
-        const long long toff = ((long long)dy * g.Hin + dx) * rowq + slice * 12;
-#pragma unroll
-        for (int i = 0; i < 3; ++i) {
-            const uint4* ga = ((amask[i] >> tap) & 1) ? in + (aidx[i] + toff) : zsrc;
-            __builtin_amdgcn_global_load_lds((oz_gptr)ga, (oz_lptr)(la + wave * B3_BLK + i * 1024), 16, 0, 0);
+        if constexpr (PAD) {
+            const long long toff = ((long long)dy * g.Hin + dx) * rowq + slice * 12;
+#pragma unroll
+            for (int i = 0; i < 3; ++i) {
+                const uint4* ga = ((amask[i] >> tap) & 1) ? aptr[i] + toff : zsrc;
+                __builtin_amdgcn_global_load_lds((oz_gptr)ga, (oz_lptr)(la + wave * B3_BLK + i * 1024), 16, 0, 0);
+            }
+        } else {
+            const unsigned toff = (unsigned)((dy * g.Hin + dx) * rowq + slice * 12);
+#pragma unroll
+            for (int i = 0; i < 3; ++i)
+                __builtin_amdgcn_global_load_lds((oz_gptr)(aptr[i] + (toff & amask[i])), (oz_lptr)(la + wave * B3_BLK + i * 1024), 16, 0, 0);
         }
     };
     auto put_be = [&](int ktc, unsigned char* lbp) {
@@ -144,6 +175,31 @@
             __builtin_amdgcn_global_load_lds((oz_gptr)(Wb + bidx_l[i] + ktc * 12), (oz_lptr)(lbp + lb * B3_BLK + i * 1024), 16, 0, 0);
     };
 
+    constexpr int KEEP = 9;
+    int k1 = kbeg + 1 < nk ? kbeg + 1 : nk - 1, slice1 = (int)oz_div_u32((unsigned)k1, g.mulTaps), tap1 = k1 - slice1 * g.taps;
+    int k2 = kbeg + 2 < nk ? kbeg + 2 : nk - 1, slice2 = (int)oz_div_u32((unsigned)k2, g.mulTaps), tap2 = k2 - slice2 * g.taps;
+    put_be(kbeg, smem + B3_TILEA); put_bl(kbeg, smem + B3_TILEA);
+    __builtin_amdgcn_sched_barrier(0);
+#pragma unroll
+    for (int i = 0; i < 3; ++i) {
+        const unsigned m = (unsigned)mt * BM + wave * 16 + arow[i];
+        aptr[i] = zsrc; amask[i] = 0;
+        if (m < M) {
+            unsigned b, oy, ox;
+            oz_row_map(m, P, (unsigned)g.Hout, g.mulP, g.mulH, b, oy, ox);
+            const int iy0 = (int)oy - g.pad, ix0 = (int)ox - g.pad;
+            aptr[i] = in + ((((long long)b * g.Hin + iy0) * g.Hin + ix0) * rowq + achunk[i]);
+            if constexpr (PAD) {
+                unsigned mk = 0;
+                for (int t = 0; t < g.taps; ++t) {
+                    const int iy = iy0 + t / 3, ix = ix0 + t % 3;
+                    if (iy >= 0 && iy < g.Hin && ix >= 0 && ix < g.Hin) mk |= 1u << t;
+                }
+                amask[i] = mk;
+            } else amask[i] = ~0u;
+        }
+    }
+
     f32x4 acc[RI][RJ];
 #pragma unroll
     for (int i = 0; i < RI; ++i)
@@ -155,13 +211,9 @@
     const int r16 = lane & 15, kg = lane >> 4;
     const int lofs = r16 * B3_ROWB + ((kg ^ ((4 - (r16 >> 2)) & 3)) * 16);
 
-    constexpr int KEEP = 9;
-    int k1 = kbeg + 1 < nk ? kbeg + 1 : nk - 1, slice1 = k1 / g.taps, tap1 = k1 - slice1 * g.taps;
-    int k2 = kbeg + 2 < nk ? kbeg + 2 : nk - 1, slice2 = k2 / g.taps, tap2 = k2 - slice2 * g.taps;
     {
-        const int slice0 = kbeg / g.taps, tap0 = kbeg - slice0 * g.taps;
+        const int slice0 = (int)oz_div_u32((unsigned)kbeg, g.mulTaps), tap0 = kbeg - slice0 * g.taps;
         put_a(slice0, tap0, smem);
-        put_be(kbeg, smem + B3_TILEA); put_bl(kbeg, smem + B3_TILEA);
         put_be(k1, smem + B3_BUF + B3_TILEA);
         put_a(slice1, tap1, smem + B3_BUF);
     }
@@ -179,6 +231,7 @@
     }
     __builtin_amdgcn_s_barrier();
     asm volatile("" ::: "memory");
+    B3_STAMP(1);
     if (wm == 1) __builtin_amdgcn_s_barrier();
     for (int kt = kbeg; kt < nk; ++kt) {
         const int buf = (kt - kbeg) & 1;
@@ -232,81 +285,93 @@
         k1 = k2; slice1 = slice2; tap1 = tap2;
         if (k2 + 1 < nk) { ++k2; if (++tap2 == g.taps) { tap2 = 0; ++slice2; } }
     }
+    B3_STAMP(2);
     if (wm == 0) __builtin_amdgcn_s_barrier();
     asm volatile("s_waitcnt vmcnt(0)" ::: "memory");
     __builtin_amdgcn_s_barrier();
     asm volatile("" ::: "memory");
 
-    if (g.ksplit > 1) {
-        float* o = reinterpret_cast<float*>(out) + (size_t)ks * g.slab;
-#pragma unroll
-        for (int j = 0; j < RJ; ++j) {
-            const int col = nt * BN + wn * 64 + j * 16 + r16;
-#pragma unroll
-            for (int i = 0; i < RI; ++i)
-#pragma unroll
-                for (int r = 0; r < 4; ++r) {
-                    const long long m = (long long)mt * BM + wm * 64 + i * 16 + kg * 4 + r;
-                    if (m < M) o[(size_t)m * g.N + col] = acc[i][j][r];
+    auto epilogue = [&](auto full_c) {
+        constexpr bool FULL = decltype(full_c)::value;
+        if (g.ksplit > 1) {
+            float* o = reinterpret_cast<float*>(out) + (size_t)ks * g.slab;
+#pragma unroll
+            for (int j = 0; j < RJ; ++j) {
+                const int col = nt * BN + wn * 64 + j * 16 + r16;
+#pragma unroll
+                for (int i = 0; i < RI; ++i)
+#pragma unroll
+                    for (int r = 0; r < 4; ++r) {
+                        const unsigned m = (unsigned)mt * BM + wm * 64 + i * 16 + kg * 4 + r;
+                        if (FULL || m < M) o[(size_t)m * g.N + col] = acc[i][j][r];
+                    }
+            }
+            return;
+        }
+        if (!g.out_b3) {
+            float* o = reinterpret_cast<float*>(out);
+#pragma unroll
+            for (int j = 0; j < RJ; ++j) {
+                const int col = nt * BN + wn * 64 + j * 16 + r16;
+                const float sc = scale[col], sh = shift[col];
+#pragma unroll
+                for (int i = 0; i < RI; ++i)
+#pragma unroll
+                    for (int r = 0; r < 4; ++r) {
+                        const unsigned m = (unsigned)mt * BM + wm * 64 + i * 16 + kg * 4 + r;
+                        float v = fmaf(acc[i][j][r], sc, sh);
+                        if (g.relu) v = fmaxf(v, 0.f);
+                        if (FULL || m < M) o[(size_t)m * g.N + col] = v;
+                    }
+            }
+            return;
+        }
+        __bf16* slice = reinterpret_cast<__bf16*>(smem + wave * B3_SLICE);
+        uint4* o = reinterpret_cast<uint4*>(out);
+        const int nq = g.N / 32 * 12;
+#pragma unroll
+        for (int hh = 0; hh < 2; ++hh) {
+            float big = 0.f;
+            auto split_pass = [&](auto clamp_c) {
+#pragma unroll
+                for (int ii = 0; ii < 2; ++ii) {
+                    const int i = hh * 2 + ii;
+#pragma unroll
+                    for (int j = 0; j < RJ; ++j) {
+                        const int lc = j * 16 + r16;
+                        const int col = nt * BN + wn * 64 + lc;
+                        const float sc = scale[col], sh = shift[col];
+#pragma unroll
+                        for (int r = 0; r < 4; ++r) {
+                            const int lr = ii * 16 + kg * 4 + r;
+                            float v = fmaf(acc[i][j][r], sc, sh);
+                            if (g.relu) v = fmaxf(v, 0.f);
+                            big = fmaxf(big, __builtin_fabsf(v));
+                            __bf16 b1, b2, b3;
+                            b3_split<decltype(clamp_c)::value>(v, b1, b2, b3);
+                            __bf16* p = slice + lr * 192 + (lc >> 5) * 96 + (lc & 31);
+                            p[0] = b1; p[32] = b2; p[64] = b3;
+                        }
+                    }
                 }
-        }
-        return;
-    }
-    if (!g.out_b3) {
-        float* o = reinterpret_cast<float*>(out);
-#pragma unroll
-        for (int j = 0; j < RJ; ++j) {
-            const int col = nt * BN + wn * 64 + j * 16 + r16;
-            const float sc = scale[col], sh = shift[col];
-#pragma unroll
-            for (int i = 0; i < RI; ++i)
-#pragma unroll
-                for (int r = 0; r < 4; ++r) {
-                    const long long m = (long long)mt * BM + wm * 64 + i * 16 + kg * 4 + r;
-                    float v = fmaf(acc[i][j][r], sc, sh);
-                    if (g.relu) v = fmaxf(v, 0.f);
-                    if (m < M) o[(size_t)m * g.N + col] = v;
-                }
-        }
-        return;
-    }
-    __bf16* slice = reinterpret_cast<__bf16*>(smem + wave * B3_SLICE);
-    uint4* o = reinterpret_cast<uint4*>(out);
-    const int nq = g.N / 32 * 12;
-#pragma unroll
-    for (int hh = 0; hh < 2; ++hh) {
-#pragma unroll
-        for (int ii = 0; ii < 2; ++ii) {
-            const int i = hh * 2 + ii;
-#pragma unroll
-            for (int j = 0; j < RJ; ++j) {
-                const int lc = j * 16 + r16;
-                const int col = nt * BN + wn * 64 + lc;
-                const float sc = scale[col], sh = shift[col];
-#pragma unroll
-                for (int r = 0; r < 4; ++r) {
-                    const int lr = ii * 16 + kg * 4 + r;
-                    float v = fmaf(acc[i][j][r], sc, sh);
-                    if (g.relu) v = fmaxf(v, 0.f);
-                    __bf16 b1, b2, b3;
-                    b3_split(v, b1, b2, b3);
-                    __bf16* p = slice + lr * 192 + (lc >> 5) * 96 + (lc & 31);
-                    p[0] = b1; p[32] = b2; p[64] = b3;
-                }
-            }
-        }
-        __builtin_amdgcn_s_waitcnt(0xC07F);
-        __builtin_amdgcn_wave_barrier();
-#pragma unroll
-        for (int c = 0; c < 12; ++c) {
-            const int q = c * 64 + lane, lr = q / 24, cq = q - lr * 24;
-            const long long m = (long long)mt * BM + wm * 64 + hh * 32 + lr;
-            const uint4 val = *reinterpret_cast<const uint4*>(reinterpret_cast<const unsigned char*>(slice) + lr * 384 + cq * 16);
-            if (m < M) o[(size_t)m * nq + ((nt * BN + wn * 64) >> 5) * 12 + cq] = val;
-        }
-        __builtin_amdgcn_s_waitcnt(0xC07F);
-        __builtin_amdgcn_wave_barrier();
-    }
+            };
+            split_pass(std::false_type());
+            if (__builtin_amdgcn_ballot_w64(!(big < __builtin_bit_cast(float, B3_SPLIT_CLAMP_FROM_BITS))) != 0) split_pass(std::true_type());
+            __builtin_amdgcn_s_waitcnt(0xC07F);
+            __builtin_amdgcn_wave_barrier();
+#pragma unroll
+            for (int c = 0; c < 12; ++c) {
+                const int q = c * 64 + lane, lr = q / 24, cq = q - lr * 24;
+                const unsigned m = (unsigned)mt * BM + wm * 64 + hh * 32 + lr;
+                const uint4 val = *reinterpret_cast<const uint4*>(reinterpret_cast<const unsigned char*>(slice) + lr * 384 + cq * 16);
+                if (FULL || m < M) o[(size_t)m * nq + ((nt * BN + wn * 64) >> 5) * 12 + cq] = val;
+            }
+            __builtin_amdgcn_s_waitcnt(0xC07F);
+            __builtin_amdgcn_wave_barrier();
+        }
+    };
+    if (full) epilogue(std::true_type()); else epilogue(std::false_type());
+    B3_STAMP_OUT(TAG);
 }
 
 #define B3B_BM 256
@@ -319,6 +384,8 @@
                                                           void* __restrict__ out, const int* __restrict__ d_count, B3Geom g,
                                                           int num_mt, const uint4* __restrict__ zero_line) {
     extern __shared__ __attribute__((aligned(16))) unsigned char smem[];
+    B3_STAMP_DECL
+    B3_STAMP(0);
     constexpr int BM = B3B_BM, BN = B3B_BN, HA = 4, RJ = 4;
     unsigned char* const rA0 = smem;
     unsigned char* const rA1 = smem + B3B_REG;
@@ -328,17 +395,19 @@
     const int id = blockIdx.x, xcd = id & 7, jb = id >> 3;
     int mt, nt, ks;
     if (num_mt < 8) {
-        mt = jb % num_mt;
-        const int q = (jb / num_mt) * 8 + xcd;
+        const int jq = (int)oz_div_u32((unsigned)jb, g.mulNumMt);
+        mt = jb - jq * num_mt;
+        const int q = jq * 8 + xcd;
         if (q >= per_mt) return;
-        nt = q / g.ksplit; ks = q - nt * g.ksplit;
+        nt = (int)oz_div_u32((unsigned)q, g.mulKs); ks = q - nt * g.ksplit;
     } else {
-        const int rem = jb % per_mt;
-        mt = (jb / per_mt) * 8 + xcd; nt = rem / g.ksplit; ks = rem - nt * g.ksplit;
-    }
-    const int P = g.Hout * g.Hout;
-    const long long M = (long long)(*d_count) * P;
-    if (mt >= num_mt || (long long)mt * BM >= M) return;
+        const int jq = (int)oz_div_u32((unsigned)jb, g.mulPerMt), rem = jb - jq * per_mt;
+        mt = jq * 8 + xcd; nt = (int)oz_div_u32((unsigned)rem, g.mulKs); ks = rem - nt * g.ksplit;
+    }
+    const unsigned P = (unsigned)(g.Hout * g.Hout);
+    const unsigned M = (unsigned)(*d_count) * P;
+    if (mt >= num_mt || (unsigned)mt * BM >= M) return;
+    const bool full = (unsigned)(mt + 1) * BM <= M;
 
     const int tid = threadIdx.x, lane = tid & 63;
     const int wave = __builtin_amdgcn_readfirstlane(tid >> 6);
@@ -346,23 +415,16 @@
     const int rowq = g.Cin / 32 * 12, wrowq = g.K / 32 * 12;
 
     unsigned aoff[2][3], boff[3];
+    int arow[3], achunk[3];
 #pragma unroll
     for (int i = 0; i < 3; ++i) {
-        const int cidx = 64 * i + lane, r = cidx / 12, pos = cidx - 12 * r, src_chunk = (pos >> 2) * 4 + ((pos & 3) ^ ((4 - (r >> 2)) & 3));
-#pragma unroll
-        for (int h = 0; h < 2; ++h) {
-            const long long m = (long long)mt * BM + (wave >> 2) * 128 + h * 64 + (wave & 3) * 16 + r;
-            aoff[h][i] = ~0u;
-            if (m < M) {
-                const int b = (int)(m / P), pix = (int)(m % P), oy = pix / g.Hout, ox = pix % g.Hout;
-                aoff[h][i] = (unsigned)((((long long)b * g.Hin + oy) * g.Hin + ox) * rowq + src_chunk);
-            }
-        }
-        boff[i] = (unsigned)(nt * BN + (wave >> 1) * 64 + (wave & 1) * 16 + r) * (unsigned)wrowq + (unsigned)src_chunk;
+        const int cidx = 64 * i + lane, r = cidx / 12, pos = cidx - 12 * r;
+        arow[i] = r; achunk[i] = (pos >> 2) * 4 + ((pos & 3) ^ ((4 - (r >> 2)) & 3));
+        boff[i] = (unsigned)(nt * BN + (wave >> 1) * 64 + (wave & 1) * 16 + r) * (unsigned)wrowq + (unsigned)achunk[i];
     }
     const unsigned bhalf = 32u * (unsigned)wrowq;
     const uint4* zsrc = zero_line + (lane & 7);
-    const int nk_all = g.K / B3_BK, kbeg = (int)((long long)nk_all * ks / g.ksplit), nk = (int)((long long)nk_all * (ks + 1) / g.ksplit);
+    const int nk_all = g.K / B3_BK, kbeg = (int)oz_div_u32((unsigned)(nk_all * ks), g.mulKs), nk = (int)oz_div_u32((unsigned)(nk_all * (ks + 1)), g.mulKs);
 
     auto put_a = [&](int h, int slice, int tap, unsigned char* reg) {
         const int dy = (tap * 11) >> 5, dx = tap - 3 * dy;
@@ -394,14 +456,29 @@
     const unsigned char* const Bt1 = rB1 + wn * 2 * B3_BLK + lofs;
 
     constexpr int KEEP = 6;
-    int ktn = kbeg + 1 < nk ? kbeg + 1 : nk - 1, slice_n = ktn / g.taps, tap_n = ktn - slice_n * g.taps;
+    int ktn = kbeg + 1 < nk ? kbeg + 1 : nk - 1, slice_n = (int)oz_div_u32((unsigned)ktn, g.mulTaps), tap_n = ktn - slice_n * g.taps;
+    put_b(0, kbeg, rB0); put_b(1, kbeg, rB1);
+    __builtin_amdgcn_sched_barrier(0);
+#pragma unroll
+    for (int i = 0; i < 3; ++i)
+#pragma unroll
+        for (int h = 0; h < 2; ++h) {
+            const unsigned m = (unsigned)mt * BM + (wave >> 2) * 128 + h * 64 + (wave & 3) * 16 + arow[i];
+            aoff[h][i] = ~0u;
+            if (m < M) {
+                unsigned b, oy, ox;
+                oz_row_map(m, P, (unsigned)g.Hout, g.mulP, g.mulH, b, oy, ox);
+                aoff[h][i] = ((b * g.Hin + oy) * g.Hin + ox) * rowq + achunk[i];
+            }
+        }
     {
-        const int slice0 = kbeg / g.taps, tap0 = kbeg - slice0 * g.taps;
-        put_b(0, kbeg, rB0); put_a(0, slice0, tap0, rA0); put_b(1, kbeg, rB1); put_a(1, slice0, tap0, rA1);
-    }
-    asm volatile("s_waitcnt vmcnt(%0)" :: "n"(KEEP) : "memory");
+        const int slice0 = (int)oz_div_u32((unsigned)kbeg, g.mulTaps), tap0 = kbeg - slice0 * g.taps;
+        put_a(0, slice0, tap0, rA0); put_a(1, slice0, tap0, rA1);
+    }
+    asm volatile("s_waitcnt vmcnt(3)" ::: "memory");
     __builtin_amdgcn_s_barrier();
     asm volatile("" ::: "memory");
+    B3_STAMP(1);
     if (wm == 1) __builtin_amdgcn_s_barrier();
     bf16x8 fa[3][HA], fb[3][2];
     for (int kt = kbeg; kt < nk; ++kt) {
@@ -454,79 +531,85 @@
         ldb(Bt0); put_a(1, slice_n, tap_n, rA1); l_end(); mma(1, 0); m_end();
         if (ktn + 1 < nk) { ++ktn; if (++tap_n == g.taps) { tap_n = 0; ++slice_n; } }
     }
+    B3_STAMP(2);
     if (wm == 0) __builtin_amdgcn_s_barrier();
     asm volatile("s_waitcnt vmcnt(0)" ::: "memory");
     __builtin_amdgcn_s_barrier();
     asm volatile("" ::: "memory");
 
-    if (g.ksplit > 1) {
-        float* o = reinterpret_cast<float*>(out) + (size_t)ks * g.slab;
-#pragma unroll
-        for (int j = 0; j < RJ; ++j) {
-            const int col = nt * BN + wn * 64 + j * 16 + r16;
-#pragma unroll
-            for (int i = 0; i < 2 * HA; ++i)
-#pragma unroll
-                for (int r = 0; r < 4; ++r) {
-                    const long long m = (long long)mt * BM + wm * 128 + i * 16 + kg * 4 + r;
-                    if (m < M) o[(size_t)m * g.N + col] = acc[i][j][r];
+    auto epilogue = [&](auto full_c) {
+        constexpr bool FULL = decltype(full_c)::value;
+        if (g.ksplit > 1) {
+            float* o = reinterpret_cast<float*>(out) + (size_t)ks * g.slab;
+#pragma unroll
+            for (int j = 0; j < RJ; ++j) {
+                const int col = nt * BN + wn * 64 + j * 16 + r16;
+#pragma unroll
+                for (int i = 0; i < 2 * HA; ++i)
+#pragma unroll
+                    for (int r = 0; r < 4; ++r) {
+                        const unsigned m = (unsigned)mt * BM + wm * 128 + i * 16 + kg * 4 + r;
+                        if (FULL || m < M) o[(size_t)m * g.N + col] = acc[i][j][r];
+                    }
+            }
+            return;
+        }
+        if (!g.out_b3) {
+            float* o = reinterpret_cast<float*>(out);
+#pragma unroll
+            for (int j = 0; j < RJ; ++j) {
+                const int col = nt * BN + wn * 64 + j * 16 + r16;
+                const float sc = scale[col], sh = shift[col];
+#pragma unroll
+                for (int i = 0; i < 2 * HA; ++i)
+#pragma unroll
+                    for (int r = 0; r < 4; ++r) {
+                        const unsigned m = (unsigned)mt * BM + wm * 128 + i * 16 + kg * 4 + r;
+                        float v = fmaf(acc[i][j][r], sc, sh);
+                        if (g.relu) v = fmaxf(v, 0.f);
+                        if (FULL || m < M) o[(size_t)m * g.N + col] = v;
+                    }
+            }
+            return;
+        }
+        __bf16* slice = reinterpret_cast<__bf16*>(smem + wave * B3_SLICE);
+        uint4* o = reinterpret_cast<uint4*>(out);
+        const int nq = g.N / 32 * 12;
+#pragma unroll
+        for (int hh = 0; hh < HA; ++hh) {
+#pragma unroll
+            for (int ii = 0; ii < 2; ++ii) {
+                const int i = hh * 2 + ii;
+#pragma unroll
+                for (int j = 0; j < RJ; ++j) {
+                    const int lc = j * 16 + r16;
+                    const int col = nt * BN + wn * 64 + lc;
+                    const float sc = scale[col], sh = shift[col];
+#pragma unroll
+                    for (int r = 0; r < 4; ++r) {
+                        const int lr = ii * 16 + kg * 4 + r;
+                        float v = fmaf(acc[i][j][r], sc, sh);
+                        if (g.relu) v = fmaxf(v, 0.f);
+                        __bf16 b1, b2, b3;
+                        b3_split(v, b1, b2, b3);
+                        __bf16* p = slice + lr * 192 + (lc >> 5) * 96 + (lc & 31);
+                        p[0] = b1; p[32] = b2; p[64] = b3;
+                    }
                 }
-        }
-        return;
-    }
-    if (!g.out_b3) {
-        float* o = reinterpret_cast<float*>(out);
-#pragma unroll
-        for (int j = 0; j < RJ; ++j) {
-            const int col = nt * BN + wn * 64 + j * 16 + r16;
-            const float sc = scale[col], sh = shift[col];
-#pragma unroll
-            for (int i = 0; i < 2 * HA; ++i)
-#pragma unroll
-                for (int r = 0; r < 4; ++r) {
-                    const long long m = (long long)mt * BM + wm * 128 + i * 16 + kg * 4 + r;
-                    float v = fmaf(acc[i][j][r], sc, sh);
-                    if (g.relu) v = fmaxf(v, 0.f);
-                    if (m < M) o[(size_t)m * g.N + col] = v;
-                }
-        }
-        return;
-    }
-    __bf16* slice = reinterpret_cast<__bf16*>(smem + wave * B3_SLICE);
-    uint4* o = reinterpret_cast<uint4*>(out);
-    const int nq = g.N / 32 * 12;
-#pragma unroll
-    for (int hh = 0; hh < HA; ++hh) {
-#pragma unroll
-        for (int ii = 0; ii < 2; ++ii) {
-            const int i = hh * 2 + ii;
-#pragma unroll
-            for (int j = 0; j < RJ; ++j) {
-                const int lc = j * 16 + r16;
-                const int col = nt * BN + wn * 64 + lc;
-                const float sc = scale[col], sh = shift[col];
-#pragma unroll
-                for (int r = 0; r < 4; ++r) {
-                    const int lr = ii * 16 + kg * 4 + r;
-                    float v = fmaf(acc[i][j][r], sc, sh);
-                    if (g.relu) v = fmaxf(v, 0.f);
-                    __bf16 b1, b2, b3;
-                    b3_split(v, b1, b2, b3);
-                    __bf16* p = slice + lr * 192 + (lc >> 5) * 96 + (lc & 31);
-                    p[0] = b1; p[32] = b2; p[64] = b3;
-                }
-            }
-        }
-        __builtin_amdgcn_s_waitcnt(0xC07F);
-        __builtin_amdgcn_wave_barrier();
-#pragma unroll
-        for (int c = 0; c < 12; ++c) {
-            const int q = c * 64 + lane, lr = q / 24, cq = q - lr * 24;
-            const long long m = (long long)mt * BM + wm * 128 + hh * 32 + lr;
-            const uint4 val = *reinterpret_cast<const uint4*>(reinterpret_cast<const unsigned char*>(slice) + lr * 384 + cq * 16);
-            if (m < M) o[(size_t)m * nq + ((nt * BN + wn * 64) >> 5) * 12 + cq] = val;
-        }
-        __builtin_amdgcn_s_waitcnt(0xC07F);
-        __builtin_amdgcn_wave_barrier();
-    }
+            }
+            __builtin_amdgcn_s_waitcnt(0xC07F);
+            __builtin_amdgcn_wave_barrier();
+#pragma unroll
+            for (int c = 0; c < 12; ++c) {
+                const int q = c * 64 + lane, lr = q / 24, cq = q - lr * 24;
+                const unsigned m = (unsigned)mt * BM + wm * 128 + hh * 32 + lr;
+                const uint4 val = *reinterpret_cast<const uint4*>(reinterpret_cast<const unsigned char*>(slice) + lr * 384 + cq * 16);
+                if (FULL || m < M) o[(size_t)m * nq + ((nt * BN + wn * 64) >> 5) * 12 + cq] = val;
+            }
+            __builtin_amdgcn_s_waitcnt(0xC07F);
+            __builtin_amdgcn_wave_barrier();
+        }
+    };
+    if (full) epilogue(std::true_type()); else epilogue(std::false_type());
+    B3_STAMP_OUT(TAG);
 }
```
